# WilliamVenner/squad-mortar-helper

Hardware: AMD Instinct MI355X
Metric: map frames/sec (1920x1080 full CV pipeline), whole job (higher is better)
Workload: dtype u8/f32

## Files before the change

### include/smh_vision_hip_debug.h

```cpp
#ifndef SMH_VISION_HIP_DEBUG_H
#define SMH_VISION_HIP_DEBUG_H

#include "smh_vision_hip.h"

#ifdef __cplusplus
extern "C" {
#endif

SMHV_API int smhv_debug_lsd_classic(int on);
SMHV_API int smhv_debug_lsd_tile_cap(uint32_t cap);
SMHV_API int smhv_debug_lsd_threads(uint32_t threads);
SMHV_API int smhv_debug_pattern_copy(smhv_batch *b, const void *d_frames, uint32_t n, uint32_t rows_in_flight, void *stream);
SMHV_API int smhv_debug_heightmap_color_map_device(smhv_heightmap *hm, void *d_rgba, float *ms);
SMHV_API int smhv_debug_skip_line_search(int on);
SMHV_API int smhv_debug_lsd_spin_limit(uint32_t polls);
SMHV_API int smhv_debug_no_host_atomics(int on);
SMHV_API int smhv_debug_side_kernel(smhv_ctx *ctx, uint32_t workgroups, void *stream);

SMHV_API int smhv_debug_pipeline_stats(smhv_pipeline *p, uint64_t out[32]);
SMHV_API int smhv_debug_pipeline_peek(smhv_pipeline *p, uint64_t out[16]);

SMHV_API int smhv_debug_marker_table(smhv_ctx *ctx, uint32_t *bits);

SMHV_API int smhv_debug_crc32_host_level(const void *data, uint64_t nbytes, int level, uint32_t *crc);
SMHV_API int smhv_debug_band_rows(uint32_t frame_w, uint32_t frame_h, uint32_t n, int fused, uint32_t *rows, uint32_t *bands, int *tiles);
SMHV_API int smhv_debug_map_band_rows(uint32_t rows);
SMHV_API int smhv_debug_render_form(uint32_t form);
SMHV_API int smhv_debug_render_rule(uint32_t map_w, uint32_t map_h, float sw, float sh, uint32_t hm_w, uint32_t hm_h, float *ratio, float *switch_ratio,
                                    uint32_t *lds_texels, uint32_t *form);
SMHV_API int smhv_debug_feed_rows(uint32_t rows);
SMHV_API int smhv_debug_feed_gray_form(uint32_t form);
SMHV_API int smhv_debug_ingest_feed(smhv_ingest *q, uint32_t n, uint32_t *counter);

#ifdef __cplusplus
}
#endif

#endif
```

### squad-mortar-helper_amd/_lib.py

```python
import ctypes as C
import os

_HERE = os.path.dirname(os.path.abspath(__file__))
LIB_PATH = os.environ.get("SMH_VISION_HIP_LIB") or os.path.join(_HERE, "libsmh_vision_hip.so")

MAX_LINES = 32
MAX_SCALES = 3

STAGE_MARKERS, STAGE_UI_MAP, STAGE_OCR, STAGE_SCALES, STAGE_ALL = 0x1, 0x2, 0x4, 0x8, 0xF
STAGE_MINIMAP = 0x10
STAGE_EXACT_STATS = 0x20
STAGE_LSD_HELPERS = 0x40
STAGE_FIRING = 0x80
STAGE_HEIGHTMAP_OVERLAY = 0x100
FIRING_BOUNDS_OFFSET = 1
FIRING_NONE, FIRING_SCALES, FIRING_HEIGHTMAP = 0, 1, 2
VIEW_NONE, VIEW_OCR_INPUT, VIEW_FIND_SCALES_INPUT, VIEW_LSD_PREPROCESS, VIEW_LSD_INPUT, VIEW_CROPPED_BRQ = range(6)
IMAGE_UI_MAP = 100
IMAGE_HEIGHTMAP_OVERLAY = 101
RENDER_HEIGHTMAP, RENDER_MARKERS, RENDER_BOUNDS_OFFSET = 1, 2, 4
RENDER_MAX_LINES = 256
PRIM_LINE, PRIM_RECT, PRIM_FOREGROUND, PRIM_SHIFT1 = 0, 1, 0x100, 0x200
RENDER_MAX_PRIMS = 256
LAYER_MINIMAP_BOUNDS = 1
# ... 106 lines not shown
                ("team_bits", C.c_uint32), ("reserved1", C.c_uint32)]


class DebugOptionsStruct(C.Structure):
    _fields_ = [("size", C.c_uint32), ("flags", C.c_uint32), ("scale", C.c_uint32), ("n_runs", C.c_uint32), ("runs", C.POINTER(TextRun)),
                ("n_probes", C.c_uint32), ("reserved", C.c_uint32), ("probes", C.POINTER(ProbePoint))]


class FeedEntry(C.Structure):
    _fields_ = [("offset", C.c_uint64), ("length", C.c_uint32), ("frame", C.c_uint32), ("kind", C.c_uint32), ("crc", C.c_uint32)]


class FeedHeader(C.Structure):
    _fields_ = [("n_entries", C.c_uint32), ("frames_done", C.c_uint32), ("n_maps", C.c_uint32), ("has_last_crc", C.c_uint32),
                ("last_crc", C.c_uint32), ("reserved", C.c_uint32), ("bytes_used", C.c_uint64)]


LOG_FN = C.CFUNCTYPE(None, C.c_int, C.c_char_p)

SIGNATURES = {
    "smhv_init": (C.c_int, [C.c_int, LOG_FN, C.POINTER(C.c_void_p)]),
    "smhv_shutdown": (None, [C.c_void_p]),
    "smhv_thread_ctx": (C.c_int, [C.c_void_p]),
    "smhv_set_ray_table": (C.c_int, [C.c_void_p, C.POINTER(C.c_float), C.POINTER(C.c_float)]),
    "smhv_last_error": (C.c_char_p, []),
    "smhv_map_bounds": (C.c_int, [C.c_uint32, C.c_uint32, C.POINTER(C.c_uint32)]),
    "smhv_button_bounds": (C.c_int, [C.c_uint32, C.c_uint32, C.POINTER(C.c_uint32)]),
    "smhv_load_frame": (C.c_int, [C.c_void_p, C.c_void_p, C.c_uint32, C.c_uint32]),
    "smhv_load_frame_view": (C.c_int, [C.c_void_p, C.c_void_p] + [C.c_uint32] * 6),
    "smhv_load_frame_device": (C.c_int, [C.c_void_p, C.c_void_p, C.c_uint32, C.c_uint32]),
    "smhv_crop_to_map": (C.c_int, [C.c_void_p, C.c_int, C.POINTER(C.c_int), C.POINTER(C.c_uint32), C.c_void_p]),
    "smhv_red_pixels": (C.c_int, [C.c_void_p, C.POINTER(C.c_uint32)]),
    "smhv_ocr_preprocess": (C.c_int, [C.c_void_p, C.POINTER(C.c_void_p), C.POINTER(C.c_size_t)]),
    "smhv_find_scales_preprocess": (C.c_int, [C.c_void_p, C.c_uint32, C.POINTER(C.c_void_p), C.POINTER(C.c_uint32), C.POINTER(C.c_uint32)]),
    "smhv_isolate_map_markers": (C.c_int, [C.c_void_p]),
    "smhv_mask_marker_lines": (C.c_int, [C.c_void_p]),
    "smhv_get_lsd_image": (C.c_int, [C.c_void_p, C.c_void_p, C.POINTER(C.c_uint32), C.POINTER(C.c_uint32)]),
    "smhv_find_longest_line": (C.c_int, [C.c_void_p, C.c_float, C.c_float, C.c_float, C.POINTER(Line), C.POINTER(C.c_float)]),
    "smhv_find_marker_lines": (C.c_int, [C.c_void_p, C.c_uint32, C.POINTER(Line), C.POINTER(C.c_uint32)]),
    "smhv_lsd_stats": (C.c_int, [C.c_void_p, C.c_uint32, C.c_int, C.POINTER(C.c_uint32), C.POINTER(C.c_uint64)]),
    "smhv_calc_meters_to_px_ratio": (C.c_int, [C.c_void_p, C.POINTER(C.c_uint32), C.c_uint32, C.POINTER(C.c_double), C.POINTER(C.c_int), C.POINTER(C.c_uint32)]),
    "smhv_find_minimap": (C.c_int, [C.c_void_p, C.POINTER(C.c_uint32), C.POINTER(C.c_int)]),
    "smhv_get_debug_view": (C.c_int, [C.c_void_p, C.c_int, C.c_void_p, C.POINTER(C.c_uint32), C.POINTER(C.c_uint32)]),
    "smhv_batch_create": (C.c_int, [C.c_void_p, C.c_uint32, C.c_uint32, C.c_uint32, C.POINTER(C.c_void_p)]),
    "smhv_batch_destroy": (None, [C.c_void_p]),
    "smhv_batch_layout_get": (C.c_int, [C.c_void_p, C.POINTER(BatchLayout)]),
    "smhv_batch_run": (C.c_int, [C.c_void_p, C.c_void_p, C.c_uint32, C.c_uint32, C.c_int, C.c_uint32, C.c_void_p, C.c_void_p]),
    "smhv_batch_device_ptrs": (C.c_int, [C.c_void_p] + [C.POINTER(C.c_void_p)] * 6),
    "smhv_batch_tile_mask": (C.c_int, [C.c_void_p, C.POINTER(C.c_void_p), C.POINTER(C.c_void_p), C.POINTER(C.c_uint32)]),
    "smhv_batch_read_tile_mask": (C.c_int, [C.c_void_p, C.c_uint32, C.c_void_p, C.c_void_p, C.c_void_p, C.POINTER(C.c_int)]),
    "smhv_batch_read_results": (C.c_int, [C.c_void_p, C.c_uint32, C.c_uint32, C.POINTER(FrameResult)]),
    "smhv_batch_read_image": (C.c_int, [C.c_void_p, C.c_int, C.c_uint32, C.c_void_p]),
    "smhv_batch_set_scales_stream": (C.c_int, [C.c_void_p, C.c_void_p]),
    "smhv_batch_wait_map_pass": (C.c_int, [C.c_void_p, C.c_void_p]),
    "smhv_batch_enable_timing": (C.c_int, [C.c_void_p, C.c_int]),
    "smhv_batch_lsd_coop_stats": (C.c_int, [C.c_void_p, C.c_uint32, C.c_uint32, C.POINTER(C.c_uint32)]),
    "smhv_batch_stage_ms": (C.c_int, [C.c_void_p, C.POINTER(C.c_float)]),
    "smhv_pipeline_create": (C.c_int, [C.c_void_p, C.c_uint32, C.c_uint32, C.c_uint32, C.c_uint32, C.POINTER(C.c_void_p)]),
    "smhv_pipeline_create_ex": (C.c_int, [C.c_void_p, C.c_uint32, C.c_uint32, C.c_uint32, C.c_uint32, C.c_void_p, C.POINTER(C.c_void_p)]),
    "smhv_pipeline_hold": (C.c_int, [C.c_void_p, C.c_uint32, C.c_void_p]),
    "smhv_debug_pipeline_stats": (C.c_int, [C.c_void_p, C.POINTER(C.c_uint64)]),
    "smhv_debug_pipeline_peek": (C.c_int, [C.c_void_p, C.POINTER(C.c_uint64)]),
    "smhv_pipeline_destroy": (None, [C.c_void_p]),
    "smhv_pipeline_submit": (C.c_int, [C.c_void_p, C.c_void_p, C.c_uint32, C.c_uint32, C.c_int, C.c_uint32, C.c_void_p, C.c_void_p, C.POINTER(C.c_uint32)]),
    "smhv_pipeline_wait": (C.c_int, [C.c_void_p, C.c_uint32]),
    "smhv_pipeline_wait_all": (C.c_int, [C.c_void_p]),
    "smhv_pipeline_slot": (C.c_int, [C.c_void_p, C.c_uint32, C.POINTER(C.c_void_p), C.POINTER(C.c_void_p)]),
    "smhv_shard_range": (None, [C.c_uint64, C.c_uint32, C.c_uint32, C.POINTER(C.c_uint64), C.POINTER(C.c_uint64)]),
    "smhv_node_create": (C.c_int, [C.POINTER(C.c_int), C.c_uint32, C.c_uint32, C.c_uint32, C.c_uint32, C.c_uint32, LOG_FN, C.POINTER(C.c_void_p)]),
    "smhv_node_destroy": (None, [C.c_void_p]),
    "smhv_node_ctx": (C.c_int, [C.c_void_p, C.c_uint32, C.POINTER(C.c_void_p), C.POINTER(C.c_void_p)]),
    "smhv_node_run": (C.c_int, [C.c_void_p, C.POINTER(C.c_void_p), C.POINTER(C.c_uint32), C.c_uint32, C.c_int, C.c_uint32, C.POINTER(C.c_void_p)]),
    "smhv_node_gather": (C.c_int, [C.c_void_p, C.POINTER(FrameResult), C.POINTER(C.c_uint32)]),
    "smhv_debug_lsd_classic": (C.c_int, [C.c_int]),
    "smhv_debug_lsd_tile_cap": (C.c_int, [C.c_uint32]),
    "smhv_debug_lsd_spin_limit": (C.c_int, [C.c_uint32]),
    "smhv_debug_lsd_threads": (C.c_int, [C.c_uint32]),
    "smhv_debug_skip_line_search": (C.c_int, [C.c_int]),
    "smhv_debug_no_host_atomics": (C.c_int, [C.c_int]),
    "smhv_debug_side_kernel": (C.c_int, [C.c_void_p, C.c_uint32, C.c_void_p]),
    "smhv_trait_times": (C.c_int, [C.c_void_p, C.POINTER(C.c_uint64), C.POINTER(C.c_uint64), C.c_int]),
    "smhv_ui_map": (C.c_int, [C.c_void_p, C.POINTER(C.c_void_p), C.POINTER(C.c_uint32), C.POINTER(C.c_uint32)]),
    "smhv_debug_pattern_copy": (C.c_int, [C.c_void_p, C.c_void_p, C.c_uint32, C.c_uint32, C.c_void_p]),
    "smhv_debug_marker_table": (C.c_int, [C.c_void_p, C.c_void_p]),
    "smhv_ingest_create": (C.c_int, [C.c_void_p, C.c_uint32, C.c_uint32, C.c_uint32, C.c_uint32, C.POINTER(C.c_void_p)]),
    "smhv_ingest_create_ex": (C.c_int, [C.c_void_p, C.c_uint32, C.c_uint32, C.c_uint32, C.c_uint32, C.c_uint32, C.POINTER(C.c_void_p)]),
    "smhv_crc32_host": (C.c_uint32, [C.c_void_p, C.c_uint64]),
    "smhv_debug_map_band_rows": (C.c_int, [C.c_uint32]),
    "smhv_debug_band_rows": (C.c_int, [C.c_uint32, C.c_uint32, C.c_uint32, C.c_int, C.POINTER(C.c_uint32), C.POINTER(C.c_uint32), C.POINTER(C.c_int)]),
    "smhv_debug_ingest_feed": (C.c_int, [C.c_void_p, C.c_uint32, C.POINTER(C.c_uint32)]),
    "smhv_debug_crc32_host_level": (C.c_int, [C.c_void_p, C.c_uint64, C.c_int, C.POINTER(C.c_uint32)]),
    "smhv_ingest_destroy": (None, [C.c_void_p]),
    "smhv_ingest_local_cpus": (C.c_int, [C.c_void_p, C.c_char_p, C.c_size_t]),
    "smhv_ingest_bind_thread": (C.c_int, [C.c_void_p]),
    "smhv_ingest_acquire": (C.c_int, [C.c_void_p, C.POINTER(C.c_void_p)]),
    "smhv_ingest_commit": (C.c_int, [C.c_void_p]),
    "smhv_ingest_push": (C.c_int, [C.c_void_p, C.c_void_p]),
    "smhv_ingest_commit_pixels": (C.c_int, [C.c_void_p, C.c_uint32]),
    "smhv_ingest_push_pixels": (C.c_int, [C.c_void_p, C.c_void_p, C.c_uint32]),
    "smhv_ingest_batch": (C.c_int, [C.c_void_p, C.POINTER(C.c_void_p), C.POINTER(C.c_uint32), C.POINTER(C.c_uint32)]),
    "smhv_ingest_reset": (C.c_int, [C.c_void_p]),
    "smhv_ingest_counts": (C.c_int, [C.c_void_p, C.POINTER(C.c_uint64), C.POINTER(C.c_uint64)]),
    "smhv_crc32_device": (C.c_int, [C.c_void_p, C.c_void_p, C.c_uint64, C.POINTER(C.c_uint32)]),
    "smhv_heightmap_create": (C.c_int, [C.c_void_p, C.c_void_p, C.c_uint32, C.c_uint32, C.POINTER(C.c_int32), C.POINTER(C.c_float), C.POINTER(C.c_void_p)]),
    "smhv_heightmap_destroy": (None, [C.c_void_p]),
    "smhv_heightmap_color_map": (C.c_int, [C.c_void_p, C.c_void_p]),
    "smhv_debug_heightmap_color_map_device": (C.c_int, [C.c_void_p, C.c_void_p, C.POINTER(C.c_float)]),
    "smhv_batch_set_firing": (C.c_int, [C.c_void_p, C.c_void_p, C.POINTER(FiringOptions)]),
    "smhv_pipeline_set_firing": (C.c_int, [C.c_void_p, C.c_void_p, C.POINTER(FiringOptions)]),
    "smhv_batch_read_firing": (C.c_int, [C.c_void_p, C.c_uint32, C.c_uint32, C.POINTER(FiringResult)]),
    "smhv_batch_firing_ptr": (C.c_int, [C.c_void_p, C.POINTER(C.c_void_p)]),
    "smhv_firing_solutions": (C.c_int, [C.c_void_p, C.c_void_p, C.c_uint32, C.POINTER(C.c_double), C.POINTER(C.c_uint32), C.c_void_p,
                                        C.POINTER(FiringOptions), C.POINTER(Firing)]),
    "smhv_batch_overlay_ptr": (C.c_int, [C.c_void_p, C.POINTER(C.c_void_p)]),
    "smhv_heightmap_overlay": (C.c_int, [C.c_void_p, C.c_void_p, C.POINTER(FiringOptions), C.c_void_p]),
    "smhv_map_viewport_calc": (C.c_int, [C.c_float, C.c_float, C.c_float, C.c_float, C.c_uint32, C.POINTER(C.c_float), C.POINTER(C.c_float),
                                         C.POINTER(RenderOptions)]),
    "smhv_batch_render": (C.c_int, [C.c_void_p, C.c_uint32, C.c_uint32, C.c_void_p, C.POINTER(RenderOptions), C.c_void_p]),
    "smhv_batch_render_ptr": (C.c_int, [C.c_void_p, C.POINTER(C.c_void_p), C.POINTER(C.c_uint64)]),
    "smhv_batch_render_size": (C.c_int, [C.c_void_p, C.POINTER(C.c_uint32), C.POINTER(C.c_uint32)]),
    "smhv_batch_read_render": (C.c_int, [C.c_void_p, C.c_uint32, C.c_void_p]),
    "smhv_batch_render_layers": (C.c_int, [C.c_void_p, C.c_uint32, C.c_uint32, C.c_void_p, C.POINTER(RenderOptions), C.POINTER(RenderLayersStruct), C.c_void_p]),
    "smhv_render_map_layers": (C.c_int, [C.c_void_p, C.c_void_p, C.POINTER(RenderOptions), C.POINTER(RenderLayersStruct), C.c_void_p, C.c_uint32, C.c_void_p]),
    "smhv_render_map": (C.c_int, [C.c_void_p, C.c_void_p, C.POINTER(RenderOptions), C.c_void_p, C.c_uint32, C.c_void_p]),
    "smhv_label_font": (C.c_int, [C.c_uint8, C.POINTER(C.c_uint8)]),
    "smhv_batch_render_labels": (C.c_int, [C.c_void_p, C.c_uint32, C.c_uint32, C.c_void_p, C.POINTER(RenderOptions), C.POINTER(LabelOptionsStruct), C.c_void_p]),
    "smhv_batch_read_labels": (C.c_int, [C.c_void_p, C.c_uint32, C.c_uint32, C.POINTER(LabelResult)]),
    "smhv_batch_labels_ptr": (C.c_int, [C.c_void_p, C.POINTER(C.c_void_p)]),
    "smhv_render_map_labeled": (C.c_int, [C.c_void_p, C.c_void_p, C.POINTER(RenderOptions), C.POINTER(RenderLayersStruct), C.c_void_p, C.c_uint32,
                                          C.POINTER(LabelOptionsStruct), C.c_void_p, C.POINTER(LabelResult)]),
    "smhv_text_font": (C.c_int, [C.c_uint8, C.POINTER(C.c_uint8)]),
    "smhv_probe_text": (C.c_int, [C.POINTER(Probe), C.c_char_p, C.c_size_t]),
    "smhv_batch_probe": (C.c_int, [C.c_void_p, C.c_uint32, C.c_uint32, C.POINTER(RenderOptions), C.POINTER(ProbePoint), C.c_uint32, C.c_void_p]),
    "smhv_batch_read_probes": (C.c_int, [C.c_void_p, C.c_uint32, C.c_uint32, C.POINTER(Probe)]),
    "smhv_batch_probes_ptr": (C.c_int, [C.c_void_p, C.POINTER(C.c_void_p)]),
    "smhv_batch_render_debug": (C.c_int, [C.c_void_p, C.c_uint32, C.c_uint32, C.POINTER(RenderOptions), C.POINTER(DebugOptionsStruct), C.c_void_p]),
    "smhv_render_map_debug": (C.c_int, [C.c_void_p, C.c_void_p, C.POINTER(RenderOptions), C.POINTER(RenderLayersStruct), C.c_void_p, C.c_uint32,
                                        C.POINTER(LabelOptionsStruct), C.POINTER(DebugOptionsStruct), C.c_void_p, C.POINTER(LabelResult), C.POINTER(Probe)]),
    "smhv_feed_create": (C.c_int, [C.c_void_p, C.c_uint64, C.c_uint32, C.POINTER(C.c_void_p)]),
    "smhv_feed_destroy": (None, [C.c_void_p]),
    "smhv_feed_reset": (C.c_int, [C.c_void_p]),
    "smhv_batch_feed": (C.c_int, [C.c_void_p, C.c_void_p, C.c_uint32, C.c_uint32, C.c_uint32, C.c_void_p]),
    "smhv_feed_read": (C.c_int, [C.c_void_p, C.POINTER(FeedHeader), C.POINTER(FeedEntry), C.c_uint32, C.c_void_p, C.c_uint64]),
    "smhv_feed_ptrs": (C.c_int, [C.c_void_p, C.POINTER(C.c_void_p), C.POINTER(C.c_void_p), C.POINTER(C.c_void_p)]),
    "smhv_feed_frame": (C.c_int, [C.c_void_p, C.c_void_p, C.c_void_p, C.c_uint32, C.POINTER(C.c_double), C.POINTER(C.c_uint32), C.c_uint32]),
    "smhv_web_event_markers": (C.c_int, [C.c_void_p, C.c_uint32, C.c_int, C.c_void_p, C.c_uint64, C.POINTER(C.c_uint64)]),
    "smhv_web_event_heightmap": (C.c_int, [C.c_void_p, C.c_uint32, C.c_uint32, C.POINTER(C.c_int32), C.POINTER(C.c_float), C.c_void_p, C.c_uint64,
                                           C.POINTER(C.c_uint64)]),
    "smhv_web_event_fit": (C.c_int, [C.c_int, C.c_void_p, C.c_uint64, C.POINTER(C.c_uint64)]),
    "smhv_web_interaction_parse": (C.c_int, [C.c_void_p, C.c_uint64, C.POINTER(C.c_uint32), C.POINTER(C.c_float), C.POINTER(C.c_uint32)]),
    "smhv_debug_feed_rows": (C.c_int, [C.c_uint32]),
    "smhv_debug_feed_gray_form": (C.c_int, [C.c_uint32]),
    "smhv_batch_feed_view": (C.c_int, [C.c_void_p, C.c_void_p, C.c_uint32, C.c_uint32, C.c_uint32, C.c_uint32, C.c_void_p]),
    "smhv_feed_frame_view": (C.c_int, [C.c_void_p, C.c_void_p, C.c_void_p, C.c_uint32, C.POINTER(C.c_double), C.POINTER(C.c_uint32), C.c_uint32, C.c_uint32]),
    "smhv_debug_render_form": (C.c_int, [C.c_uint32]),
    "smhv_debug_render_rule": (C.c_int, [C.c_uint32, C.c_uint32, C.c_float, C.c_float, C.c_uint32, C.c_uint32, C.POINTER(C.c_float), C.POINTER(C.c_float),
                                         C.POINTER(C.c_uint32), C.POINTER(C.c_uint32)]),
}


def firing_options(fit_to_minimap=True, viewport=None):
    o = FiringOptions()
    o.size = C.sizeof(FiringOptions)
    o.flags = 0 if fit_to_minimap else FIRING_BOUNDS_OFFSET
    if viewport is not None:
        sw, sh, tx, ty = viewport
# ... 62 lines not shown
```

### squad-mortar-helper_amd/batch.py

```python
import ctypes as C

import numpy as np

from . import _lib as L

STAGE_NAMES = ("button", "map_pass", "brq_pass", "lsd", "scale_ratio")


def make_anchors(per_frame):
    arr = (L.Anchors * len(per_frame))()
    for i, (start_y, scales) in enumerate(per_frame):
        arr[i].n = min(len(scales), L.MAX_SCALES)
        arr[i].scales_start_y = start_y
        for j, (m, x, y) in enumerate(scales[:L.MAX_SCALES]):
            arr[i].scales[j][0], arr[i].scales[j][1], arr[i].scales[j][2] = m, x, y
    return arr


def results_to_dicts(recs):
    out = []
    for r in recs:
        n = r.n_lines
        out.append(dict(
            map_open=int(r.map_open), n_lines=int(n),
            lines=np.array([[r.lines[i].x0, r.lines[i].y0, r.lines[i].x1, r.lines[i].y1] for i in range(n)], np.float32).reshape(-1, 4),
            mpx=(r.mpx if r.has_mpx else None), n_mask_px=int(r.n_mask_px), red_pixels=int(r.red_pixels),
            rounds=int(r.rounds), ray_steps=int(r.ray_steps),
            length_px=np.array(r.length_px[:n], np.float64), meters=np.array(r.meters[:n], np.float64),
            angle=np.array(r.angle[:n], np.float32),
            minimap=(tuple(r.minimap) if r.has_minimap else None),
            status=int(r.status), error=(None if r.status == L.FRAME_OK else "line search gave the frame up (SMHV_FRAME_LSD_STUCK)" if r.status == L.FRAME_LSD_STUCK
                                         else "status %d" % r.status)))
    return out


class FrameBatch:

    def __init__(self, vision, frame_w, frame_h, max_frames, _handle=None):
        self._lib = L.load()
        self._vision = vision
        self._owned = _handle is None
        if _handle is None:
            b = C.c_void_p()
            L.check(self._lib.smhv_batch_create(vision._ctx, frame_w, frame_h, max_frames, C.byref(b)))
        else:
            b = _handle
        self._b = b
        self.max_frames = max_frames
        self.frame_w, self.frame_h = frame_w, frame_h
        self.layout = L.BatchLayout()
        L.check(self._lib.smhv_batch_layout_get(self._b, C.byref(self.layout)))

    def close(self):
        if self._b:
            if self._owned:
                self._lib.smhv_batch_destroy(self._b)
            self._b = None

    def __del__(self):
        try:
            self.close()
        except Exception:
            pass

    @property
    def roi(self):
        return tuple(self.layout.roi)

    def enable_timing(self, on=True):
        L.check(self._lib.smhv_batch_enable_timing(self._b, int(on)))

    def run(self, frames_ptr, n, stages=L.STAGE_ALL, grayscale=True, max_gap=15, anchors=None, stream=0):
        if anchors is not None and len(anchors) < n:
            raise ValueError("anchors holds %d entries, the run covers %d frames" % (len(anchors), n))
        a = C.cast(anchors, C.c_void_p) if anchors is not None else None
        L.check(self._lib.smhv_batch_run(self._b, C.c_void_p(frames_ptr), n, stages, int(bool(grayscale)), max_gap, a, C.c_void_p(stream)))

    def set_scales_stream(self, stream=0):
        L.check(self._lib.smhv_batch_set_scales_stream(self._b, C.c_void_p(stream)))

    def wait_map_pass(self, stream=0):
        L.check(self._lib.smhv_batch_wait_map_pass(self._b, C.c_void_p(stream)))

    def stage_ms(self):
        ms = (C.c_float * 5)()
        L.check(self._lib.smhv_batch_stage_ms(self._b, ms))
        return dict(zip(STAGE_NAMES, [float(v) for v in ms]))

    def lsd_coop_stats(self, first=0, n=None):
        n = self.max_frames - first if n is None else n
        out = np.zeros((n, 4), np.uint32)
        L.check(self._lib.smhv_batch_lsd_coop_stats(self._b, first, n, out.ctypes.data_as(C.POINTER(C.c_uint32))))
        return out

    def device_ptrs(self):
        p = [C.c_void_p() for _ in range(6)]
        L.check(self._lib.smhv_batch_device_ptrs(self._b, *[C.byref(x) for x in p]))
        return dict(zip(("results", "ui", "mask", "ocr", "scales", "bits"), [x.value for x in p]))

    def tile_mask(self, frame=0):
        geo = (C.c_uint32 * 4)()
        L.check(self._lib.smhv_batch_tile_mask(self._b, None, None, geo))
        trows, wcols, opitch, xoff = [int(v) for v in geo]
        tiled = np.zeros((trows, wcols, 8), np.uint32)
        occ = np.zeros((trows, opitch), np.uint8)
        bits = np.zeros((self.roi[3], wcols), np.uint32)
        written = C.c_int(0)
        L.check(self._lib.smhv_batch_read_tile_mask(self._b, frame, tiled.ctypes.data, occ.ctypes.data, bits.ctypes.data, C.byref(written)))
        return (tiled if written.value else None), (occ if written.value else None), bits, xoff

    def read_results(self, first=0, n=None, check=True):
        n = self.max_frames - first if n is None else n
        recs = (L.FrameResult * n)()
        rc = self._lib.smhv_batch_read_results(self._b, first, n, recs)
        if rc != 0 and not (rc == L.E_STATE and not check):
            try:
                L.check(rc)
            except L.VisionError as e:
                e.records = recs if rc == L.E_STATE else None
                raise
        return recs

    def set_firing(self, heightmap=None, fit_to_minimap=True, viewport=None):
        opt = L.firing_options(fit_to_minimap, viewport)
        L.check(self._lib.smhv_batch_set_firing(self._b, heightmap._hm if heightmap is not None else None, C.byref(opt)))

    def read_firing(self, first=0, n=None):
        n = self.max_frames - first if n is None else n
        out = (L.FiringResult * n)()
        L.check(self._lib.smhv_batch_read_firing(self._b, first, n, out))
        raw = np.frombuffer(out, np.uint8).reshape(n, C.sizeof(L.FiringResult))
        n_lines = raw[:, :4].copy().view(np.uint32).reshape(n)
        lines = raw[:, 8:].copy().view(L.firing_dtype()).reshape(n, L.MAX_LINES)
        return n_lines, lines

    def firing_ptr(self):
        d = C.c_void_p()
        L.check(self._lib.smhv_batch_firing_ptr(self._b, C.byref(d)))
        return d.value or 0

    def read_overlay(self, frame):
        return self.read_image(L.IMAGE_HEIGHTMAP_OVERLAY, frame)

    def overlay_ptr(self):
        d = C.c_void_p()
        L.check(self._lib.smhv_batch_overlay_ptr(self._b, C.byref(d)))
        return d.value or 0

    def render(self, viewport, out_w, out_h, first=0, n=None, heightmap=None, markers=False, fit_to_minimap=True, background=(0, 0, 0, 255),
               stream=None, options=None, layers=None):
        from .render import render_options
        n = self.max_frames - first if n is None else n
        opt = options if options is not None else render_options(viewport, out_w, out_h, heightmap is not None, markers, fit_to_minimap, background)
        if layers is not None:
            ly, keep = layers.struct()
            L.check(self._lib.smhv_batch_render_layers(self._b, first, n, heightmap._hm if heightmap is not None else None, C.byref(opt), C.byref(ly), stream))
            del keep
            return
        L.check(self._lib.smhv_batch_render(self._b, first, n, heightmap._hm if heightmap is not None else None, C.byref(opt), stream))

    def render_size(self):
        w, h = C.c_uint32(), C.c_uint32()
        L.check(self._lib.smhv_batch_render_size(self._b, C.byref(w), C.byref(h)))
        return int(w.value), int(h.value)

    def read_render(self, frame):
        w, h = self.render_size()
        out = np.empty((h, w, 4), np.uint8)
        L.check(self._lib.smhv_batch_read_render(self._b, frame, out.ctypes.data))
        return out

    def render_ptr(self):
        d, st = C.c_void_p(), C.c_uint64()
        L.check(self._lib.smhv_batch_render_ptr(self._b, C.byref(d), C.byref(st)))
        return d.value or 0, int(st.value)

    def render_labels(self, options, labels, first=0, n=None, heightmap=None, stream=None):
        n = self.max_frames - first if n is None else n
        lo, keep = labels.struct()
        L.check(self._lib.smhv_batch_render_labels(self._b, first, n, heightmap._hm if heightmap is not None else None, C.byref(options), C.byref(lo), stream))
        del keep
# ... 149 lines not shown
```

### squad-mortar-helper_amd/csrc/smh_feed.inc

```

struct smhv_feed {
	smhv_ctx *ctx = nullptr;
	uint64_t capacity = 0;
	uint32_t max_frames = 0;
	uint8_t *d_bytes = nullptr;
	smhv_feed_header *d_header = nullptr;
	smhv_feed_entry *d_entries = nullptr;
	uint32_t *d_state = nullptr, *d_raw = nullptr, *d_tab = nullptr;
	FeedMap *d_maps = nullptr;
	uint32_t tab_w = 0, tab_h = 0, tab_xoff = 0, tab_ppg = 0;
	uint8_t *d_view = nullptr;
	size_t view_cap = 0;
	hipEvent_t ev_last = nullptr;
	bool used = false;
	smhv_frame_result *d_rec = nullptr, *h_rec = nullptr;
};

extern "C" SMHV_API void smhv_feed_destroy(smhv_feed *f) {
	if (!f) return;
	if (f->ctx) (void)hipSetDevice(f->ctx->device);
	(void)hipDeviceSynchronize();
	void *ptrs[] = {f->d_bytes, f->d_header, f->d_entries, f->d_state, f->d_raw, f->d_tab, f->d_maps, f->d_rec, f->d_view};
	for (void *p : ptrs)
		if (p) (void)hipFree(p);
// ... 77 lines not shown
	const uint32_t cquads = image ? SMH_FEED_IMAGE_ROW / 4u : v.quads, cxoff = image ? 0u : v.xoff;
	if (f->tab_w != cw || f->tab_h != ch || f->tab_xoff != cxoff || f->tab_ppg != v.ppg) {
		if (v.ppg == 4u) HIPCHK(launch_feed_tables(f->d_tab, cw, ch, cxoff, cquads, s));
		else HIPCHK(launch_feed_view_tables(f->d_tab, cw, ch, cxoff, cquads, v.ppg, s));
		f->tab_w = cw; f->tab_h = ch; f->tab_xoff = cxoff; f->tab_ppg = v.ppg;
	}
	FeedRun r;
	memset(&r, 0, sizeof r);
	r.ui = v.base; r.res = res;
	r.ui_stride = v.stride; r.ui_pitch = v.pitch;
	r.w = v.w; r.h = v.h; r.xoff = v.xoff; r.quads = v.quads;
	r.n = n; r.first = first; r.flags = flags;
	r.len_term = crc32_mul(crc32_xpow(32ull * v.w * v.h), 0xFFFFFFFFu) ^ 0xFFFFFFFFu;
	r.rows_per_wave = feed_rows_per_wave(ch, n);
	r.capacity = f->capacity;
	r.raw = f->d_raw; r.tab = f->d_tab; r.state = f->d_state;
	r.header = f->d_header; r.entries = f->d_entries; r.bytes = f->d_bytes; r.maps = f->d_maps;
	if (v.mode == SMH_RND_SRC_UI) HIPCHK(launch_feed(r, s));
	else if (!image) HIPCHK(launch_feed_view(r, v.mode, s));
	else {
		FeedRun c = r;
		c.ui = v.base - 4ull * v.lead; c.ui_pitch = 4ull * SMH_FEED_IMAGE_ROW; c.ui_stride = 0;
		c.w = cw; c.h = ch; c.xoff = 0u; c.quads = cquads;
		HIPCHK(launch_feed_image(c, r, s));
	}
	HIPCHK(hipEventRecord(f->ev_last, s));
	f->used = true;
	return SMHV_OK;
}

static int feed_batch_source(const smhv_batch *b, uint32_t first, uint32_t map_source, bool resolve, FeedSrc *v) {
	const Geom &g = b->g;
	if (map_source > (uint32_t)SMHV_VIEW_CROPPED_BRQ) return fail(SMHV_E_INVALID, "batch_feed_view: unknown map source %u", map_source);
	if (resolve && !b->ui_written) return fail(SMHV_E_STATE, "batch_feed: no run of this batch has produced a ui_map (SMHV_STAGE_UI_MAP)");
	*v = feed_src_ui(g, b->d_ui + (size_t)first * g.ui_stride);
	switch ((int)map_source) {
	case SMHV_VIEW_NONE: break;
	case SMHV_VIEW_OCR_INPUT:
	case SMHV_VIEW_FIND_SCALES_INPUT: {
		const bool ocr = map_source == (uint32_t)SMHV_VIEW_OCR_INPUT;
		if (resolve && !(ocr ? b->ocr_written : b->scales_written))
			return fail(SMHV_E_STATE, "batch_feed_view: no run of this batch has produced the %s image", ocr ? "OCR input (SMHV_STAGE_OCR)" : "scales input (SMHV_STAGE_SCALES with anchors)");
		v->mode = SMH_RND_SRC_GRAY; v->ppg = 16u;
		v->base = (ocr ? b->d_ocr : b->d_scales) + (size_t)first * g.ocr_stride;
		v->pitch = g.ocr_pitch; v->stride = g.ocr_stride; v->xoff = g.q_xoff; v->w = g.qw; v->h = g.qh;
		v->quads = (v->w + v->xoff + 15u) / 16u;
		break;
	}
	case SMHV_VIEW_LSD_INPUT:
		if (resolve && !b->mask_written) return fail(SMHV_E_STATE, "batch_feed_view: no run of this batch has produced the marker mask (SMHV_STAGE_MARKERS)");
		v->mode = SMH_RND_SRC_GRAY; v->ppg = 16u;
		v->base = b->d_mask + (size_t)first * g.mask_stride;
		v->pitch = g.mask_pitch; v->stride = g.mask_stride;
		v->quads = (v->w + v->xoff + 15u) / 16u;
		break;
	default:
		if (resolve && b->ui_gray) return fail(SMHV_E_STATE, "batch_feed_view: the batch's ui_map is grayscale, map source %u needs the colour one", map_source);
		if (map_source == (uint32_t)SMHV_VIEW_CROPPED_BRQ) {
			const uint32_t x0 = g.m_xoff + g.rw / 2u;
			v->mode = SMH_RND_SRC_CROPPED; v->w = g.rw / 2u; v->h = g.rh / 2u;
			if (resolve && (v->w == 0u || v->h == 0u)) return fail(SMHV_E_STATE, "batch_feed_view: the map has no bottom right quarter");
			v->base += (size_t)(g.rh / 2u) * g.ui_pitch + 16ull * (x0 / 4u);
			v->xoff = x0 & 3u; v->quads = (v->w + v->xoff + 3u) / 4u;
		} else v->mode = SMH_RND_SRC_PREPROCESS;
		break;
	}
	return SMHV_OK;
}

extern "C" SMHV_API int smhv_batch_feed_view(smhv_batch *b, smhv_feed *f, uint32_t first, uint32_t n, uint32_t flags, uint32_t map_source, void *stream) {
	if (!b || !f) return fail(SMHV_E_INVALID, "batch_feed: null argument");
	CTX_OPEN(b->ctx);
	CTX_OPEN(f->ctx);
	if (f->ctx->device != b->ctx->device) return fail(SMHV_E_INVALID, "batch_feed: the feed lives on device %d, the batch on %d", f->ctx->device, b->ctx->device);
	if (n == 0u || (uint64_t)first + n > b->max_frames) return fail(SMHV_E_INVALID, "batch_feed: frames [%u, %u + %u) of a batch of %u", first, first, n, b->max_frames);
	FeedSrc v;
	int rc = feed_batch_source(b, first, map_source, false, &v);
	if (rc) return rc;
	rc = feed_check(f, v.w, v.h, n, flags, "batch_feed");
	if (rc) return rc;
	rc = feed_batch_source(b, first, map_source, true, &v);
	if (rc) return rc;
	HIPCHK(hipSetDevice(b->ctx->device));
	return feed_enqueue(f, v, b->d_results + first, first, n, flags, (hipStream_t)stream);
}

extern "C" SMHV_API int smhv_batch_feed(smhv_batch *b, smhv_feed *f, uint32_t first, uint32_t n, uint32_t flags, void *stream) {
	return smhv_batch_feed_view(b, f, first, n, flags, (uint32_t)SMHV_VIEW_NONE, stream);
}

extern "C" SMHV_API int smhv_feed_read(smhv_feed *f, smhv_feed_header *header, smhv_feed_entry *entries, uint32_t max_entries, uint8_t *bytes, uint64_t cap) {
	if (!f || !header) return fail(SMHV_E_INVALID, "feed_read: null argument");
	CTX_OPEN(f->ctx);
	HIPCHK(hipSetDevice(f->ctx->device));
	if (f->used) HIPCHK(wait_event(f->ev_last));
	HIPCHK(hipMemcpy(header, f->d_header, sizeof *header, hipMemcpyDeviceToHost));
	if (entries && header->n_entries > max_entries) return fail(SMHV_E_INVALID, "feed_read: %u entries, room for %u", header->n_entries, max_entries);
	if (bytes && header->bytes_used > cap) return fail(SMHV_E_INVALID, "feed_read: %llu bytes, room for %llu", (unsigned long long)header->bytes_used, (unsigned long long)cap);
	if (entries && header->n_entries) HIPCHK(hipMemcpy(entries, f->d_entries, sizeof(smhv_feed_entry) * header->n_entries, hipMemcpyDeviceToHost));
	if (bytes && header->bytes_used) HIPCHK(hipMemcpy(bytes, f->d_bytes, (size_t)header->bytes_used, hipMemcpyDeviceToHost));
	return SMHV_OK;
}

extern "C" SMHV_API int smhv_feed_ptrs(smhv_feed *f, void **d_header, void **d_entries, void **d_bytes) {
	if (!f) return fail(SMHV_E_INVALID, "feed_ptrs: null feed");
	if (d_header) *d_header = f->d_header;
	if (d_entries) *d_entries = f->d_entries;
	if (d_bytes) *d_bytes = f->d_bytes;
	return SMHV_OK;
}

extern "C" SMHV_API int smhv_debug_feed_gray_form(uint32_t form) {
	if (form != 0u && form != 4u) return fail(SMHV_E_INVALID, "feed gray form %u (0 = the rule, 4 = four lookups per message dword)", form);
	feed_set_gray_form(form);
	return SMHV_OK;
}

extern "C" SMHV_API int smhv_debug_feed_rows(uint32_t rows) {
	if (rows > 64u) return fail(SMHV_E_INVALID, "feed rows per wave %u (0 = the rule, 1 .. 64)", rows);
	feed_set_rows(rows);
	return SMHV_OK;
}

extern "C" SMHV_API int smhv_feed_frame_view(smhv_ctx *c, smhv_feed *f, const smhv_line *lines, uint32_t n_lines, const double *mpx, const uint32_t minimap[4],
                                             uint32_t flags, uint32_t map_source) {
	int rc = require_open(c, "feed_frame");
	if (rc) return rc;
	CTX_OPEN(c);
	if (!f || (n_lines && !lines)) return fail(SMHV_E_INVALID, "feed_frame: null argument");
	CTX_OPEN(f->ctx);
	if (f->ctx->device != c->device) return fail(SMHV_E_INVALID, "feed_frame: the feed lives on device %d, the context on %d", f->ctx->device, c->device);
	if (n_lines > SMHV_MAX_LINES) return fail(SMHV_E_INVALID, "feed_frame: %u lines (at most %u)", n_lines, (unsigned)SMHV_MAX_LINES);
	if (map_source > (uint32_t)SMHV_VIEW_CROPPED_BRQ) return fail(SMHV_E_INVALID, "feed_frame_view: unknown map source %u", map_source);
	smhv_batch *b = c->fb;
	const Geom &g = b->g;
	FeedSrc v = feed_src_ui(g, b->d_ui);
	if (map_source != (uint32_t)SMHV_VIEW_NONE) {
		const int which = (int)map_source;
		const bool brq = which == SMHV_VIEW_OCR_INPUT || which == SMHV_VIEW_FIND_SCALES_INPUT || which == SMHV_VIEW_CROPPED_BRQ;
		v.mode = SMH_RND_SRC_RGBA; v.w = brq ? g.qw : g.rw; v.h = brq ? g.qh : g.rh;
		v.xoff = 0u; v.quads = 0u; v.pitch = 4ull * v.w; v.stride = 0;
	}
	rc = feed_check(f, v.w, v.h, 1, flags, "feed_frame");
	if (rc) return rc;
	HIPCHK(hipSetDevice(c->device));
	if (f->used) HIPCHK(wait_event(f->ev_last));
	if (v.mode == SMH_RND_SRC_RGBA) {
		const uint64_t dw = (uint64_t)v.w * v.h, rows = (dw + SMH_FEED_IMAGE_ROW - 1u) / SMH_FEED_IMAGE_ROW;
		const size_t need = (size_t)rows * SMH_FEED_IMAGE_ROW * 4u;
		if (rows > SMH_FEED_MAX_ROWS) return fail(SMHV_E_INVALID, "feed_frame_view: a view of %u x %u pixels", v.w, v.h);
		if (f->view_cap < need) {
			if (f->d_view) (void)hipFree(f->d_view);
			f->d_view = nullptr; f->view_cap = 0;
			HIPCHK(hipMalloc((void **)&f->d_view, need));
			f->view_cap = need;
		}
		v.lead = (uint32_t)(rows * SMH_FEED_IMAGE_ROW - dw);
		v.base = f->d_view + 4ull * v.lead;
		if (v.lead) HIPCHK(hipMemsetAsync(f->d_view, 0, 4ull * v.lead, c->s_main));
		Buffers bf = make_buffers(b, c->frame_ptr, 0);
		HIPCHK(launch_debug_view(g, bf, 0, (int)map_source, c->isolated ? 1 : 0, f->d_view + 4ull * v.lead, c->s_main));
	}
	smhv_frame_result *h = f->h_rec;
	memset(h, 0, sizeof *h);
	h->map_open = 1u; h->status = SMHV_FRAME_OK;
	h->n_lines = n_lines;
// ... 83 lines not shown
```

### squad-mortar-helper_amd/csrc/smh_kernels.h

```cpp
#pragma once
#include <hip/hip_runtime.h>
#include <stdint.h>

#include "../../include/smh_vision_hip.h"
#include "../../include/smh_vision_hip_debug.h"

namespace smh {

struct Geom {
	uint32_t W, H;
	uint32_t rx, ry, rw, rh;
	uint32_t bx, by, bw, bh;
	uint32_t qx, qy, qw, qh;
	uint32_t m_ax, m_xoff, m_quads, m_block;
	uint32_t q_ax, q_xoff, q_quads, q_block;
	uint64_t frame_bytes;
	uint64_t ui_pitch, ui_stride;
	uint64_t mask_pitch, mask_stride;
	uint32_t bits_pitch_w; uint64_t bits_stride_w;
	uint64_t ocr_pitch, ocr_stride;
};

struct FrameAux {
	uint32_t open;
// ... 206 lines not shown
#define SMH_CULL_CELLS (SMH_SECTOR_DIM * 4)
#define SMH_CULL_TAB_WORDS (SMH_CULL_CELLS + (SMH_SECTOR_ENTRIES + 3) / 4)

#define SVC_MAX_SLOTS 32u
struct SvcSlot {
	Buffers b;
	uint32_t n;
	uint32_t seq;
	uint32_t done;
	uint32_t pad;
	unsigned long long t_pub;
};
#define SVC_REMOTE_RING 12u
#define SVC_REMOTE_OPEN 0x80000000ull
struct SvcRemoteEntry {
	unsigned long long post;
	unsigned long long claim;
	uint32_t res_a[4];
	uint32_t res_b[4];
	unsigned long long pad[2];
};
struct SvcRemote {
	unsigned long long state;
	unsigned long long info;
	unsigned long long pad[6];
	SvcRemoteEntry ring[SVC_REMOTE_RING];
};
#define SVC_HELP_RING 256u
struct SvcCtl {
	int32_t avail;
	uint32_t closing;
	int32_t help_avail;
	uint32_t help_head, help_reserve;
	uint32_t stat_remote;
	uint32_t head;
	uint32_t reserve;
	uint32_t completed;
	uint32_t busy;
	uint32_t stat_items, stat_waves;
	unsigned long long stat_busy, stat_life;
	unsigned long long stat_phase[4];
	unsigned long long stat_help;
	uint32_t stat_requests, stat_attached;
	unsigned long long stat_t_wait, stat_t_sub, stat_t_last;
	uint32_t stat_h_polls, stat_h_empty, stat_h_lost, stat_h_idle_exit, stat_h_closed_exit, stat_h_pad;
	unsigned long long stat_h_cycles, stat_h_cast_cycles;
	unsigned long long help_ring[SVC_HELP_RING];
};
struct SvcHost {
	unsigned long long state;
	uint32_t launches;
	uint32_t pad0;
	uint32_t done_seq[SVC_MAX_SLOTS];
	uint32_t pad[12];
};
struct SvcParams {
	SvcCtl *ctl;
	unsigned long long *ring;
	SvcSlot *slots;
	SvcHost *host;
	const uint32_t *cull_tab;
	const float *ray_off;
	float max_gap;
	uint32_t tile_cap, list_cap;
	uint32_t part_words;
	uint32_t ring_log2;
	uint32_t epoch;
	uint32_t idle_short, idle_long;
	uint32_t flags;
	SvcRemote *remote;
	uint32_t *remote_store;
	uint32_t remote_store_words;
	uint32_t remote_after;
	uint32_t remote_tickets;
	uint32_t remote_last_div;
	uint32_t compact;
};
uint32_t svc_waves_for(const Geom &g, uint32_t tile_limit, uint32_t *part_words, uint32_t *tile_cap, uint32_t *list_cap, uint32_t *lds_bytes, uint32_t *compact = nullptr);
uint32_t svc_store_words_for(const Geom &g, uint32_t tile_cap, uint32_t compact);
hipError_t svc_probe_host_atomics(SvcHost *h, SvcHost *d_h, bool *ok);
hipError_t launch_svc_publish(SvcCtl *ctl, unsigned long long *ring, SvcSlot *slots, uint32_t slot, const Buffers &b, uint32_t n, uint32_t seq, uint32_t ring_log2, hipStream_t s);
hipError_t launch_lsd_service(const Geom &g, const SvcParams &p, uint32_t workgroups, uint32_t waves, uint32_t lds_bytes, hipStream_t s);

enum : uint32_t { MAP_UI = 1u, MAP_MASK = 2u, MAP_PRIO = 0x100u, MAP_BAND_MAJOR = 0x200u };
enum : uint32_t { BRQ_OCR = 1u, BRQ_SCALES = 2u };

hipError_t launch_button(const Geom &g, const Buffers &b, uint32_t n, int force_open, hipStream_t s);
hipError_t launch_map_pass(const Geom &g, const Buffers &b, uint32_t n, uint32_t flags, int grayscale, hipStream_t s, bool tiles_wanted = false, bool overlapped = false);
struct LaunchTuning {
	uint32_t map_lds_total;
	uint32_t map_grid_cap;
	uint32_t lsd_tile_limit;
	uint32_t map_prio;
	uint32_t map_deep;
	uint32_t map_overlapped;
};
uint32_t map_brq_lds_bytes(const Geom &g);
uint32_t lsd_tile_lds_bytes(const Geom &g, uint32_t tile_limit);
hipError_t launch_map_brq_pass(const Geom &g, const Buffers &b, uint32_t n, uint32_t flags, uint32_t qflags, int grayscale, uint32_t fixed_start_y, int use_anchor_start, hipStream_t s,
                               const LaunchTuning *tune = nullptr);
hipError_t launch_pattern_copy(const Geom &g, const Buffers &b, uint32_t n, uint32_t rows_in_flight, hipStream_t s);
void map_band_rows(uint32_t rh, uint32_t n, int fused, uint32_t *rows, int *tiles);
hipError_t launch_brq_pass(const Geom &g, const Buffers &b, uint32_t n, uint32_t flags, uint32_t fixed_start_y, int use_anchor_start, hipStream_t s);
struct LsdFork { hipStream_t s1, s2; hipEvent_t fork, join1, join2; };
bool lsd_rows_only(const Geom &g);
hipError_t launch_lsd(const Geom &g, const Buffers &b, uint32_t n, float max_gap, int mode, float px, float py, hipStream_t s, const LsdFork *fk, uint32_t tile_bs = 0,
                      bool prefer_classic = false, uint32_t tile_limit = 0, bool *record_fused = nullptr);
size_t lsd_coop_ctl_bytes(uint32_t n);
hipError_t launch_scale_ratio(const Geom &g, const Buffers &b, uint32_t n, uint32_t *d_bars, hipStream_t s);
hipError_t launch_find_minimap(const Geom &g, const Buffers &b, uint32_t n, hipStream_t s);
hipError_t launch_finalize(const Geom &g, const Buffers &b, uint32_t n, uint32_t stages, hipStream_t s);
hipError_t launch_scales_finalize(const Geom &g, const Buffers &b, uint32_t n, uint32_t stages, uint32_t *d_bars, hipStream_t s);
hipError_t launch_firing_lines(const FiringRun &r, const smhv_line *lines, uint32_t n, uint32_t has_mpx, double mpx, uint32_t has_minimap,
                               const uint32_t minimap[4], smhv_firing *out, hipStream_t s);
hipError_t launch_heightmap_color_map(const uint16_t *hm, uint64_t n, uint32_t *mm, uint32_t *rgba, hipStream_t s);
#define SMH_HM_LUT_ENTRIES 65536u
hipError_t launch_heightmap_lut(const uint16_t *hm, uint64_t n, uint32_t *mm, uint32_t *lut, hipStream_t s);
hipError_t launch_hm_overlay(const Geom &g, const OverlayRun &r, uint32_t n, hipStream_t s);
hipError_t launch_render_map(const Geom &g, const RenderRun &r, uint32_t n, hipStream_t s);
hipError_t launch_render_map_layers(const Geom &g, const RenderRun &r, const RenderLayersRun &y, uint32_t n, hipStream_t s);
hipError_t launch_heightmap_lut16(const uint32_t *lut, uint16_t *lut16, uint32_t *vr, hipStream_t s);
#define SMH_HM_LUT_WORDS (SMH_HM_LUT_ENTRIES + 4u + SMH_HM_LUT_ENTRIES / 2u)
hipError_t launch_labels(const LabelRun &r, uint32_t n, hipStream_t s);
hipError_t launch_debug_text(const Geom &g, const DebugRun &r, uint32_t n, hipStream_t s);
void render_set_form(uint32_t form);
uint32_t render_rule(const Geom &g, const RenderRun &r, uint32_t *texels, float *ratio);
float render_switch_ratio();
hipError_t launch_debug_view(const Geom &g, const Buffers &b, uint32_t frame, int which, int isolated, uint8_t *d_rgba, hipStream_t s);
hipError_t launch_marker_table(uint32_t *d_bits, hipStream_t s);
hipError_t launch_pack_rows(const void *d_src, uint32_t src_pitch_bytes, void *d_dst, uint32_t row_bytes, uint32_t rows, hipStream_t s);
hipError_t launch_side_probe(uint32_t *d_out, uint32_t workgroups, uint32_t spin, hipStream_t s);
hipError_t launch_build_sector_table(unsigned long long *d_tab, uint32_t T, hipStream_t s);
hipError_t launch_build_ray_offsets(float *d_off, hipStream_t s);
size_t lsd_lds_bytes();
void lsd_set_classic(bool on);
void lsd_set_tile_cap(uint32_t cap);
void lsd_set_threads(uint32_t threads);
void lsd_set_spin_limit(uint32_t polls);
hipError_t set_ray_table(const float *dx, const float *dy);
#define SMH_CRC_BS 1024
hipError_t launch_to_bgra(const void *d_src, void *d_bgra, uint64_t n_px, uint32_t layout, hipStream_t s);
hipError_t launch_unpack_rows(const void *d_pack, void *d_frame, uint32_t pitch_px, uint32_t roi_x, uint32_t roi_y, uint32_t roi_w, uint32_t roi_h, uint32_t btn_x,
                              uint32_t btn_y, uint32_t btn_w, uint32_t btn_h, hipStream_t s);
hipError_t launch_crc32(const void *d_msg, uint64_t n_dwords, uint32_t wgs, uint32_t rounds, uint32_t x_skip, const uint32_t *d_x_local,
                        const uint32_t *d_x_wg, uint32_t *d_acc, hipStream_t s);
uint32_t crc32_xpow(uint64_t n);
uint32_t crc32_mul(uint32_t a, uint32_t b);

struct FeedMap { uint64_t dst; uint32_t frame, pad; };
struct FeedRun {
	const uint8_t *ui;
	const smhv_frame_result *res;
	uint64_t ui_stride, ui_pitch;
	uint32_t w, h, xoff, quads;
	uint32_t n, first, flags;
	uint32_t len_term;
	uint32_t rows_per_wave;
	uint64_t capacity;
	uint32_t *raw;
	const uint32_t *tab;
	uint32_t *state;
	smhv_feed_header *header;
	smhv_feed_entry *entries;
	uint8_t *bytes;
	FeedMap *maps;
};
#define SMH_FEED_MAX_ROWS 16384u
hipError_t launch_feed_tables(uint32_t *d_tab, uint32_t w, uint32_t h, uint32_t xoff, uint32_t quads, hipStream_t s);
uint32_t feed_rows_per_wave(uint32_t h, uint32_t n);
void feed_set_rows(uint32_t rows);
hipError_t launch_feed(const FeedRun &r, hipStream_t s);
#define SMH_FEED_IMAGE_ROW 1024u
hipError_t launch_feed_view_tables(uint32_t *d_tab, uint32_t w, uint32_t h, uint32_t xoff, uint32_t quads, uint32_t ppg, hipStream_t s);
hipError_t launch_feed_view(const FeedRun &r, uint32_t src_mode, hipStream_t s);
hipError_t launch_feed_image(const FeedRun &crc, const FeedRun &r, hipStream_t s);
void feed_set_gray_form(uint32_t form);

}
```

### squad-mortar-helper_amd/csrc/smh_misc.hip

```cpp
#include "smh_device.h"
#include "smh_record.inc"

namespace smh {

__global__ void __launch_bounds__(64 * SMHV_MAX_SCALES) k_scale_ratio(Geom g, Buffers b, uint32_t *bars) { scale_ratio_body(g, b, blockIdx.x, bars); }

__device__ __forceinline__ bool flat_pixel(const uint8_t *roi0, uint32_t W, uint32_t x, uint32_t y) {
	const uint32_t *p = (const uint32_t *)(roi0 + ((size_t)y * W + x) * 4);
	const int Wi = (int)W;
	const uint32_t c = p[0] & 0x00FFFFFFu;
	uint32_t mx = 0;
#pragma unroll
	for (int dy = -1; dy <= 1; ++dy)
#pragma unroll
		for (int dx = -1; dx <= 1; ++dx)
			if (dx != 0 || dy != 0) mx = max(mx, (uint32_t)__builtin_amdgcn_sad_u8(c, p[dy * Wi + dx] & 0x00FFFFFFu, 0u));
	return (float)mx / 765.0f <= 0.01f;
}

__device__ uint32_t find_edge(const uint8_t *roi0, uint32_t W, uint32_t w, uint32_t h, uint32_t x0, uint32_t y0, int dir) {
	const uint32_t lane = threadIdx.x & 63u;
	const bool vertical = dir < 2;
	uint32_t c_max = vertical ? h : w, oc_max = vertical ? w : h;
	const int cod = (dir == 0 || dir == 2) ? -1 : 1;
// ... 254 lines not shown
__global__ void k_debug_view(Geom g, Buffers b, uint32_t f, int which, int isolated, uint8_t *out) {
	const bool brq = which == SMHV_VIEW_OCR_INPUT || which == SMHV_VIEW_FIND_SCALES_INPUT || which == SMHV_VIEW_CROPPED_BRQ;
	const uint32_t w = brq ? g.qw : g.rw, h = brq ? g.qh : g.rh;
	const uint32_t i = blockIdx.x * blockDim.x + threadIdx.x;
	if (i >= w * h) return;
	const uint32_t y = i / w, x = i - y * w;
	const uint8_t *fp = b.frames + (size_t)f * g.frame_bytes;
	uint32_t o;
	if (which == SMHV_VIEW_OCR_INPUT || which == SMHV_VIEW_FIND_SCALES_INPUT) {
		const uint8_t *img = (which == SMHV_VIEW_OCR_INPUT ? b.ocr : b.scales) + (size_t)f * g.ocr_stride + g.q_xoff;
		o = (uint32_t)img[(size_t)y * g.ocr_pitch + x] * 0x00010101u | 0xFF000000u;
	} else if (which == SMHV_VIEW_LSD_INPUT) {
		o = (uint32_t)b.mask[(size_t)f * g.mask_stride + (size_t)y * g.mask_pitch + g.m_xoff + x] * 0x00010101u | 0xFF000000u;
	} else {
		const uint32_t fx = brq ? g.qx + x : g.rx + x, fy = brq ? g.qy + y : g.ry + y;
		const uint32_t p = *(const uint32_t *)(fp + ((size_t)fy * g.W + fx) * 4);
		uint32_t bb = p & 255u, gg = (p >> 8) & 255u, rr = (p >> 16) & 255u;
		if (which == SMHV_VIEW_LSD_PREPROCESS && isolated && !is_marker(rr, gg, bb)) { rr = 0; gg = 0; bb = 0; }
		o = rr | (gg << 8) | (bb << 16) | 0xFF000000u;
	}
	((uint32_t *)out)[i] = o;
}

__global__ void k_marker_table(uint32_t *bits) {
	const uint32_t w = blockIdx.x * blockDim.x + threadIdx.x;
	if (w >= (1u << 24) / 32u) return;
	uint32_t acc = 0;
	for (uint32_t k = 0; k < 32; ++k) {
		const uint32_t c = w * 32u + k;
		if (is_marker((c >> 16) & 255u, (c >> 8) & 255u, c & 255u)) acc |= 1u << k;
	}
	bits[w] = acc;
}

__global__ void __launch_bounds__(256) k_side_probe(uint32_t *out, uint32_t spin) {
	__shared__ uint32_t lds[21u * 256u];
	asm volatile("; the register footprint of the kernel this one stands in for" ::: "v255", "a23");
	for (uint32_t i = threadIdx.x; i < 21u * 256u; i += blockDim.x) lds[i] = i ^ blockIdx.x;
	__syncthreads();
	uint32_t acc = lds[(threadIdx.x * 37u) % (21u * 256u)];
	for (uint32_t i = 0; i < spin; ++i) acc = acc * 1664525u + 1013904223u;
	if (threadIdx.x == 0) out[blockIdx.x] = acc;
}
hipError_t launch_side_probe(uint32_t *d_out, uint32_t workgroups, uint32_t spin, hipStream_t s) {
	hipLaunchKernelGGL(k_side_probe, dim3(workgroups), dim3(256), 0, s, d_out, spin);
	return hipGetLastError();
}

hipError_t launch_scale_ratio(const Geom &g, const Buffers &b, uint32_t n, uint32_t *d_bars, hipStream_t s) {
	hipLaunchKernelGGL(k_scale_ratio, dim3(n), dim3(64 * SMHV_MAX_SCALES), 0, s, g, b, d_bars);
	return hipGetLastError();
}

hipError_t launch_find_minimap(const Geom &g, const Buffers &b, uint32_t n, hipStream_t s) {
	hipLaunchKernelGGL(k_find_minimap, dim3(n), dim3(256), 0, s, g, b);
	return hipGetLastError();
}

hipError_t launch_finalize(const Geom &g, const Buffers &b, uint32_t n, uint32_t stages, hipStream_t s) {
	if (stages & SMHV_STAGE_FIRING) hipLaunchKernelGGL(k_finalize_firing, dim3(n), dim3(64), 0, s, g, b, stages);
	else hipLaunchKernelGGL(k_finalize, dim3(n), dim3(64), 0, s, g, b, stages);
	return hipGetLastError();
}

hipError_t launch_scales_finalize(const Geom &g, const Buffers &b, uint32_t n, uint32_t stages, uint32_t *d_bars, hipStream_t s) {
	if (stages & SMHV_STAGE_FIRING) hipLaunchKernelGGL(k_scales_finalize_firing, dim3(n), dim3(64 * SMHV_MAX_SCALES), 0, s, g, b, stages, d_bars);
	else hipLaunchKernelGGL(k_scales_finalize, dim3(n), dim3(64 * SMHV_MAX_SCALES), 0, s, g, b, stages, d_bars);
	return hipGetLastError();
}

__global__ void __launch_bounds__(256) k_pack_rows(const uint32_t *__restrict__ src, uint32_t src_pitch_w, uint32_t *__restrict__ dst, uint32_t row_w, uint32_t rows) {
	const uint32_t r = blockIdx.y;
	const uint32_t *s = src + (size_t)r * src_pitch_w;
	uint32_t *d = dst + (size_t)r * row_w;
	for (uint32_t x = blockIdx.x * blockDim.x + threadIdx.x; x < row_w; x += gridDim.x * blockDim.x) d[x] = s[x];
}
hipError_t launch_pack_rows(const void *d_src, uint32_t src_pitch_bytes, void *d_dst, uint32_t row_bytes, uint32_t rows, hipStream_t s) {
	if ((src_pitch_bytes | row_bytes) & 3u) return hipErrorInvalidValue;
	const uint32_t row_w = row_bytes / 4u;
	hipLaunchKernelGGL(k_pack_rows, dim3((row_w + 255u) / 256u, rows), dim3(256), 0, s, (const uint32_t *)d_src, src_pitch_bytes / 4u, (uint32_t *)d_dst, row_w, rows);
	return hipGetLastError();
}

hipError_t launch_debug_view(const Geom &g, const Buffers &b, uint32_t frame, int which, int isolated, uint8_t *d_rgba, hipStream_t s) {
	const bool brq = which == SMHV_VIEW_OCR_INPUT || which == SMHV_VIEW_FIND_SCALES_INPUT || which == SMHV_VIEW_CROPPED_BRQ;
	const uint32_t npx = brq ? g.qw * g.qh : g.rw * g.rh;
	hipLaunchKernelGGL(k_debug_view, dim3((npx + 255) / 256), dim3(256), 0, s, g, b, frame, which, isolated, d_rgba);
	return hipGetLastError();
}

hipError_t launch_marker_table(uint32_t *d_bits, hipStream_t s) {
	hipLaunchKernelGGL(k_marker_table, dim3(((1u << 24) / 32u + 255) / 256), dim3(256), 0, s, d_bits);
	return hipGetLastError();
}

#define CRC_POLY SMH_CRC_POLY
#define CRC_BS 1024

__global__ void __launch_bounds__(CRC_BS) k_crc32(const uint32_t *msg, uint64_t n_dwords, uint32_t rounds, uint32_t x_skip,
                                                 const uint32_t *x_local, const uint32_t *x_wg, uint32_t *acc) {
	__shared__ uint32_t tab[4][256];
	__shared__ uint32_t wsum[CRC_BS / 64];
	const uint32_t tid = threadIdx.x;
	if (tid < 256u) {
		uint32_t c = tid;
		for (int k = 0; k < 8; ++k) c = (c >> 1) ^ ((c & 1u) ? CRC_POLY : 0u);
		tab[0][tid] = c;
	}
	__syncthreads();
	if (tid < 256u) {
		uint32_t c = tab[0][tid];
		for (int k = 1; k < 4; ++k) { c = (c >> 8) ^ tab[0][c & 255u]; tab[k][tid] = c; }
	}
	__syncthreads();
	const uint64_t G = (uint64_t)gridDim.x * CRC_BS, T = (uint64_t)blockIdx.x * CRC_BS + tid;
	const uint64_t pad = (uint64_t)rounds * G * 4u - n_dwords;
	uint32_t v = 0;
	for (uint32_t r = 0; r < rounds; ++r) {
		const uint64_t vi = ((uint64_t)r * G + T) * 4u;
		uint32_t d[4] = {0u, 0u, 0u, 0u};
		if (vi >= pad && ((vi - pad) & 3u) == 0u && (((uintptr_t)msg) & 15u) == 0u) {
			const uint4 q = *(const uint4 *)(msg + (vi - pad));
			d[0] = q.x; d[1] = q.y; d[2] = q.z; d[3] = q.w;
		} else {
#pragma unroll
			for (int j = 0; j < 4; ++j) if (vi + j >= pad) d[j] = msg[vi + j - pad];
		}
		if (r) v = gf2_mulmod(v, x_skip);
#pragma unroll
		for (int j = 0; j < 4; ++j) {
			const uint32_t c = v ^ d[j];
			v = tab[3][c & 255u] ^ tab[2][(c >> 8) & 255u] ^ tab[1][(c >> 16) & 255u] ^ tab[0][c >> 24];
		}
	}
	v = gf2_mulmod(v, x_local[tid]);
	v = wave_xor32_dpp(v);
	if ((tid & 63u) == 0u) wsum[tid >> 6] = v;
	__syncthreads();
	if (tid == 0) {
		uint32_t w = 0;
		for (int k = 0; k < CRC_BS / 64; ++k) w ^= wsum[k];
		atomicXor(acc, gf2_mulmod(w, x_wg[blockIdx.x]));
	}
}

uint32_t crc32_xpow(uint64_t n) {
	uint32_t r = 0x80000000u, b = 0x40000000u;
	for (; n; n >>= 1) { if (n & 1u) r = gf2_mulmod(r, b); b = gf2_mulmod(b, b); }
	return r;
}
uint32_t crc32_mul(uint32_t a, uint32_t b) { return gf2_mulmod(a, b); }

hipError_t launch_crc32(const void *d_msg, uint64_t n_dwords, uint32_t wgs, uint32_t rounds, uint32_t x_skip, const uint32_t *d_x_local,
                        const uint32_t *d_x_wg, uint32_t *d_acc, hipStream_t s) {
	hipLaunchKernelGGL(k_crc32, dim3(wgs), dim3(CRC_BS), 0, s, (const uint32_t *)d_msg, n_dwords, rounds, x_skip, d_x_local, d_x_wg, d_acc);
	return hipGetLastError();
}

template <int BPP>
__global__ void __launch_bounds__(256) k_to_bgra(const uint32_t *__restrict__ src, uint4 *__restrict__ dst, uint64_t n_groups, uint64_t n_px) {
	for (uint64_t gidx = (uint64_t)blockIdx.x * 256u + threadIdx.x; gidx < n_groups; gidx += (uint64_t)gridDim.x * 256u) {
		uint32_t w[4] = {0u, 0u, 0u, 0u}, px[4];
		const uint64_t n_src_dwords = (n_px * BPP + 3u) / 4u;
#pragma unroll
		for (int k = 0; k < BPP; ++k) { const uint64_t i = gidx * BPP + k; if (i < n_src_dwords) w[k] = src[i]; }
		if (BPP == 4) {
// ... 60 lines not shown
```

### squad-mortar-helper_amd/csrc/smh_runtime.cpp

```cpp
#include <hip/hip_runtime.h>

#include <atomic>
#include <condition_variable>
#include <deque>
#include <thread>
#include <cmath>
#include <cstdarg>
#include <cstdio>
#include <cstdlib>
#include <cstring>
#include <ctime>
#include <sched.h>
#include <pthread.h>
#include <cctype>
#include <mutex>
#include <vector>
#include <new>
#include <string>

#include "smh_consts.h"
#include "smh_kernels.h"

using namespace smh;

// ... 90 lines not shown
	if ((uint64_t)xr + w > W || (uint64_t)yb + h > H || w == 0 || h == 0)
		return fail(SMHV_E_GEOMETRY, "frame %ux%u: button bounds underflow", W, H);
	out[0] = W - xr - w; out[1] = H - yb - h; out[2] = w; out[3] = h;
	return SMHV_OK;
}

static int compute_geom(uint32_t W, uint32_t H, Geom *g) {
	uint32_t m[4], bt[4];
	int rc = smhv_map_bounds(W, H, m);
	if (rc) return rc;
	rc = smhv_button_bounds(W, H, bt);
	if (rc) return rc;
	memset(g, 0, sizeof *g);
	g->W = W; g->H = H;
	g->rx = m[0]; g->ry = m[1]; g->rw = m[2]; g->rh = m[3];
	g->bx = bt[0]; g->by = bt[1]; g->bw = bt[2]; g->bh = bt[3];
	g->qw = g->rw / 2; g->qh = g->rh / 2;
	g->qx = g->rx + g->qw; g->qy = g->ry + g->qh;
	if (g->qw < SMH_OCR_DILATE_RADIUS || g->qh < SMH_OCR_DILATE_RADIUS) return fail(SMHV_E_GEOMETRY, "frame %ux%u too small", W, H);
	g->m_ax = g->rx & ~3u; g->m_xoff = g->rx - g->m_ax;
	g->m_quads = (g->rw + g->m_xoff + 3u) / 4u;
	g->m_block = (g->m_quads + 63u) & ~63u;
	g->q_ax = g->qx & ~3u; g->q_xoff = g->qx - g->q_ax;
	g->q_quads = (g->qw + g->q_xoff + 3u) / 4u;
	g->q_block = (g->q_quads + 63u) & ~63u;
	if (g->m_block > 1024u) return fail(SMHV_E_GEOMETRY, "frame %ux%u: map ROI wider than 4096 px is not supported", W, H);
	const uint32_t mq = (g->m_quads + 15u) & ~15u, qq = (g->q_quads + 15u) & ~15u;
	g->frame_bytes = (uint64_t)W * H * 4;
	g->ui_pitch = (uint64_t)mq * 16; g->ui_stride = g->ui_pitch * g->rh;
	g->mask_pitch = (uint64_t)mq * 4; g->mask_stride = g->mask_pitch * g->rh;
	g->bits_pitch_w = mq / 8; g->bits_stride_w = (uint64_t)g->bits_pitch_w * g->rh;
	g->ocr_pitch = (uint64_t)qq * 4; g->ocr_stride = g->ocr_pitch * g->qh;
	return SMHV_OK;
}

struct smhv_batch {
	smhv_ctx *ctx = nullptr;
	Geom g{};
	uint32_t max_frames = 0;
	uint8_t *d_ui = nullptr, *d_mask = nullptr, *d_ocr = nullptr, *d_scales = nullptr;
	uint32_t *d_bits = nullptr, *d_bars = nullptr, *d_tiled = nullptr;
	uint8_t *d_occ = nullptr;
	FrameAux *d_aux = nullptr;
	smhv_frame_result *d_results = nullptr;
	smhv_anchors *d_anchors = nullptr;
	BatchError *h_err = nullptr, *d_err = nullptr;
	FarmFrame *d_farm = nullptr;
	uint8_t *d_lsd_ctl = nullptr;
	uint32_t *d_lsd_req = nullptr;
	LsdCacheEntry *d_lsd_cache = nullptr;
	uint32_t lsd_epoch = 0;
	struct AnchorStage { smhv_anchors *h = nullptr; hipEvent_t done = nullptr; };
	std::vector<AnchorStage> anchor_stage;
	static constexpr int TIMING_RING = 64;
	static constexpr int TIMING_EVENTS = 10;
	bool timing = false;
	hipEvent_t (*ev)[TIMING_EVENTS] = nullptr;
	uint64_t timed_runs = 0;
	hipStream_t s_scales = nullptr;
	hipStream_t s_scales_ext = nullptr;
	hipEvent_t ev_map_done = nullptr;
	hipEvent_t ev_fork = nullptr, ev_join = nullptr;
	LsdFork lsd_fork{};
	uint32_t lsd_late_kc = 0;
	uint32_t lsd_bs = 1024;
	bool lsd_prefer_classic = false;
	LaunchTuning tune{0u, 0u, 0u, 0u};
	hipEvent_t ev_probe[3] = {nullptr, nullptr, nullptr};
	bool probe = false, probe_valid = false;
	smhv_heightmap *fire_hm = nullptr;
	smhv_firing_options fire_opt{};
	smhv_firing_result *d_firing = nullptr;
	FiringRun *d_fire_run = nullptr;
	struct FireStage { FiringRun *h = nullptr; hipEvent_t done = nullptr; };
	std::vector<FireStage> fire_stage;
	uint8_t *d_overlay = nullptr;
	uint8_t *d_render = nullptr;
	size_t render_cap = 0;
	uint32_t render_w = 0, render_h = 0;
	smhv_heightmap *render_hm = nullptr;
	hipEvent_t ev_render = nullptr;
	bool ui_written = false;
	bool ui_gray = false, mask_written = false, ocr_written = false, scales_written = false;
	smhv_render_prim *h_prims = nullptr, *d_prims = nullptr;
	hipEvent_t ev_prims = nullptr;
	smhv_label_result *d_labels = nullptr;
	LabelCull *d_label_cull = nullptr;
	smhv_label_line *h_label_extra = nullptr, *d_label_extra = nullptr;
	hipEvent_t ev_label_extra = nullptr;
	smhv_heightmap *label_hm = nullptr;
	smhv_probe *d_probes = nullptr;
	DebugItem *d_dbg_items = nullptr;
	uint8_t *d_dbg_pool = nullptr, *h_dbg_stage = nullptr, *d_dbg_stage = nullptr;
	hipEvent_t ev_dbg_stage = nullptr, ev_dbg = nullptr;
	bool probed = false;
};

struct smhv_heightmap {
	smhv_ctx *ctx = nullptr;
	uint16_t *d = nullptr;
	uint32_t w = 0, h = 0;
	int32_t bounds[4] = {0, 0, 0, 0};
	float scale[3] = {0.0f, 0.0f, 0.0f};
	std::atomic<int> refs{1};
	mutable std::mutex lut_mu;
	mutable std::atomic<uint32_t *> d_lut{nullptr};
};
static void hm_retain(smhv_heightmap *hm) { if (hm) hm->refs.fetch_add(1, std::memory_order_relaxed); }
static void hm_release(smhv_heightmap *hm);

struct smhv_ctx {
	int device = 0;
	smhv_log_fn log = nullptr;
	hipStream_t s_main = nullptr, s_markers = nullptr, s_scales = nullptr;
	hipStream_t s_ui = nullptr;
	hipEvent_t ev_map = nullptr, ev_ui[2] = {nullptr, nullptr};
	hipEvent_t ev_ui_part[3] = {nullptr, nullptr, nullptr};
	uint8_t *h_ui[2] = {nullptr, nullptr};
	size_t h_ui_cap[2] = {0, 0};
	uint8_t *d_ui_tight = nullptr;
	size_t d_ui_tight_cap = 0;
	uint8_t *d_fire = nullptr, *h_fire = nullptr;
	size_t fire_cap = 0;
	std::mutex fire_mu;
	uint32_t ui_turn = 0;
	bool ui_pending = false, minimap_cached = false;
	uint32_t W = 0, H = 0;
	bool have_frame = false;
	uint8_t *d_frame = nullptr;
	size_t d_frame_cap = 0;
	const uint8_t *frame_ptr = nullptr;
	smhv_batch *fb = nullptr;
	uint8_t *h_ocr = nullptr, *h_scales = nullptr;
	uint8_t *h_stage[3] = {nullptr, nullptr, nullptr};
	size_t h_stage_cap[3] = {0, 0, 0};
	smhv_frame_result *h_res = nullptr;
	FrameAux *h_aux = nullptr;
	uint32_t *h_bars = nullptr;
	bool cropped = false, map_open = false, isolated = false, mask_valid = false, scales_valid = false;
	static constexpr int SECTOR_CACHE = 8;
	uint32_t sector_T[SECTOR_CACHE] = {};
	uint32_t *sector_tab[SECTOR_CACHE] = {};
	int sector_n = 0;
	float *d_ray_off = nullptr;
	uint32_t *d_side = nullptr;
	std::atomic<uint64_t> tt_ns[SMHV_TRAIT_CALLS] = {}, tt_calls[SMHV_TRAIT_CALLS] = {};
	std::mutex mu;
	std::atomic<int> refs{1};
	std::atomic<bool> closed{false};
};

static std::mutex g_ctx_mu;
static std::vector<smhv_ctx *> g_ctx_open;

static void ctx_release(smhv_ctx *c) {
	if (c && c->refs.fetch_sub(1, std::memory_order_acq_rel) == 1) delete c;
}
#define CTX_OPEN(c)                                                                                          \
	do {                                                                                                     \
		if (!(c) || (c)->closed.load(std::memory_order_acquire)) return fail(SMHV_E_INVALID, "the context was shut down"); \
	} while (0)

static void logf(smhv_ctx *c, int lvl, const char *fmt, ...) {
	if (!c || !c->log) return;
	char buf[512];
	va_list ap;
// ... 181 lines not shown
	g_no_host_atomics.store(on != 0, std::memory_order_relaxed);
	return SMHV_OK;
}
extern "C" SMHV_API int smhv_debug_side_kernel(smhv_ctx *c, uint32_t workgroups, void *stream) {
	if (!c || workgroups == 0 || workgroups > 1024u) return fail(SMHV_E_INVALID, "side_kernel: 1..1024 workgroups");
	CTX_OPEN(c);
	HIPCHK(hipSetDevice(c->device));
	if (!c->d_side) HIPCHK(hipMalloc((void **)&c->d_side, 1024u * sizeof(uint32_t)));
	HIPCHK(launch_side_probe(c->d_side, workgroups, 64u, (hipStream_t)stream));
	return SMHV_OK;
}
extern "C" SMHV_API int smhv_debug_lsd_threads(uint32_t threads) {
	if (threads != 0 && (threads < 128 || threads > 1024 || threads % 64)) return fail(SMHV_E_INVALID, "lsd_threads: 0 or a multiple of 64 from 128 to 1024");
	lsd_set_threads(threads);
	return SMHV_OK;
}

extern "C" SMHV_API int smhv_debug_lsd_spin_limit(uint32_t polls) {
	lsd_set_spin_limit(polls);
	return SMHV_OK;
}

extern "C" SMHV_API int smhv_set_ray_table(smhv_ctx *c, const float *dx, const float *dy) {
	if (!c || !dx || !dy) return fail(SMHV_E_INVALID, "bad arguments");
	CTX_OPEN(c);
	for (int i = 0; i < SMH_LSD_RAYS; ++i) {
		const double a = (double)i / 10.0 * 3.14159265358979323846 / 180.0;
		if (!(std::fabs((double)dx[i] - std::cos(a)) < 1e-5 && std::fabs((double)dy[i] - std::sin(a)) < 1e-5))
			return fail(SMHV_E_INVALID, "ray table entry %d is not (cos, sin) of %.1f degrees", i, i / 10.0);
	}
	std::lock_guard<std::mutex> lk(g_ctx_mu);
	HIPCHK(hipSetDevice(c->device));
	HIPCHK(hipDeviceSynchronize());
	HIPCHK(set_ray_table(dx, dy));
	for (smhv_ctx *o : g_ctx_open)
		if (o->device == c->device && o->d_ray_off) HIPCHK(launch_build_ray_offsets(o->d_ray_off, c->s_main));
	HIPCHK(hipStreamSynchronize(c->s_main));
	return SMHV_OK;
}

static hipError_t create_stream(hipStream_t *st, const uint32_t *cu_mask) {
	return cu_mask ? hipExtStreamCreateWithCUMask(st, 8, cu_mask) : hipStreamCreateWithFlags(st, hipStreamNonBlocking);
}

extern "C" SMHV_API int smhv_batch_create(smhv_ctx *c, uint32_t W, uint32_t H, uint32_t max_frames, smhv_batch **out) {
	if (!c || !out || max_frames == 0) return fail(SMHV_E_INVALID, "bad arguments");
	*out = nullptr;
	CTX_OPEN(c);
	Geom g;
	int rc = compute_geom(W, H, &g);
	if (rc) return rc;
	HIPCHK(hipSetDevice(c->device));
	smhv_batch *b = new (std::nothrow) smhv_batch();
	if (!b) return fail(SMHV_E_INVALID, "out of host memory");
	c->refs.fetch_add(1, std::memory_order_relaxed);
	b->ctx = c; b->g = g; b->max_frames = max_frames;
	const size_t n = max_frames;
#define ALLOC0(ptr, bytes)                                          \
	do {                                                            \
		hipError_t _e = hipMalloc((void **)&(ptr), (bytes));        \
		if (_e == hipSuccess) _e = hipMemset((ptr), 0, (bytes));    \
		if (_e != hipSuccess) { smhv_batch_destroy(b); return fail(SMHV_E_HIP, "allocating %zu bytes: %s", (size_t)(bytes), hipGetErrorString(_e)); } \
	} while (0)
	ALLOC0(b->d_ui, g.ui_stride * n);
	ALLOC0(b->d_mask, g.mask_stride * n);
	ALLOC0(b->d_bits, g.bits_stride_w * 4 * n);
	ALLOC0(b->d_tiled, tiled_stride_w(g) * 4 * n);
	ALLOC0(b->d_occ, occ_stride(g) * n);
	ALLOC0(b->d_ocr, g.ocr_stride * n);
	ALLOC0(b->d_scales, g.ocr_stride * n);
	ALLOC0(b->d_aux, sizeof(FrameAux) * n);
	ALLOC0(b->d_results, sizeof(smhv_frame_result) * (n + 3));
	ALLOC0(b->d_anchors, sizeof(smhv_anchors) * n);
	ALLOC0(b->d_bars, sizeof(uint32_t) * SMHV_MAX_SCALES * 4 * n);
	ALLOC0(b->d_lsd_ctl, lsd_coop_ctl_bytes(max_frames));
	ALLOC0(b->d_lsd_req, sizeof(uint32_t) * SMH_LSD_REQ_CAP * n);
	ALLOC0(b->d_farm, sizeof(FarmFrame) * n);
	ALLOC0(b->d_lsd_cache, sizeof(LsdCacheEntry) * SMH_LSD_CACHE_SLOTS * n);
#undef ALLOC0
	{
		hipError_t e = hipHostMalloc((void **)&b->h_err, sizeof(BatchError), hipHostMallocMapped | hipHostMallocCoherent);
		if (e == hipSuccess) { memset(b->h_err, 0, sizeof(BatchError)); e = hipHostGetDevicePointer((void **)&b->d_err, b->h_err, 0); }
		if (e == hipSuccess) e = hipEventCreateWithFlags(&b->ev_map_done, hipEventDisableTiming);
		if (max_frames > 1 && !lsd_rows_only(b->g)) {
			if (e == hipSuccess) e = create_stream(&b->lsd_fork.s1, nullptr);
			if (e == hipSuccess) e = create_stream(&b->lsd_fork.s2, nullptr);
			if (e == hipSuccess) e = hipEventCreateWithFlags(&b->lsd_fork.fork, hipEventDisableTiming);
			if (e == hipSuccess) e = hipEventCreateWithFlags(&b->lsd_fork.join1, hipEventDisableTiming);
			if (e == hipSuccess) e = hipEventCreateWithFlags(&b->lsd_fork.join2, hipEventDisableTiming);
		}
		if (e != hipSuccess) { smhv_batch_destroy(b); return fail(SMHV_E_HIP, "branch streams: %s", hipGetErrorString(e)); }
	}
	*out = b;
	return SMHV_OK;
}

extern "C" SMHV_API void smhv_batch_destroy(smhv_batch *b) {
	if (!b) return;
	if (b->ctx) (void)hipSetDevice(b->ctx->device);
	(void)hipDeviceSynchronize();
	void *ptrs[] = {b->d_ui, b->d_mask, b->d_bits, b->d_tiled, b->d_occ, b->d_ocr, b->d_scales, b->d_aux, b->d_results, b->d_anchors, b->d_bars, b->d_farm,
	                b->d_lsd_ctl, b->d_lsd_req, b->d_lsd_cache, b->d_firing, b->d_fire_run, b->d_overlay, b->d_render, b->d_prims, b->d_labels,
	                b->d_label_cull, b->d_label_extra, b->d_probes, b->d_dbg_items, b->d_dbg_pool, b->d_dbg_stage};
	for (void *p : ptrs)
		if (p) (void)hipFree(p);
	if (b->h_prims) (void)hipHostFree(b->h_prims);
	if (b->ev_prims) (void)hipEventDestroy(b->ev_prims);
	if (b->h_label_extra) (void)hipHostFree(b->h_label_extra);
	if (b->ev_label_extra) (void)hipEventDestroy(b->ev_label_extra);
	if (b->h_dbg_stage) (void)hipHostFree(b->h_dbg_stage);
	if (b->ev_dbg_stage) (void)hipEventDestroy(b->ev_dbg_stage);
	if (b->ev_dbg) (void)hipEventDestroy(b->ev_dbg);
	if (b->h_err) (void)hipHostFree(b->h_err);
	for (auto &a : b->anchor_stage) {
		if (a.h) (void)hipHostFree(a.h);
		if (a.done) (void)hipEventDestroy(a.done);
	}
	for (auto &a : b->fire_stage) {
		if (a.h) (void)hipHostFree(a.h);
		if (a.done) (void)hipEventDestroy(a.done);
	}
	hm_release(b->fire_hm);
	hm_release(b->render_hm);
	hm_release(b->label_hm);
	if (b->ev_render) (void)hipEventDestroy(b->ev_render);
	if (b->ev) {
		for (int r = 0; r < smhv_batch::TIMING_RING; ++r)
			for (int i = 0; i < smhv_batch::TIMING_EVENTS; ++i) if (b->ev[r][i]) (void)hipEventDestroy(b->ev[r][i]);
		delete[] b->ev;
	}
	if (b->s_scales) (void)hipStreamDestroy(b->s_scales);
	if (b->ev_fork) (void)hipEventDestroy(b->ev_fork);
	if (b->ev_join) (void)hipEventDestroy(b->ev_join);
	if (b->ev_map_done) (void)hipEventDestroy(b->ev_map_done);
	for (auto e : b->ev_probe) if (e) (void)hipEventDestroy(e);
	if (b->lsd_fork.s1) (void)hipStreamDestroy(b->lsd_fork.s1);
	if (b->lsd_fork.s2) (void)hipStreamDestroy(b->lsd_fork.s2);
	if (b->lsd_fork.fork) (void)hipEventDestroy(b->lsd_fork.fork);
	if (b->lsd_fork.join1) (void)hipEventDestroy(b->lsd_fork.join1);
	if (b->lsd_fork.join2) (void)hipEventDestroy(b->lsd_fork.join2);
	ctx_release(b->ctx);
	delete b;
}

static int batch_check_errors(smhv_batch *b, const char *what) {
	BatchError *e = b->h_err;
	if (!e) return SMHV_OK;
	const uint32_t count = __atomic_load_n(&e->count, __ATOMIC_ACQUIRE);
	if (count == 0) return SMHV_OK;
	const BatchError snap = *e;
	memset(e, 0, sizeof *e);
	logf(b->ctx, 1, "%s: %u frame(s) failed, first: frame %u status %u", what, count, snap.frame, snap.status);
	if (snap.status == SMHV_FRAME_LSD_STUCK)
		return fail(SMHV_E_STATE, "%s: %u frame(s) without marker lines (status != 0 in their records); first: frame %u, line search gave up "
		            "(SMHV_FRAME_LSD_STUCK: head %u tail %u list %u/%u lines %u rounds %u spec %u head-state %u)", what, count, snap.frame,
		            snap.info[0], snap.info[1], snap.info[2], snap.info[3], snap.info[4], snap.info[5], snap.info[6], snap.info[7]);
	return fail(SMHV_E_STATE, "%s: %u frame(s) failed; first: frame %u, status %u", what, count, snap.frame, snap.status);
}
extern "C" int smhv_internal_batch_check(smhv_batch *b, const char *what) { return b ? batch_check_errors(b, what) : SMHV_OK; }

extern "C" SMHV_API int smhv_batch_layout_get(smhv_batch *b, smhv_batch_layout *o) {
	if (!b || !o) return fail(SMHV_E_INVALID, "bad arguments");
	const Geom &g = b->g;
	memset(o, 0, sizeof *o);
	o->frame_w = g.W; o->frame_h = g.H;
	o->roi[0] = g.rx; o->roi[1] = g.ry; o->roi[2] = g.rw; o->roi[3] = g.rh;
	o->button[0] = g.bx; o->button[1] = g.by; o->button[2] = g.bw; o->button[3] = g.bh;
	o->brq_w = g.qw; o->brq_h = g.qh;
	o->ui_pitch = g.ui_pitch; o->ui_stride = g.ui_stride; o->ui_offset = (uint64_t)g.m_xoff * 4;
	o->mask_pitch = g.mask_pitch; o->mask_stride = g.mask_stride; o->mask_offset = g.m_xoff;
	o->ocr_pitch = g.ocr_pitch; o->ocr_stride = g.ocr_stride; o->ocr_offset = g.q_xoff;
	o->scales_pitch = g.ocr_pitch; o->scales_stride = g.ocr_stride; o->scales_offset = g.q_xoff;
	o->bits_pitch_words = g.bits_pitch_w; o->bits_stride = g.bits_stride_w * 4; o->bits_xoff = g.m_xoff;
	return SMHV_OK;
}

extern "C" SMHV_API int smhv_batch_enable_timing(smhv_batch *b, int enable) {
	if (!b) return fail(SMHV_E_INVALID, "null batch");
	if (enable && !b->ev) {
		HIPCHK(hipSetDevice(b->ctx->device));
		b->ev = new hipEvent_t[smhv_batch::TIMING_RING][smhv_batch::TIMING_EVENTS]();
		for (int r = 0; r < smhv_batch::TIMING_RING; ++r)
			for (int i = 0; i < smhv_batch::TIMING_EVENTS; ++i) HIPCHK(hipEventCreate(&b->ev[r][i]));
	}
	b->timing = enable != 0;
	b->timed_runs = 0;
	return SMHV_OK;
}

static void hm_release(smhv_heightmap *hm) {
	if (!hm || hm->refs.fetch_sub(1, std::memory_order_acq_rel) != 1) return;
	(void)hipSetDevice(hm->ctx->device);
	(void)hipDeviceSynchronize();
	if (hm->d) (void)hipFree(hm->d);
	if (uint32_t *l = hm->d_lut.load(std::memory_order_acquire)) (void)hipFree(l);
	ctx_release(hm->ctx);
	delete hm;
}

static smhv_firing_options firing_opts(const smhv_firing_options *opt) {
	smhv_firing_options o{};
	o.size = sizeof o;
	if (opt) { o.flags = opt->flags; o.viewport_scale[0] = opt->viewport_scale[0]; o.viewport_scale[1] = opt->viewport_scale[1];
	           o.viewport_top_left[0] = opt->viewport_top_left[0]; o.viewport_top_left[1] = opt->viewport_top_left[1]; }
	if (o.viewport_scale[0] == 0.0f) o.viewport_scale[0] = 1.0f;
	if (o.viewport_scale[1] == 0.0f) o.viewport_scale[1] = 1.0f;
	return o;
}

static void firing_run_params(const smhv_heightmap *hm, const smhv_firing_options *o, FiringRun *r) {
	memset(r, 0, sizeof *r);
	if (hm) {
		r->hm = hm->d; r->hm_w = hm->w; r->hm_h = hm->h;
		r->b0x = (float)hm->bounds[0]; r->b0y = (float)hm->bounds[1];
		r->zscale = (double)hm->scale[2] / 0.1953125;
	}
	r->flags = o->flags;
// ... 22 lines not shown
		hipError_t e = hipMalloc((void **)&b->d_firing, sizeof(smhv_firing_result) * (size_t)b->max_frames);
		if (e == hipSuccess) e = hipMalloc((void **)&b->d_fire_run, sizeof(FiringRun));
		if (e == hipSuccess) e = hipMemset(b->d_firing, 0, sizeof(smhv_firing_result) * (size_t)b->max_frames);
		if (e != hipSuccess) {
			if (b->d_firing) (void)hipFree(b->d_firing);
			if (b->d_fire_run) (void)hipFree(b->d_fire_run);
			b->d_firing = nullptr; b->d_fire_run = nullptr;
			return fail(SMHV_E_HIP, "firing slab: %s", hipGetErrorString(e));
		}
	}
	smhv_batch::FireStage *st = nullptr;
	for (auto &a : b->fire_stage)
		if (hipEventQuery(a.done) == hipSuccess) { st = &a; break; }
	if (!st) {
		smhv_batch::FireStage a;
		hipError_t e = hipHostMalloc((void **)&a.h, sizeof(FiringRun));
		if (e == hipSuccess) e = hipEventCreateWithFlags(&a.done, hipEventDisableTiming);
		if (e != hipSuccess) { if (a.h) (void)hipHostFree(a.h); return fail(SMHV_E_HIP, "firing staging: %s", hipGetErrorString(e)); }
		b->fire_stage.push_back(a);
		st = &b->fire_stage.back();
	}
	firing_run_params(b->fire_hm, &b->fire_opt, st->h);
	st->h->out = b->d_firing;
	HIPCHK(hipMemcpyAsync(b->d_fire_run, st->h, sizeof(FiringRun), hipMemcpyHostToDevice, sb));
	HIPCHK(hipEventRecord(st->done, sb));
	return SMHV_OK;
}

static int hm_lut(const smhv_heightmap *hm, const uint32_t **lut) {
	uint32_t *l = hm->d_lut.load(std::memory_order_acquire);
	if (!l) {
		std::lock_guard<std::mutex> lk(hm->lut_mu);
		l = hm->d_lut.load(std::memory_order_relaxed);
		if (!l) {
			HIPCHK(hipSetDevice(hm->ctx->device));
			hipStream_t s = nullptr;
			hipError_t e = hipMalloc((void **)&l, sizeof(uint32_t) * SMH_HM_LUT_WORDS);
			if (e == hipSuccess) e = hipStreamCreateWithFlags(&s, hipStreamNonBlocking);
			if (e == hipSuccess) e = launch_heightmap_lut(hm->d, (uint64_t)hm->w * hm->h, l + SMH_HM_LUT_ENTRIES, l, s);
			if (e == hipSuccess) e = launch_heightmap_lut16(l, (uint16_t *)(l + SMH_HM_LUT_ENTRIES + 4u), l + SMH_HM_LUT_ENTRIES + 2u, s);
			if (e == hipSuccess) e = hipStreamSynchronize(s);
			if (s) (void)hipStreamDestroy(s);
			if (e != hipSuccess) {
				if (l) (void)hipFree(l);
				return fail(SMHV_E_HIP, "heightmap overlay colour table: %s", hipGetErrorString(e));
			}
			hm->d_lut.store(l, std::memory_order_release);
		}
	}
	*lut = l;
	return SMHV_OK;
}

static int overlay_prepare(smhv_batch *b, const smhv_heightmap *hm, uint32_t flags, const smhv_frame_result *res, hipStream_t s, OverlayRun *r) {
	const uint32_t *lut = nullptr;
	int rc = hm_lut(hm, &lut);
	if (rc) return rc;
	if (!b->d_overlay) {
		const size_t bytes = b->g.ui_stride * (size_t)b->max_frames;
		hipError_t e = hipMalloc((void **)&b->d_overlay, bytes);
		if (e == hipSuccess) e = hipMemsetAsync(b->d_overlay, 0, bytes, s);
		if (e != hipSuccess) {
			if (b->d_overlay) (void)hipFree(b->d_overlay);
			b->d_overlay = nullptr;
			return fail(SMHV_E_HIP, "overlay slab: %s", hipGetErrorString(e));
		}
	}
	memset(r, 0, sizeof *r);
	r->ui = b->d_ui; r->out = b->d_overlay; r->aux = b->d_aux; r->res = res;
	r->hm = hm->d; r->lut = lut; r->hm_w = hm->w; r->hm_h = hm->h;
	r->b0x = (float)hm->bounds[0]; r->b0y = (float)hm->bounds[1];
	r->flags = flags;
	return SMHV_OK;
}

static int check_overlay_stages(uint32_t stages, const smhv_heightmap *hm) {
	if (!(stages & SMHV_STAGE_HEIGHTMAP_OVERLAY)) return SMHV_OK;
	if ((stages & (SMHV_STAGE_UI_MAP | SMHV_STAGE_MINIMAP)) != (SMHV_STAGE_UI_MAP | SMHV_STAGE_MINIMAP))
		return fail(SMHV_E_INVALID, "SMHV_STAGE_HEIGHTMAP_OVERLAY needs SMHV_STAGE_UI_MAP and SMHV_STAGE_MINIMAP");
	if (!hm) return fail(SMHV_E_INVALID, "SMHV_STAGE_HEIGHTMAP_OVERLAY needs a heightmap (smhv_batch_set_firing / smhv_pipeline_set_firing)");
	return SMHV_OK;
}

struct SvcPublish { SvcCtl *ctl; unsigned long long *ring; SvcSlot *slots; uint32_t slot, seq, ring_log2; const uint32_t *cull_tab; bool have_cull; hipStream_t s_pro; hipEvent_t ev_pro;
                    bool *published; };
static int batch_run_impl(smhv_batch *b, const void *d_frames, uint32_t n, uint32_t stages, int grayscale, uint32_t max_gap,
                          const smhv_anchors *anchors, hipStream_t s, hipStream_t sl, const SvcPublish *svc = nullptr) {
	if (!b || !d_frames || n == 0 || n > b->max_frames) return fail(SMHV_E_INVALID, "bad arguments (n=%u, capacity %u)", n, b ? b->max_frames : 0);
	if ((uintptr_t)d_frames & 3u) return fail(SMHV_E_INVALID, "d_frames is not aligned to a pixel (4 bytes)");
	CTX_OPEN(b->ctx);
	if ((stages & (SMHV_STAGE_ALL | SMHV_STAGE_MINIMAP)) == 0) return fail(SMHV_E_INVALID, "no stage selected");
	if ((stages & SMHV_STAGE_FIRING) && !(stages & SMHV_STAGE_MARKERS)) return fail(SMHV_E_INVALID, "SMHV_STAGE_FIRING needs SMHV_STAGE_MARKERS");
	{ int rc = check_overlay_stages(stages, b->fire_hm); if (rc) return rc; }
	stages &= SMHV_STAGE_ALL | SMHV_STAGE_MINIMAP | SMHV_STAGE_EXACT_STATS | SMHV_STAGE_LSD_HELPERS | SMHV_STAGE_FIRING | SMHV_STAGE_HEIGHTMAP_OVERLAY;
	HIPCHK(hipSetDevice(b->ctx->device));
	const Geom &g = b->g;
	Buffers bf = make_buffers(b, (const uint8_t *)d_frames, 0);
	OverlayRun orun{};
	if (stages & SMHV_STAGE_HEIGHTMAP_OVERLAY) {
		int rc = overlay_prepare(b, b->fire_hm, b->fire_opt.flags, bf.results, s, &orun);
		if (rc) return rc;
	}
	if ((bf.co.epoch & 0xFFFFu) == 0u && b->d_farm) HIPCHK(hipMemsetAsync(b->d_farm, 0, sizeof(FarmFrame) * (size_t)b->max_frames, s));
	if (stages & SMHV_STAGE_LSD_HELPERS) bf.co.ctl = (LsdCtl *)b->d_lsd_ctl;
	if (svc && svc->have_cull) bf.cull_tab = svc->cull_tab;
	else if ((stages & SMHV_STAGE_MARKERS) && !(stages & SMHV_STAGE_EXACT_STATS)) {
		int rc = sector_table_for(b->ctx, max_gap, s, &bf);
		if (rc) return rc;
	}
	const bool scales = (stages & SMHV_STAGE_SCALES) && anchors;
	const hipStream_t sb = (svc && svc->s_pro) ? svc->s_pro : s;
	if (scales) {
		smhv_batch::AnchorStage *st = nullptr;
		for (auto &a : b->anchor_stage)
			if (hipEventQuery(a.done) == hipSuccess) { st = &a; break; }
		if (!st) {
			smhv_batch::AnchorStage a;
			hipError_t e = hipHostMalloc((void **)&a.h, sizeof(smhv_anchors) * b->max_frames);
			if (e == hipSuccess) e = hipEventCreateWithFlags(&a.done, hipEventDisableTiming);
			if (e != hipSuccess) { if (a.h) (void)hipHostFree(a.h); return fail(SMHV_E_HIP, "anchor staging: %s", hipGetErrorString(e)); }
			b->anchor_stage.push_back(a);
			st = &b->anchor_stage.back();
		}
		memcpy(st->h, anchors, sizeof(smhv_anchors) * n);
		HIPCHK(hipMemcpyAsync(b->d_anchors, st->h, sizeof(smhv_anchors) * n, hipMemcpyHostToDevice, sb));
		HIPCHK(hipEventRecord(st->done, sb));
	}
	if (stages & SMHV_STAGE_FIRING) {
		int rc = firing_upload(b, sb);
		if (rc) return rc;
		bf.firing = b->d_fire_run;
	}
	const bool t = b->timing;
	hipEvent_t *ev = t ? b->ev[b->timed_runs % smhv_batch::TIMING_RING] : nullptr;
#define STAGE_BEGIN(i, st) do { if (t) HIPCHK(hipEventRecord(ev[2 * (i)], (st))); } while (0)
#define STAGE_END(i, st) do { if (t) HIPCHK(hipEventRecord(ev[2 * (i) + 1], (st))); } while (0)
	STAGE_BEGIN(0, sb);
	HIPCHK(launch_button(g, bf, n, 0, sb));
	STAGE_END(0, sb);
	if (sb != s) {
		HIPCHK(hipEventRecord(svc->ev_pro, sb));
		HIPCHK(hipStreamWaitEvent(s, svc->ev_pro, 0));
	}
	uint32_t mflags = 0, qflags = 0;
	if (stages & SMHV_STAGE_MARKERS) mflags |= MAP_MASK;
	if (stages & SMHV_STAGE_UI_MAP) mflags |= MAP_UI;
	if (stages & SMHV_STAGE_OCR) qflags |= BRQ_OCR;
	if (scales) qflags |= BRQ_SCALES;
	if (b->probe) HIPCHK(hipEventRecord(b->ev_probe[0], s));
	STAGE_BEGIN(1, s);
	if (mflags && qflags) HIPCHK(launch_map_brq_pass(g, bf, n, mflags, qflags, grayscale, 0, 1, s, &b->tune));
	else if (mflags) HIPCHK(launch_map_pass(g, bf, n, mflags, grayscale, s, true, b->tune.map_overlapped != 0u));
	STAGE_END(1, s);
	if (mflags & MAP_UI) { b->ui_written = true; b->ui_gray = grayscale != 0; }
	if (mflags & MAP_MASK) b->mask_written = true;
	if (qflags & BRQ_OCR) b->ocr_written = true;
	if (qflags & BRQ_SCALES) b->scales_written = true;
	STAGE_BEGIN(2, s);
	if (qflags && !mflags) HIPCHK(launch_brq_pass(g, bf, n, qflags, 0, 1, s));
	STAGE_END(2, s);
	if (!svc) HIPCHK(hipEventRecord(b->ev_map_done, s));
	if (b->probe) HIPCHK(hipEventRecord(b->ev_probe[1], s));
	if (sl != s) HIPCHK(hipStreamWaitEvent(sl, b->ev_map_done, 0));
	const bool skip_lsd = g_skip_lsd.load(std::memory_order_relaxed);
	if (svc) {
		if (stages & SMHV_STAGE_MINIMAP) HIPCHK(launch_find_minimap(g, bf, n, s));
		if (stages & SMHV_STAGE_HEIGHTMAP_OVERLAY) HIPCHK(launch_hm_overlay(g, orun, n, s));
		bf.rec_stages = SMH_REC_ON | (scales ? stages : (stages & ~SMHV_STAGE_SCALES));
		bf.rec_bars = b->d_bars;
		STAGE_BEGIN(3, s);
		HIPCHK(launch_svc_publish(svc->ctl, svc->ring, svc->slots, svc->slot, bf, n, svc->seq, svc->ring_log2, s));
		if (svc->published) *svc->published = true;
		STAGE_END(3, s);
		STAGE_BEGIN(4, s);
		STAGE_END(4, s);
		if (t) b->timed_runs++;
		return SMHV_OK;
	}
	STAGE_BEGIN(3, sl);
	const uint32_t late_kc = b->lsd_late_kc;
	if (late_kc > 0u) { bf.lsd_flags |= SMH_LSD_LATE_HELP; bf.lsd_late_kc = late_kc; }
	bool record_fused = false;
	if (!(stages & SMHV_STAGE_MINIMAP)) {
		bf.rec_stages = SMH_REC_ON | (scales ? stages : (stages & ~SMHV_STAGE_SCALES));
		bf.rec_bars = b->d_bars;
	}
	if ((stages & SMHV_STAGE_MARKERS) && !skip_lsd) HIPCHK(launch_lsd(g, bf, n, (float)max_gap, 0, 0.0f, 0.0f, sl, b->lsd_fork.s1 ? &b->lsd_fork : nullptr, b->lsd_bs, b->lsd_prefer_classic,
	                                                      (mflags && qflags) ? b->tune.lsd_tile_limit : 0u,
	                                                      &record_fused));
	STAGE_END(3, sl);
	if (b->probe) { HIPCHK(hipEventRecord(b->ev_probe[2], sl)); b->probe_valid = (stages & SMHV_STAGE_MARKERS) && mflags; }
	if (stages & SMHV_STAGE_MINIMAP) HIPCHK(launch_find_minimap(g, bf, n, sl));
	if (stages & SMHV_STAGE_HEIGHTMAP_OVERLAY) HIPCHK(launch_hm_overlay(g, orun, n, sl));
	STAGE_BEGIN(4, sl);
	if (record_fused) {  }
	else if (scales) HIPCHK(launch_scales_finalize(g, bf, n, stages, b->d_bars, sl));
	else HIPCHK(launch_finalize(g, bf, n, stages & ~SMHV_STAGE_SCALES, sl));
	STAGE_END(4, sl);
#undef STAGE_BEGIN
#undef STAGE_END
	if (t) b->timed_runs++;
	return SMHV_OK;
}

extern "C" SMHV_API int smhv_batch_run(smhv_batch *b, const void *d_frames, uint32_t n, uint32_t stages, int grayscale, uint32_t max_gap,
                                       const smhv_anchors *anchors, void *stream) {
	return batch_run_impl(b, d_frames, n, stages, grayscale, max_gap, anchors, (hipStream_t)stream, (hipStream_t)stream);
}

extern "C" SMHV_API int smhv_debug_pattern_copy(smhv_batch *b, const void *d_frames, uint32_t n, uint32_t rows_in_flight, void *stream) {
	if (!b || !d_frames || n == 0 || n > b->max_frames || (rows_in_flight != 0u && rows_in_flight != 4u && rows_in_flight != 8u && rows_in_flight != 12u))
		return fail(SMHV_E_INVALID, "bad arguments (rows in flight: 0 = 4, 4, 8, 12)");
	CTX_OPEN(b->ctx);
	HIPCHK(hipSetDevice(b->ctx->device));
	const Buffers bf = make_buffers(b, (const uint8_t *)d_frames, 0);
	HIPCHK(launch_pattern_copy(b->g, bf, n, rows_in_flight, (hipStream_t)stream));
	return SMHV_OK;
}

extern "C" SMHV_API int smhv_batch_wait_map_pass(smhv_batch *b, void *stream) {
	if (!b) return fail(SMHV_E_INVALID, "null batch");
	HIPCHK(hipSetDevice(b->ctx->device));
	HIPCHK(hipStreamWaitEvent((hipStream_t)stream, b->ev_map_done, 0));
	return SMHV_OK;
}

extern "C" SMHV_API int smhv_batch_set_scales_stream(smhv_batch *b, void *stream) {
	if (!b) return fail(SMHV_E_INVALID, "null batch");
	(void)stream;
	return SMHV_OK;
}

extern "C" SMHV_API int smhv_batch_stage_ms(smhv_batch *b, float ms[5]) {
	if (!b || !ms) return fail(SMHV_E_INVALID, "bad arguments");
	if (!b->ev || b->timed_runs == 0) return fail(SMHV_E_STATE, "no timed smhv_batch_run since timing was enabled");
	const uint64_t runs = b->timed_runs < (uint64_t)smhv_batch::TIMING_RING ? b->timed_runs : (uint64_t)smhv_batch::TIMING_RING;
	double acc[5] = {0, 0, 0, 0, 0};
	for (uint64_t r = 0; r < runs; ++r) {
		hipEvent_t *ev = b->ev[(b->timed_runs - 1 - r) % smhv_batch::TIMING_RING];
		for (int i = 0; i < 5; ++i) {
			float m = 0;
			HIPCHK(hipEventSynchronize(ev[2 * i + 1]));
			HIPCHK(hipEventElapsedTime(&m, ev[2 * i], ev[2 * i + 1]));
			acc[i] += m;
		}
	}
	for (int i = 0; i < 5; ++i) ms[i] = (float)(acc[i] / (double)runs);
	b->timed_runs = 0;
	return SMHV_OK;
}

extern "C" SMHV_API int smhv_batch_lsd_coop_stats(smhv_batch *b, uint32_t first, uint32_t n, uint32_t *out) {
	if (!b || !out || (uint64_t)first + n > b->max_frames) return fail(SMHV_E_INVALID, "bad arguments");
	HIPCHK(hipSetDevice(b->ctx->device));
	HIPCHK(hipDeviceSynchronize());
	std::vector<LsdCoop> h(n);
	HIPCHK(hipMemcpy(h.data(), b->d_lsd_ctl + sizeof(LsdCtl) + sizeof(LsdCoop) * (size_t)first, sizeof(LsdCoop) * n, hipMemcpyDeviceToHost));
	for (uint32_t i = 0; i < n; ++i) { out[4 * i] = h[i].stat_groups; out[4 * i + 1] = h[i].stat_hits; out[4 * i + 2] = h[i].stat_casts; out[4 * i + 3] = h[i].req_tail; }
	return SMHV_OK;
}

extern "C" SMHV_API int smhv_batch_device_ptrs(smhv_batch *b, void **r, void **ui, void **mask, void **ocr, void **scales, void **bits) {
	if (!b) return fail(SMHV_E_INVALID, "null batch");
	if (r) *r = b->d_results;
	if (ui) *ui = b->d_ui;
	if (mask) *mask = b->d_mask;
	if (ocr) *ocr = b->d_ocr;
	if (scales) *scales = b->d_scales;
	if (bits) *bits = b->d_bits;
	return SMHV_OK;
}

extern "C" SMHV_API int smhv_batch_tile_mask(smhv_batch *b, void **d_tiled, void **d_occ, uint32_t geometry[4]) {
	if (!b) return fail(SMHV_E_INVALID, "null batch");
	if (d_tiled) *d_tiled = b->d_tiled;
	if (d_occ) *d_occ = b->d_occ;
	if (geometry) { geometry[0] = tiled_rows(b->g); geometry[1] = b->g.bits_pitch_w; geometry[2] = occ_pitch(b->g); geometry[3] = b->g.m_xoff; }
	return SMHV_OK;
}

extern "C" SMHV_API int smhv_batch_read_tile_mask(smhv_batch *b, uint32_t frame, uint32_t *tiled, uint8_t *occ, uint32_t *bits, int *written) {
	if (!b || frame >= b->max_frames) return fail(SMHV_E_INVALID, "bad arguments");
	HIPCHK(hipSetDevice(b->ctx->device));
	HIPCHK(hipDeviceSynchronize());
	const Geom &g = b->g;
	if (tiled) HIPCHK(hipMemcpy(tiled, b->d_tiled + (size_t)frame * tiled_stride_w(g), tiled_stride_w(g) * 4, hipMemcpyDeviceToHost));
	if (occ) HIPCHK(hipMemcpy(occ, b->d_occ + (size_t)frame * occ_stride(g), occ_stride(g), hipMemcpyDeviceToHost));
	if (bits) HIPCHK(hipMemcpy(bits, b->d_bits + (size_t)frame * g.bits_stride_w, g.bits_stride_w * 4, hipMemcpyDeviceToHost));
	if (written) {
		FrameAux a;
		HIPCHK(hipMemcpy(&a, b->d_aux + frame, sizeof a, hipMemcpyDeviceToHost));
		*written = a.tiles ? 1 : 0;
	}
	return SMHV_OK;
}

extern "C" SMHV_API int smhv_batch_read_results(smhv_batch *b, uint32_t first, uint32_t n, smhv_frame_result *out) {
	if (!b || !out || (uint64_t)first + n > b->max_frames) return fail(SMHV_E_INVALID, "bad arguments");
	HIPCHK(hipSetDevice(b->ctx->device));
	HIPCHK(hipDeviceSynchronize());
	HIPCHK(hipMemcpy(out, b->d_results + first, sizeof(smhv_frame_result) * n, hipMemcpyDeviceToHost));
	return batch_check_errors(b, "batch_read_results");
}

static int copy_image_d2h(smhv_ctx *c, int slot, uint8_t *dst, const uint8_t *d_rows, size_t pitch, size_t xoff, size_t width, size_t rows, hipStream_t s) {
	const size_t bytes = pitch * rows;
	if (c->h_stage_cap[slot] < bytes) {
		if (c->h_stage[slot]) { (void)hipHostFree(c->h_stage[slot]); c->h_stage[slot] = nullptr; c->h_stage_cap[slot] = 0; }
		HIPCHK(hipHostMalloc((void **)&c->h_stage[slot], bytes, hipHostMallocDefault));
		c->h_stage_cap[slot] = bytes;
	}
	HIPCHK(hipMemcpyAsync(c->h_stage[slot], d_rows, bytes, hipMemcpyDeviceToHost, s));
	HIPCHK(wait_stream(s));
	for (size_t r = 0; r < rows; ++r) memcpy(dst + r * width, c->h_stage[slot] + r * pitch + xoff, width);
	return SMHV_OK;
}

extern "C" SMHV_API int smhv_batch_read_image(smhv_batch *b, int which, uint32_t frame, uint8_t *out) {
	if (!b || !out || frame >= b->max_frames) return fail(SMHV_E_INVALID, "bad arguments");
	CTX_OPEN(b->ctx);
	const Geom &g = b->g;
	HIPCHK(hipSetDevice(b->ctx->device));
	HIPCHK(hipDeviceSynchronize());
	if (which == SMHV_IMAGE_HEIGHTMAP_OVERLAY && !b->d_overlay) return fail(SMHV_E_STATE, "batch_read_image: no run of this batch had SMHV_STAGE_HEIGHTMAP_OVERLAY");
	switch (which) {
	case 100:
	case SMHV_IMAGE_HEIGHTMAP_OVERLAY:
		HIPCHK(hipMemcpy2D(out, (size_t)g.rw * 4, (which == 100 ? b->d_ui : b->d_overlay) + frame * g.ui_stride + (size_t)g.m_xoff * 4, g.ui_pitch, (size_t)g.rw * 4,
		                   g.rh, hipMemcpyDeviceToHost));
		break;
	case SMHV_VIEW_LSD_INPUT: {
		std::lock_guard<std::mutex> lk(b->ctx->mu);
		return copy_image_d2h(b->ctx, 2, out, b->d_mask + frame * g.mask_stride, g.mask_pitch, g.m_xoff, g.rw, g.rh, b->ctx->s_main);
	}
	case SMHV_VIEW_OCR_INPUT: {
		std::lock_guard<std::mutex> lk(b->ctx->mu);
		return copy_image_d2h(b->ctx, 2, out, b->d_ocr + frame * g.ocr_stride, g.ocr_pitch, g.q_xoff, g.qw, g.qh, b->ctx->s_main);
	}
	case SMHV_VIEW_FIND_SCALES_INPUT: {
		std::lock_guard<std::mutex> lk(b->ctx->mu);
		return copy_image_d2h(b->ctx, 2, out, b->d_scales + frame * g.ocr_stride, g.ocr_pitch, g.q_xoff, g.qw, g.qh, b->ctx->s_main);
	}
	default:
		return fail(SMHV_E_INVALID, "unsupported image id %d", which);
	}
	return SMHV_OK;
}

static std::atomic<int> g_own_queues[64];
struct smhv_pipeline {
	smhv_ctx *ctx = nullptr;
	uint32_t depth = 0;
	smhv_pipeline_options opt{};
	std::vector<smhv_batch *> batch;
	std::vector<hipStream_t> stream;
	std::vector<hipEvent_t> done;
	std::vector<hipEvent_t> hold;
	std::vector<char> held;
	std::vector<hipStream_t> last_sl;
	hipEvent_t ev_after = nullptr;
	LaunchTuning tuning{0u, 0u, 0u, 0u};
	bool adapt = false, tune_on = true;
	float ratio_ema = 0.0f;
	uint64_t submitted = 0;
	uint64_t round_start = 0;
	bool svc = false;
	uint32_t svc_compact = 0;
	uint32_t svc_streams = 0, svc_waves = 0, svc_part_words = 0, svc_tile_cap = 0, svc_list_cap = 0, svc_lds = 0, svc_wgs = 0, svc_ring_log2 = 0;
	SvcCtl *d_svc_ctl = nullptr;
	unsigned long long *d_svc_ring = nullptr;
	SvcSlot *d_svc_slots = nullptr;
	SvcHost *h_svc = nullptr, *d_svc_host = nullptr;
	SvcRemote *d_svc_remote = nullptr;
	uint32_t *d_svc_store = nullptr;
	uint32_t svc_store_words = 0;
	hipStream_t s_search = nullptr, s_pro = nullptr;
	std::mutex peek_mu;
	hipStream_t s_peek = nullptr;
	SvcCtl *h_peek = nullptr;
	smhv_heightmap *fire_hm = nullptr;
	smhv_firing_options fire_opt{};
	std::vector<hipEvent_t> ev_pub;
	std::vector<hipEvent_t> ev_pro;
	std::vector<uint32_t> seq;
	std::vector<hipStream_t> slot_st;
	uint32_t seq_counter = 0, svc_epoch = 0;
	bool svc_key_valid = false;
	const uint32_t *svc_cull = nullptr;
	uint32_t svc_max_gap = 0;
	std::vector<hipStream_t> svc_stream;
	std::vector<uint8_t> slot_frame;
	bool adaptive = false, mode_frame = false;
	uint32_t own_queues = 0;
	struct ModeCtl {
		uint32_t phase = 0, count = 0, settle = 0, key_n = 0, key_stages = 0, key_gap = 0, decisions = 0;
		uint32_t cand_n = 0, cand_stages = 0, cand_gap = 0, cand_count = 0;
		uint32_t remeasured = 0;
		bool window_mixed = false;
		uint64_t frames = 0;
		struct timespec t0{};
		double rate[2] = {0.0, 0.0};
	} mc;
};
static int svc_wait_slot(smhv_pipeline *p, uint32_t slot);
static int slot_wait(smhv_pipeline *p, uint32_t slot) {
	if (p->svc && p->slot_frame[slot]) return svc_wait_slot(p, slot);
	HIPCHK(wait_event(p->done[slot]));
	return SMHV_OK;
}
static int svc_launch(smhv_pipeline *p, uint32_t slot);
static int svc_submit(smhv_pipeline *p, uint32_t slot, const void *d_frames, uint32_t n, uint32_t stages, int grayscale, uint32_t max_gap,
                      const smhv_anchors *anchors, void *after_stream, uint32_t *slot_out);

extern "C" SMHV_API void smhv_pipeline_destroy(smhv_pipeline *p) {
	if (!p) return;
// ... 575 lines not shown

static void reset_frame_state(smhv_ctx *c) {
	c->have_frame = true; c->cropped = false; c->map_open = false; c->isolated = false; c->mask_valid = false; c->minimap_cached = false;
}

extern "C" SMHV_API int smhv_load_frame(smhv_ctx *c, const uint8_t *bgra, uint32_t w, uint32_t h) {
	TraitTimer tt_(c, SMHV_T_LOAD_FRAME);
	if (!c || !bgra || w == 0 || h == 0) return fail(SMHV_E_INVALID, "bad arguments");
	CTX_OPEN(c);
	HIPCHK(hipSetDevice(c->device));
	int rc = ensure_frame_buffers(c, w, h);
	if (rc) return rc;
	const size_t bytes = (size_t)w * h * 4;
	if (c->d_frame_cap < bytes) {
		HIPCHK(hipDeviceSynchronize());
		if (c->d_frame) (void)hipFree(c->d_frame);
		c->d_frame = nullptr; c->d_frame_cap = 0;
		HIPCHK(hipMalloc((void **)&c->d_frame, bytes));
		c->d_frame_cap = bytes;
	}
	const Geom &g = c->fb->g;
	const uint32_t y0 = g.ry < g.by ? g.ry : g.by;
	const uint32_t y1 = (g.ry + g.rh > g.by + g.bh) ? g.ry + g.rh : g.by + g.bh;
	const size_t off = (size_t)y0 * w * 4, len = (size_t)(y1 - y0) * w * 4;
	HIPCHK(hipMemcpyAsync(c->d_frame + off, bgra + off, len, hipMemcpyHostToDevice, c->s_main));
	HIPCHK(wait_stream(c->s_main));
	c->frame_ptr = c->d_frame;
	reset_frame_state(c);
	return SMHV_OK;
}

extern "C" SMHV_API int smhv_load_frame_view(smhv_ctx *c, const uint8_t *parent_bgra, uint32_t parent_w, uint32_t parent_h,
                                              uint32_t x, uint32_t y, uint32_t w, uint32_t h) {
	if (!c || !parent_bgra || w == 0 || h == 0) return fail(SMHV_E_INVALID, "bad arguments");
	if ((uint64_t)x + w > parent_w || (uint64_t)y + h > parent_h)
		return fail(SMHV_E_INVALID, "load_frame_view: the view %ux%u+%u+%u does not lie inside its %ux%u parent", w, h, x, y, parent_w, parent_h);
	if (x == 0 && w == parent_w) return smhv_load_frame(c, parent_bgra + (size_t)y * parent_w * 4, w, h);
	CTX_OPEN(c);
	HIPCHK(hipSetDevice(c->device));
	int rc = ensure_frame_buffers(c, w, h);
	if (rc) return rc;
	const size_t bytes = (size_t)w * h * 4;
	if (c->d_frame_cap < bytes) {
		HIPCHK(hipDeviceSynchronize());
		if (c->d_frame) (void)hipFree(c->d_frame);
		c->d_frame = nullptr; c->d_frame_cap = 0;
		HIPCHK(hipMalloc((void **)&c->d_frame, bytes));
		c->d_frame_cap = bytes;
	}
	const Geom &g = c->fb->g;
	const uint32_t y0 = g.ry < g.by ? g.ry : g.by;
	const uint32_t y1 = (g.ry + g.rh > g.by + g.bh) ? g.ry + g.rh : g.by + g.bh;
	const uint8_t *src = parent_bgra + ((size_t)(y + y0) * parent_w + x) * 4;
	HIPCHK(hipMemcpy2DAsync(c->d_frame + (size_t)y0 * w * 4, (size_t)w * 4, src, (size_t)parent_w * 4, (size_t)w * 4, y1 - y0, hipMemcpyHostToDevice, c->s_main));
	HIPCHK(wait_stream(c->s_main));
	c->frame_ptr = c->d_frame;
	reset_frame_state(c);
	return SMHV_OK;
}

extern "C" SMHV_API int smhv_load_frame_device(smhv_ctx *c, const void *d_bgra, uint32_t w, uint32_t h) {
	TraitTimer tt_(c, SMHV_T_LOAD_FRAME);
	if (!c || !d_bgra || w == 0 || h == 0) return fail(SMHV_E_INVALID, "bad arguments");
	CTX_OPEN(c);
	HIPCHK(hipSetDevice(c->device));
	int rc = ensure_frame_buffers(c, w, h);
	if (rc) return rc;
	c->frame_ptr = (const uint8_t *)d_bgra;
	reset_frame_state(c);
	return SMHV_OK;
}

static int require_open(smhv_ctx *c, const char *what);
extern "C" SMHV_API int smhv_crop_to_map(smhv_ctx *c, int grayscale, int *map_open, uint32_t roi[4], uint8_t *ui_rgba) {
	TraitTimer tt_(c, SMHV_T_CROP_TO_MAP);
	if (!c || !map_open) return fail(SMHV_E_INVALID, "bad arguments");
	if (!c->have_frame) return fail(SMHV_E_INVALID, "crop_to_map called before load_frame");
	HIPCHK(hipSetDevice(c->device));
	smhv_batch *b = c->fb;
	const Geom &g = b->g;
	Buffers bf = make_buffers(b, c->frame_ptr, 0);
	hipStream_t s = c->s_main;
	HIPCHK(launch_button(g, bf, 1, 0, s));
	HIPCHK(launch_map_pass(g, bf, 1, MAP_UI | MAP_MASK, grayscale, s));
	b->ui_written = true; b->ui_gray = grayscale != 0;
	HIPCHK(hipEventRecord(c->ev_map, s));
	Buffers bm = make_buffers(b, c->frame_ptr, 3);
	HIPCHK(launch_find_minimap(g, bm, 1, s));
	HIPCHK(hipMemcpyAsync(c->h_aux, b->d_aux, sizeof(FrameAux), hipMemcpyDeviceToHost, s));
	HIPCHK(hipMemcpyAsync(&c->h_res[3], b->d_results + 3, sizeof(smhv_frame_result), hipMemcpyDeviceToHost, s));
	HIPCHK(wait_stream(s));
	c->cropped = true; c->isolated = false; c->mask_valid = false; c->ui_pending = false;
	c->map_open = c->h_aux->open != 0;
	*map_open = c->map_open ? 1 : 0;
	if (!c->map_open) return SMHV_OK;
	c->minimap_cached = true;
	if (roi) { roi[0] = g.rx; roi[1] = g.ry; roi[2] = g.rw; roi[3] = g.rh; }
	c->mask_valid = true;
	const uint32_t t = (c->ui_turn++) & 1u;
	const size_t ui_bytes = (size_t)g.rw * g.rh * 4;
	if (c->h_ui_cap[t] < ui_bytes) {
		if (c->h_ui[t]) { HIPCHK(hipEventSynchronize(c->ev_ui[t])); (void)hipHostFree(c->h_ui[t]); c->h_ui[t] = nullptr; c->h_ui_cap[t] = 0; }
		HIPCHK(hipHostMalloc((void **)&c->h_ui[t], ui_bytes, hipHostMallocDefault));
		c->h_ui_cap[t] = ui_bytes;
	}
	if (c->d_ui_tight_cap < ui_bytes) {
		HIPCHK(wait_stream(c->s_ui));
		if (c->d_ui_tight) (void)hipFree(c->d_ui_tight);
		c->d_ui_tight = nullptr; c->d_ui_tight_cap = 0;
		HIPCHK(hipMalloc((void **)&c->d_ui_tight, ui_bytes));
		c->d_ui_tight_cap = ui_bytes;
	}
	HIPCHK(hipStreamWaitEvent(c->s_ui, c->ev_map, 0));
	const size_t row_bytes = (size_t)g.rw * 4;
	HIPCHK(launch_pack_rows(b->d_ui + (size_t)g.m_xoff * 4, g.ui_pitch, c->d_ui_tight, (uint32_t)row_bytes, g.rh, c->s_ui));
	if (!ui_rgba) {
		HIPCHK(hipMemcpyAsync(c->h_ui[t], c->d_ui_tight, ui_bytes, hipMemcpyDeviceToHost, c->s_ui));
		HIPCHK(hipEventRecord(c->ev_ui[t], c->s_ui));
		c->ui_pending = true;
		return SMHV_OK;
	}
	const uint32_t parts = 4, rows_per = (g.rh + parts - 1) / parts;
	for (uint32_t k = 0; k < parts; ++k) {
		const uint32_t r0 = k * rows_per, r1 = std::min(g.rh, r0 + rows_per);
		if (r1 > r0) HIPCHK(hipMemcpyAsync(c->h_ui[t] + (size_t)r0 * row_bytes, c->d_ui_tight + (size_t)r0 * row_bytes, (size_t)(r1 - r0) * row_bytes, hipMemcpyDeviceToHost, c->s_ui));
		HIPCHK(hipEventRecord(k + 1 < parts ? c->ev_ui_part[k] : c->ev_ui[t], c->s_ui));
	}
	c->ui_pending = true;
	for (uint32_t k = 0; k < parts; ++k) {
		const uint32_t r0 = k * rows_per, r1 = std::min(g.rh, r0 + rows_per);
		HIPCHK(wait_event(k + 1 < parts ? c->ev_ui_part[k] : c->ev_ui[t]));
		if (r1 > r0) memcpy(ui_rgba + (size_t)r0 * row_bytes, c->h_ui[t] + (size_t)r0 * row_bytes, (size_t)(r1 - r0) * row_bytes);
	}
	return SMHV_OK;
}

extern "C" SMHV_API int smhv_ui_map(smhv_ctx *c, const uint8_t **rgba, uint32_t *w, uint32_t *h) {
	TraitTimer tt_(c, SMHV_T_UI_MAP);
	int rc = require_open(c, "ui_map");
	if (rc) return rc;
	if (!rgba) return fail(SMHV_E_INVALID, "null output");
	if (!c->ui_pending) return fail(SMHV_E_STATE, "ui_map: crop_to_map has not produced a map for this frame");
	HIPCHK(hipSetDevice(c->device));
	const uint32_t t = (c->ui_turn - 1u) & 1u;
	HIPCHK(wait_event(c->ev_ui[t]));
	*rgba = c->h_ui[t];
	if (w) *w = c->fb->g.rw;
	if (h) *h = c->fb->g.rh;
	return SMHV_OK;
}

extern "C" SMHV_API int smhv_red_pixels(smhv_ctx *c, uint32_t *count) {
	if (!c || !count) return fail(SMHV_E_INVALID, "bad arguments");
	if (!c->cropped) return fail(SMHV_E_STATE, "crop_to_map has not run for this frame");
	*count = c->h_aux->red;
	return SMHV_OK;
}

static int require_open(smhv_ctx *c, const char *what) {
	if (!c) return fail(SMHV_E_INVALID, "null context");
	if (!c->have_frame || !c->cropped) return fail(SMHV_E_INVALID, "%s called before load_frame/crop_to_map", what);
	if (!c->map_open) return fail(SMHV_E_STATE, "%s: the map is closed for this frame (crop_to_map returned None)", what);
	return SMHV_OK;
}

extern "C" SMHV_API int smhv_ocr_preprocess(smhv_ctx *c, const uint8_t **out, size_t *len) {
	TraitTimer tt_(c, SMHV_T_OCR_PREPROCESS);
	int rc = require_open(c, "ocr_preprocess");
	if (rc) return rc;
	if (!out || !len) return fail(SMHV_E_INVALID, "null output");
	HIPCHK(hipSetDevice(c->device));
	smhv_batch *b = c->fb;
	const Geom &g = b->g;
	Buffers bf = make_buffers(b, c->frame_ptr, 1);
	hipStream_t s = c->s_scales;
	HIPCHK(launch_brq_pass(g, bf, 1, BRQ_OCR, 0, 0, s));
	rc = copy_image_d2h(c, 1, c->h_ocr, b->d_ocr, g.ocr_pitch, g.q_xoff, g.qw, g.qh, s);
	if (rc) return rc;
	*out = c->h_ocr; *len = (size_t)g.qw * g.qh;
	return SMHV_OK;
}

extern "C" SMHV_API int smhv_find_scales_preprocess(smhv_ctx *c, uint32_t scales_start_y, const uint8_t **out, uint32_t *w, uint32_t *h) {
	TraitTimer tt_(c, SMHV_T_FIND_SCALES_PREPROCESS);
	int rc = require_open(c, "find_scales_preprocess");
	if (rc) return rc;
	HIPCHK(hipSetDevice(c->device));
	smhv_batch *b = c->fb;
	const Geom &g = b->g;
	if (scales_start_y > g.qh) return fail(SMHV_E_INVALID, "scales_start_y %u is below the %u-row quadrant", scales_start_y, g.qh);
	Buffers bf = make_buffers(b, c->frame_ptr, 1);
	hipStream_t s = c->s_scales;
	HIPCHK(launch_brq_pass(g, bf, 1, BRQ_SCALES, scales_start_y, 0, s));
	rc = copy_image_d2h(c, 1, c->h_scales, b->d_scales, g.ocr_pitch, g.q_xoff, g.qw, g.qh, s);
	if (rc) return rc;
	c->scales_valid = true;
	if (out) *out = c->h_scales;
	if (w) *w = g.qw;
	if (h) *h = g.qh;
	return SMHV_OK;
}

extern "C" SMHV_API int smhv_isolate_map_markers(smhv_ctx *c) {
	TraitTimer tt_(c, SMHV_T_ISOLATE_MAP_MARKERS);
	int rc = require_open(c, "isolate_map_markers");
	if (rc) return rc;
	c->isolated = true;
	return SMHV_OK;
}

extern "C" SMHV_API int smhv_mask_marker_lines(smhv_ctx *c) {
	TraitTimer tt_(c, SMHV_T_MASK_MARKER_LINES);
	int rc = require_open(c, "mask_marker_lines");
	if (rc) return rc;
	if (c->mask_valid) return SMHV_OK;
	HIPCHK(hipSetDevice(c->device));
	smhv_batch *b = c->fb;
	Buffers bf = make_buffers(b, c->frame_ptr, 0);
	HIPCHK(launch_map_pass(b->g, bf, 1, MAP_MASK, 1, c->s_markers));
	HIPCHK(wait_stream(c->s_markers));
	c->mask_valid = true;
	return SMHV_OK;
}

static int require_mask(smhv_ctx *c, const char *what) {
	int rc = require_open(c, what);
	if (rc) return rc;
	if (!c->mask_valid) return fail(SMHV_E_INVALID, "%s called before mask_marker_lines", what);
	return SMHV_OK;
}

extern "C" SMHV_API int smhv_get_lsd_image(smhv_ctx *c, uint8_t *out, uint32_t *w, uint32_t *h) {
	int rc = require_mask(c, "get_lsd_image");
	if (rc) return rc;
	HIPCHK(hipSetDevice(c->device));
	const Geom &g = c->fb->g;
	if (w) *w = g.rw;
	if (h) *h = g.rh;
	if (out) {
		rc = copy_image_d2h(c, 0, out, c->fb->d_mask, g.mask_pitch, g.m_xoff, g.rw, g.rh, c->s_markers);
		if (rc) return rc;
	}
	return SMHV_OK;
}

extern "C" SMHV_API int smhv_find_longest_line(smhv_ctx *c, float px, float py, float max_gap, smhv_line *line, float *len_sq) {
	TraitTimer tt_(c, SMHV_T_FIND_LONGEST_LINE);
	int rc = require_mask(c, "find_longest_line");
	if (rc) return rc;
	if (!line || !len_sq) return fail(SMHV_E_INVALID, "null output");
	HIPCHK(hipSetDevice(c->device));
	smhv_batch *b = c->fb;
	Buffers bf = make_buffers(b, c->frame_ptr, 2);
	hipStream_t s = c->s_markers;
	HIPCHK(launch_lsd(b->g, bf, 1, max_gap, 1, px, py, s, nullptr));
	HIPCHK(hipMemcpyAsync(&c->h_res[2], b->d_results + 2, sizeof(smhv_frame_result), hipMemcpyDeviceToHost, s));
	HIPCHK(wait_stream(s));
	*line = c->h_res[2].lines[0];
	*len_sq = (float)c->h_res[2].length_px[0];
	return SMHV_OK;
}

extern "C" SMHV_API int smhv_find_marker_lines(smhv_ctx *c, uint32_t max_gap, smhv_line out[SMHV_MAX_LINES], uint32_t *n) {
	TraitTimer tt_(c, SMHV_T_FIND_MARKER_LINES);
	int rc = require_mask(c, "find_marker_lines");
	if (rc) return rc;
	if (!out || !n) return fail(SMHV_E_INVALID, "null output");
	HIPCHK(hipSetDevice(c->device));
	smhv_batch *b = c->fb;
	Buffers bf = make_buffers(b, c->frame_ptr, 0);
	hipStream_t s = c->s_markers;
	rc = sector_table_for(c, max_gap, s, &bf);
	if (rc) return rc;
	HIPCHK(launch_lsd(b->g, bf, 1, (float)max_gap, 0, 0.0f, 0.0f, s, nullptr, 1024u, true));
	HIPCHK(launch_finalize(b->g, bf, 1, SMHV_STAGE_MARKERS, s));
	HIPCHK(hipMemcpyAsync(&c->h_res[0], b->d_results, sizeof(smhv_frame_result), hipMemcpyDeviceToHost, s));
	HIPCHK(wait_stream(s));
	*n = c->h_res[0].n_lines;
	memcpy(out, c->h_res[0].lines, sizeof(smhv_line) * SMHV_MAX_LINES);
	return SMHV_OK;
}

extern "C" SMHV_API int smhv_lsd_stats(smhv_ctx *c, uint32_t max_gap, int exact, uint32_t *rounds, uint64_t *ray_steps) {
	int rc = require_mask(c, "lsd_stats");
	if (rc) return rc;
	if (!rounds || !ray_steps) return fail(SMHV_E_INVALID, "null output");
	HIPCHK(hipSetDevice(c->device));
	smhv_batch *b = c->fb;
	Buffers bf = make_buffers(b, c->frame_ptr, 2);
	hipStream_t s = c->s_markers;
	if (!exact) {
		rc = sector_table_for(c, max_gap, s, &bf);
		if (rc) return rc;
	}
	HIPCHK(launch_lsd(b->g, bf, 1, (float)max_gap, 0, 0.0f, 0.0f, s, nullptr, 1024u, true));
	HIPCHK(hipMemcpyAsync(&c->h_res[2], b->d_results + 2, sizeof(smhv_frame_result), hipMemcpyDeviceToHost, s));
	HIPCHK(wait_stream(s));
	*rounds = c->h_res[2].rounds;
	*ray_steps = c->h_res[2].ray_steps;
	return SMHV_OK;
}

// ... 423 lines not shown
	if (q->roi) HIPCHK(wait_event(q->done[slot]));
	*host_bgra = q->h_stage[slot];
	q->acquired = true;
	return SMHV_OK;
}

static uint32_t pixel_layout_bytes(uint32_t layout) {
	switch (layout) {
	case SMHV_PIXELS_BGRA8: case SMHV_PIXELS_RGBA8: return 4u;
	case SMHV_PIXELS_RGB8: return 3u;
	case SMHV_PIXELS_LUMA_A8: return 2u;
	case SMHV_PIXELS_LUMA8: return 1u;
	default: return 0u;
	}
}

extern "C" SMHV_API int smhv_ingest_commit_pixels(smhv_ingest *q, uint32_t layout) {
	if (!q || !q->acquired) return fail(SMHV_E_INVALID, "ingest_commit: nothing acquired");
	const uint32_t bpp = pixel_layout_bytes(layout);
	if (!bpp) return fail(SMHV_E_INVALID, "ingest_commit_pixels: unknown pixel layout %u", layout);
	HIPCHK(hipSetDevice(q->ctx->device));
	const uint32_t slot = (uint32_t)(q->head % q->slots);
	if (q->roi) {
		if (layout != SMHV_PIXELS_BGRA8) return fail(SMHV_E_INVALID, "ingest_commit_pixels: a queue created with SMHV_INGEST_ROI_UPLOAD takes BGRA8 frames only");
		{
			std::lock_guard<std::mutex> lk(q->mu);
			q->crc_state[slot] = 1;
			q->jobs.push_back(slot);
		}
		q->cv_job.notify_one();
		q->head++;
		q->acquired = false;
		return SMHV_OK;
	}
	if (layout == SMHV_PIXELS_BGRA8) {
		HIPCHK(hipMemcpyAsync(q->d_stage[slot], q->h_stage[slot], q->frame_bytes, hipMemcpyHostToDevice, q->s));
	} else {
		if (!q->d_raw[slot]) HIPCHK(hipMalloc((void **)&q->d_raw[slot], q->frame_bytes));
		HIPCHK(hipMemcpyAsync(q->d_raw[slot], q->h_stage[slot], q->frame_bytes / 4 * bpp, hipMemcpyHostToDevice, q->s));
		HIPCHK(launch_to_bgra(q->d_raw[slot], q->d_stage[slot], (uint64_t)q->W * q->H, layout, q->s));
	}
	HIPCHK(hipMemsetAsync(q->d_acc + slot, 0, sizeof(uint32_t), q->s));
	HIPCHK(launch_crc32(q->d_stage[slot], q->frame_bytes / 4, q->wgs, q->rounds, q->x_skip, q->d_x_local, q->d_x_wg, q->d_acc + slot, q->s));
	HIPCHK(hipMemcpyAsync(q->h_acc + slot, q->d_acc + slot, sizeof(uint32_t), hipMemcpyDeviceToHost, q->s));
	HIPCHK(hipEventRecord(q->done[slot], q->s));
	q->head++;
	q->acquired = false;
	return SMHV_OK;
}

extern "C" SMHV_API int smhv_ingest_commit(smhv_ingest *q) { return smhv_ingest_commit_pixels(q, SMHV_PIXELS_BGRA8); }

extern "C" SMHV_API int smhv_ingest_push_pixels(smhv_ingest *q, const uint8_t *pixels, uint32_t layout) {
	if (!q || !pixels) return fail(SMHV_E_INVALID, "ingest_push: null argument");
	const uint32_t bpp = pixel_layout_bytes(layout);
	if (!bpp) return fail(SMHV_E_INVALID, "ingest_push_pixels: unknown pixel layout %u", layout);
	uint8_t *dst = nullptr;
	int rc = smhv_ingest_acquire(q, &dst);
	if (rc) return rc;
	memcpy(dst, pixels, q->frame_bytes / 4 * bpp);
	return smhv_ingest_commit_pixels(q, layout);
}

namespace smh { extern std::atomic<uint32_t> g_map_band_rows, g_map_band_major; }
extern "C" SMHV_API int smhv_debug_map_band_rows(uint32_t rows) {
	g_map_band_major.store((rows >> 31) ? 1u : ((rows >> 30) & 1u) ? 2u : 0u, std::memory_order_relaxed);
	rows &= 0x3FFFFFFFu;
	if (rows & 7u) return fail(SMHV_E_INVALID, "debug_map_band_rows: a multiple of 8 (0: the library's rule)");
	g_map_band_rows.store(rows, std::memory_order_relaxed);
	return SMHV_OK;
}

extern "C" SMHV_API int smhv_debug_band_rows(uint32_t frame_w, uint32_t frame_h, uint32_t n, int fused, uint32_t *rows, uint32_t *bands, int *tiles) {
	Geom g;
	int rc = compute_geom(frame_w, frame_h, &g);
	if (rc) return rc;
	uint32_t rb = 0;
	map_band_rows(g.rh, n ? n : 1u, fused, &rb, tiles);
	if (rows) *rows = rb;
	if (bands) *bands = (g.rh + rb - 1) / rb;
	return SMHV_OK;
}

extern "C" SMHV_API int smhv_debug_ingest_feed(smhv_ingest *q, uint32_t n, uint32_t *counter) {
	if (!q || !counter) return fail(SMHV_E_INVALID, "ingest_feed: null argument");
	for (uint32_t i = 0; i < n; ++i) {
		uint8_t *buf = nullptr;
		int rc = smhv_ingest_acquire(q, &buf);
		if (rc) return rc;
		const uint32_t c = (*counter)++;
		buf[0] = (uint8_t)c; buf[1] = (uint8_t)(c >> 8); buf[2] = (uint8_t)(c >> 16); buf[3] = 255;
		rc = smhv_ingest_commit(q);
		if (rc) return rc;
	}
	return SMHV_OK;
}

extern "C" SMHV_API int smhv_ingest_push(smhv_ingest *q, const uint8_t *bgra) { return smhv_ingest_push_pixels(q, bgra, SMHV_PIXELS_BGRA8); }

extern "C" SMHV_API int smhv_ingest_batch(smhv_ingest *q, const void **d_frames, uint32_t *n, uint32_t *last_crc) {
	if (!q || !d_frames || !n) return fail(SMHV_E_INVALID, "ingest_batch: null argument");
	if (q->acquired) return fail(SMHV_E_INVALID, "ingest_batch: a staging buffer is acquired but not committed");
	HIPCHK(hipSetDevice(q->ctx->device));
	while (q->tail < q->head) {
		int rc = ingest_resolve_one(q);
		if (rc == INGEST_FULL) break;
		if (rc) return rc;
	}
	HIPCHK(wait_stream(q->s));
	if (q->roi) HIPCHK(wait_stream(q->s_alt));
	*d_frames = q->d_slab; *n = q->count;
	if (last_crc) *last_crc = q->last_crc;
	return SMHV_OK;
}

extern "C" SMHV_API int smhv_ingest_reset(smhv_ingest *q) {
	if (!q) return fail(SMHV_E_INVALID, "ingest_reset: null argument");
	if (q->acquired) return fail(SMHV_E_INVALID, "ingest_reset: a staging buffer is acquired but not committed");
	q->count = 0;
	return SMHV_OK;
}

extern "C" SMHV_API int smhv_ingest_counts(smhv_ingest *q, uint64_t *n_new, uint64_t *n_dup) {
	if (!q) return fail(SMHV_E_INVALID, "ingest_counts: null argument");
	if (n_new) *n_new = q->n_new;
	if (n_dup) *n_dup = q->n_dup;
	return SMHV_OK;
}

extern "C" SMHV_API int smhv_heightmap_create(smhv_ctx *c, const uint16_t *data, uint32_t w, uint32_t h, const int32_t bounds[4], const float scale[3],
                                              smhv_heightmap **out) {
	if (!c || !data || !bounds || !scale || !out) return fail(SMHV_E_INVALID, "heightmap_create: null argument");
	*out = nullptr;
	CTX_OPEN(c);
	if (w == 0 || h == 0 || (uint64_t)w * h > (1ull << 28)) return fail(SMHV_E_INVALID, "heightmap_create: %u x %u texels (1 .. 2^28)", w, h);
	HIPCHK(hipSetDevice(c->device));
	smhv_heightmap *hm = new (std::nothrow) smhv_heightmap();
	if (!hm) return fail(SMHV_E_INVALID, "out of host memory");
	hm->w = w; hm->h = h;
	memcpy(hm->bounds, bounds, sizeof hm->bounds);
	memcpy(hm->scale, scale, sizeof hm->scale);
	const size_t bytes = (size_t)w * h * sizeof(uint16_t);
	hipError_t e = hipMalloc((void **)&hm->d, bytes);
	if (e == hipSuccess) e = hipMemcpy(hm->d, data, bytes, hipMemcpyHostToDevice);
	if (e != hipSuccess) {
		if (hm->d) (void)hipFree(hm->d);
		delete hm;
		return fail(SMHV_E_HIP, "heightmap_create: %s", hipGetErrorString(e));
	}
	c->refs.fetch_add(1, std::memory_order_relaxed);
	hm->ctx = c;
	*out = hm;
	return SMHV_OK;
}

extern "C" SMHV_API void smhv_heightmap_destroy(smhv_heightmap *hm) { hm_release(hm); }

extern "C" SMHV_API int smhv_heightmap_color_map(smhv_heightmap *hm, uint8_t *rgba) {
	if (!hm || !rgba) return fail(SMHV_E_INVALID, "heightmap_color_map: null argument");
	smhv_ctx *c = hm->ctx;
	CTX_OPEN(c);
	HIPCHK(hipSetDevice(c->device));
	const uint64_t n = (uint64_t)hm->w * hm->h;
	uint32_t *d = nullptr;
	HIPCHK(hipMalloc((void **)&d, 16 + n * 4));
	hipError_t e = launch_heightmap_color_map(hm->d, n, d, d + 4, c->s_main);
// ... 317 lines not shown
	return copy_image_d2h(c, 2, rgba, b->d_render, (size_t)r.out_stride / opt->out_h, 0, (size_t)opt->out_w * 4, opt->out_h, c->s_main);
}

static int check_render_layers(const smhv_render_layers *ly, const char *what) {
	if (!ly) return fail(SMHV_E_INVALID, "%s: null layers", what);
	if (ly->size != sizeof(smhv_render_layers)) return fail(SMHV_E_INVALID, "%s: smhv_render_layers.size %u != %zu", what, ly->size, sizeof(smhv_render_layers));
	if (ly->flags & ~SMHV_LAYER_MINIMAP_BOUNDS) return fail(SMHV_E_INVALID, "%s: unknown layer flags 0x%x", what, ly->flags);
	if (ly->map_source > (uint32_t)SMHV_VIEW_CROPPED_BRQ) return fail(SMHV_E_INVALID, "%s: unknown map source %u", what, ly->map_source);
	if (ly->n_prims > SMHV_RENDER_MAX_PRIMS) return fail(SMHV_E_INVALID, "%s: %u prims (at most %u)", what, ly->n_prims, SMHV_RENDER_MAX_PRIMS);
	if (ly->n_prims && !ly->prims) return fail(SMHV_E_INVALID, "%s: %u prims and a null pointer", what, ly->n_prims);
	for (uint32_t i = 0; i < ly->n_prims; ++i) {
		const smhv_render_prim &p = ly->prims[i];
		if ((p.kind & ~(0xFFu | SMHV_PRIM_FOREGROUND | SMHV_PRIM_SHIFT1)) || (p.kind & 0xFFu) > SMHV_PRIM_RECT)
			return fail(SMHV_E_INVALID, "%s: prim %u has the unknown kind 0x%x", what, i, p.kind);
		if (p.rgba[3] != 255u) return fail(SMHV_E_INVALID, "%s: prim %u has alpha %u (255 only)", what, i, p.rgba[3]);
	}
	return SMHV_OK;
}

static int render_upload_prims(smhv_batch *b, const smhv_render_layers *ly, RenderLayersRun *y, hipStream_t s) {
	if (ly->n_prims == 0u) return SMHV_OK;
	const size_t cap = sizeof(smhv_render_prim) * (size_t)SMHV_RENDER_MAX_PRIMS;
	if (!b->h_prims) HIPCHK(hipHostMalloc((void **)&b->h_prims, cap));
	if (!b->d_prims) HIPCHK(hipMalloc((void **)&b->d_prims, cap));
	if (!b->ev_prims) HIPCHK(hipEventCreateWithFlags(&b->ev_prims, hipEventDisableTiming));
	else HIPCHK(wait_event(b->ev_prims));
	uint32_t k = 0;
	for (uint32_t pass = 0; pass < 2u; ++pass) {
		for (uint32_t i = 0; i < ly->n_prims; ++i)
			if (((ly->prims[i].kind & SMHV_PRIM_FOREGROUND) != 0u) == (pass == 1u)) b->h_prims[k++] = ly->prims[i];
		if (pass == 0u) y->n_below = k;
	}
	y->n_fg = k - y->n_below;
	y->prims = b->d_prims;
	HIPCHK(hipMemcpyAsync(b->d_prims, b->h_prims, sizeof(smhv_render_prim) * (size_t)k, hipMemcpyHostToDevice, s));
	HIPCHK(hipEventRecord(b->ev_prims, s));
	return SMHV_OK;
}

extern "C" SMHV_API int smhv_batch_render_layers(smhv_batch *b, uint32_t first, uint32_t n, const smhv_heightmap *hm, const smhv_render_options *opt,
                                                 const smhv_render_layers *layers, void *stream) {
	if (!b) return fail(SMHV_E_INVALID, "batch_render_layers: null batch");
	CTX_OPEN(b->ctx);
	int rc = check_render_options(opt, hm, "batch_render_layers");
	if (rc) return rc;
	rc = check_render_layers(layers, "batch_render_layers");
	if (rc) return rc;
	if (n == 0u || (uint64_t)first + n > b->max_frames) return fail(SMHV_E_INVALID, "batch_render_layers: frames [%u, %u + %u) of a batch of %u", first, first, n, b->max_frames);
	if (!b->ui_written) return fail(SMHV_E_STATE, "batch_render_layers: no run of this batch has produced a ui_map (SMHV_STAGE_UI_MAP)");
	const Geom &g = b->g;
	RenderLayersRun y{};
	y.flags = layers->flags;
	y.src_mode = SMH_RND_SRC_UI; y.src_w = g.rw; y.src_h = g.rh;
	switch ((int)layers->map_source) {
	case SMHV_VIEW_NONE: break;
	case SMHV_VIEW_OCR_INPUT:
	case SMHV_VIEW_FIND_SCALES_INPUT: {
		const bool ocr = layers->map_source == (uint32_t)SMHV_VIEW_OCR_INPUT;
		if (!(ocr ? b->ocr_written : b->scales_written))
			return fail(SMHV_E_STATE, "batch_render_layers: no run of this batch has produced the %s image", ocr ? "OCR input (SMHV_STAGE_OCR)" : "scales input (SMHV_STAGE_SCALES with anchors)");
		y.src_mode = SMH_RND_SRC_GRAY; y.src = (ocr ? b->d_ocr : b->d_scales) + (size_t)first * g.ocr_stride;
		y.src_pitch = g.ocr_pitch; y.src_stride = g.ocr_stride; y.src_xoff = g.q_xoff; y.src_w = g.qw; y.src_h = g.qh;
		break;
	}
	case SMHV_VIEW_LSD_INPUT:
		if (!b->mask_written) return fail(SMHV_E_STATE, "batch_render_layers: no run of this batch has produced the marker mask (SMHV_STAGE_MARKERS)");
		y.src_mode = SMH_RND_SRC_GRAY; y.src = b->d_mask + (size_t)first * g.mask_stride;
		y.src_pitch = g.mask_pitch; y.src_stride = g.mask_stride; y.src_xoff = g.m_xoff;
		break;
	default:
		if (b->ui_gray) return fail(SMHV_E_STATE, "batch_render_layers: the batch's ui_map is grayscale, map source %u needs the colour one", layers->map_source);
		if (layers->map_source == (uint32_t)SMHV_VIEW_CROPPED_BRQ) {
			y.src_mode = SMH_RND_SRC_CROPPED; y.src_w = g.rw / 2u; y.src_h = g.rh / 2u;
			if (y.src_w == 0u || y.src_h == 0u) return fail(SMHV_E_STATE, "batch_render_layers: the map has no bottom right quarter");
		} else y.src_mode = SMH_RND_SRC_PREPROCESS;
		break;
	}
	HIPCHK(hipSetDevice(b->ctx->device));
	const bool use_hm = (opt->flags & SMHV_RENDER_HEIGHTMAP) != 0u;
	RenderRun r;
	rc = render_prepare(b, first, n, b->d_results + first, use_hm ? hm : nullptr, opt, &r);
	if (rc) return rc;
	hipStream_t s = (hipStream_t)stream;
	rc = render_upload_prims(b, layers, &y, s);
	if (rc) return rc;
	render_bind(b, use_hm ? hm : nullptr);
	for (uint32_t done = 0; done < n;) {
		const uint32_t k = std::min(n - done, 65535u);
		RenderRun part = r;
		part.ui += (size_t)done * g.ui_stride; part.out += (size_t)done * r.out_stride; part.aux += done; part.res += done;
		RenderLayersRun yp = y;
		if (yp.src) yp.src += (size_t)done * y.src_stride;
		HIPCHK(launch_render_map_layers(g, part, yp, k, s));
		done += k;
	}
	HIPCHK(hipEventRecord(b->ev_render, s));
	return SMHV_OK;
}

extern "C" SMHV_API int smhv_render_map_layers(smhv_ctx *c, const smhv_heightmap *hm, const smhv_render_options *opt, const smhv_render_layers *layers,
                                               const smhv_line *lines, uint32_t n_lines, uint8_t *rgba) {
	int rc = require_open(c, "render_map_layers");
	if (rc) return rc;
	CTX_OPEN(c);
	if (!rgba || (n_lines && !lines)) return fail(SMHV_E_INVALID, "render_map_layers: null argument");
	if (n_lines > SMHV_RENDER_MAX_LINES) return fail(SMHV_E_INVALID, "render_map_layers: %u lines (at most %u)", n_lines, SMHV_RENDER_MAX_LINES);
	rc = check_render_options(opt, hm, "render_map_layers");
	if (rc) return rc;
	rc = check_render_layers(layers, "render_map_layers");
	if (rc) return rc;
	HIPCHK(hipSetDevice(c->device));
	smhv_batch *b = c->fb;
	const Geom &g = b->g;
	const bool use_hm = (opt->flags & SMHV_RENDER_HEIGHTMAP) != 0u;
	std::lock_guard<std::mutex> lk(c->fire_mu);
	RenderRun r;
	rc = render_prepare(b, 0, 1, b->d_results + 3, use_hm ? hm : nullptr, opt, &r);
	if (rc) return rc;
	RenderLayersRun y{};
	y.flags = layers->flags;
	y.src_mode = SMH_RND_SRC_UI; y.src_w = g.rw; y.src_h = g.rh;
	uint8_t *d_view = nullptr;
	if (layers->map_source != (uint32_t)SMHV_VIEW_NONE) {
		const int which = (int)layers->map_source;
		const bool brq = which == SMHV_VIEW_OCR_INPUT || which == SMHV_VIEW_FIND_SCALES_INPUT || which == SMHV_VIEW_CROPPED_BRQ;
		y.src_w = brq ? g.qw : g.rw; y.src_h = brq ? g.qh : g.rh;
		HIPCHK(hipMalloc((void **)&d_view, (size_t)y.src_w * y.src_h * 4u));
		Buffers bf = make_buffers(b, c->frame_ptr, 0);
		hipError_t e = launch_debug_view(g, bf, 0, which, c->isolated ? 1 : 0, d_view, c->s_main);
		if (e != hipSuccess) { (void)hipFree(d_view); return fail(SMHV_E_HIP, "render_map_layers: debug view: %s", hipGetErrorString(e)); }
		y.src_mode = SMH_RND_SRC_RGBA; y.src = d_view; y.src_pitch = (uint64_t)y.src_w * 4u;
	}
	const auto run = [&]() -> int {
		const size_t line_bytes = sizeof(smhv_line) * (size_t)SMHV_RENDER_MAX_LINES;
		if (c->fire_cap < line_bytes) {
			if (c->d_fire) (void)hipFree(c->d_fire);
			if (c->h_fire) (void)hipHostFree(c->h_fire);
			c->d_fire = c->h_fire = nullptr; c->fire_cap = 0;
			HIPCHK(hipMalloc((void **)&c->d_fire, line_bytes));
			HIPCHK(hipHostMalloc((void **)&c->h_fire, line_bytes));
			c->fire_cap = line_bytes;
		}
		if (n_lines && (opt->flags & SMHV_RENDER_MARKERS)) {
			memcpy(c->h_fire, lines, sizeof(smhv_line) * (size_t)n_lines);
			HIPCHK(hipMemcpyAsync(c->d_fire, c->h_fire, sizeof(smhv_line) * (size_t)n_lines, hipMemcpyHostToDevice, c->s_main));
			r.lines = (const smhv_line *)c->d_fire; r.n_lines = n_lines;
		} else
			r.flags &= ~SMHV_RENDER_MARKERS;
		int rc2 = render_upload_prims(b, layers, &y, c->s_main);
		if (rc2) return rc2;
		HIPCHK(launch_render_map_layers(g, r, y, 1, c->s_main));
		HIPCHK(hipEventRecord(b->ev_render, c->s_main));
		std::lock_guard<std::mutex> lk2(c->mu);
		return copy_image_d2h(c, 2, rgba, b->d_render, (size_t)r.out_stride / opt->out_h, 0, (size_t)opt->out_w * 4, opt->out_h, c->s_main);
	};
	rc = run();
	if (d_view) {
		if (rc) (void)hipStreamSynchronize(c->s_main);
		(void)hipFree(d_view);
	}
	return rc;
}

extern "C" SMHV_API int smhv_debug_render_form(uint32_t form) {
	if (form > 3u) return fail(SMHV_E_INVALID, "render form %u (0 = the rule, 1 = gathers, 2 = LDS staging, 3 = the colour table in LDS)", form);
	render_set_form(form);
// ... 24 lines not shown
```

### squad-mortar-helper_amd/csrc/smh_stream.hip

```cpp
#include <algorithm>
#include <atomic>
#include <cstdlib>

#include "smh_device.h"

namespace smh {

__device__ __forceinline__ uint32_t tile_occupancy(uint64_t rows_any, uint32_t lane, uint32_t ntr, uint8_t *occp, uint32_t pitch) {
	uint32_t alo = (uint32_t)rows_any, ahi = (uint32_t)(rows_any >> 32);
	alo |= SMH_DPP(alo, 0x101); ahi |= SMH_DPP(ahi, 0x101);
	alo |= SMH_DPP(alo, 0x102); ahi |= SMH_DPP(ahi, 0x102);
	alo |= SMH_DPP(alo, 0x104); ahi |= SMH_DPP(ahi, 0x104);
	uint32_t occ = 0;
#pragma unroll
	for (int t = 0; t < 4; ++t) occ |= (((alo >> (8 * t)) & 255u) ? 1u : 0u) << t;
#pragma unroll
	for (int t = 0; t < 3; ++t) occ |= (((ahi >> (8 * t)) & 255u) ? 1u : 0u) << (4 + t);
	if (lane & 7u) occ = 0u;
	uint32_t mine = 0;
#pragma unroll
	for (int t = 0; t < 7; ++t) {
		const uint64_t bal = __ballot((occ >> t) & 1u) & 0x0101010101010101ull;
		const uint32_t byte = (uint32_t)((bal * 0x0102040810204080ull) >> 56);
		if (lane == (uint32_t)t) mine = byte;
// ... 89 lines not shown
				uint32_t ov[4];
#pragma unroll
				for (int c = 0; c < 4; ++c) {
					const uint32_t p = pv[c], bb = p & 255u, gg = (p >> 8) & 255u, rr8 = (p >> 16) & 255u;
					if (GRAY) ov[c] = luma8(rr8, gg, bb) * 0x00010101u | 0xFF000000u;
					else ov[c] = rr8 | (gg << 8) | (bb << 16) | 0xFF000000u;
				}
				o.x = ov[0]; o.y = ov[1]; o.z = ov[2]; o.w = ov[3];
				*(uint4 *)(uip + (size_t)row * g.ui_pitch) = o;
			}
			if (do_mask) {
				uint32_t pre = 0;
#pragma unroll
				for (int c = 0; c < 4; ++c) pre |= marker_prefilter(pv[c]) ? (1u << c) : 0u;
				prehits |= (pre & vmask) << (4 * k);
			}
		}
		if (do_mask && __any(prehits != 0u)) {
			uint32_t *hpx = s_hits + wave * 160u;
			uint32_t *hres = hpx + 64;
			unsigned short *hid = (unsigned short *)(hres + 64);
			const uint32_t cnt = (uint32_t)__popc(prehits);
			uint32_t incl = cnt;
			for (int o = 1; o < 64; o <<= 1) { const uint32_t t = __shfl_up(incl, o); if (lane >= (uint32_t)o) incl += t; }
			const uint32_t total = __shfl(incl, 63);
			const uint32_t off = incl - cnt;
			hres[lane] = 0u;
			for (uint32_t base = 0; base < total; base += 64u) {
				uint32_t o = off - base;
#pragma unroll
				for (int k = 0; k < 4; ++k) {
					const uint32_t pk[4] = {px[k].x, px[k].y, px[k].z, px[k].w};
#pragma unroll
					for (int c = 0; c < 4; ++c)
						if ((prehits >> (4 * k + c)) & 1u) {
							if (o < 64u) { hpx[o] = pk[c]; hid[o] = (unsigned short)((lane << 4) | (uint32_t)(4 * k + c)); }
							++o;
						}
				}
				__builtin_amdgcn_wave_barrier();
				const uint32_t e = base + lane;
				if (e < total) {
					const uint32_t p = hpx[lane];
					if (marker_exact((p >> 16) & 255u, (p >> 8) & 255u, p & 255u)) {
						const uint32_t id = hid[lane];
						atomicOr(&hres[id >> 4], 1u << (id & 15u));
					}
				}
				__builtin_amdgcn_wave_barrier();
			}
			const uint32_t res = hres[lane];
			if (res) {
				const int sh = r - (r0 - 1);
#pragma unroll
				for (int c = 0; c < 4; ++c) {
					uint32_t y = (res >> c) & 0x1111u;
					y = (y | (y >> 3) | (y >> 6) | (y >> 9)) & 0xFu;
					P[c] |= (uint64_t)y << sh;
				}
			}
		}
	}
	if (!do_mask) return;

	__shared__ uint64_t s_edge_first[16], s_edge_last[16];
	if (lane == 0) s_edge_first[wave] = P[0];
	if (lane == 63) s_edge_last[wave] = P[3];
	__syncthreads();
	uint64_t left = __shfl_up(P[3], 1), right = __shfl_down(P[0], 1);
	if (lane == 0) left = wave > 0 ? s_edge_last[wave - 1] : 0ull;
	if (lane == 63) right = wave + 1 < nwave ? s_edge_first[wave + 1] : 0ull;
	const int nrows = r1 - r0;
	const uint64_t rowmask = ((nrows >= 63 ? ~0ull : ((1ull << nrows) - 1ull)) << 1);
	uint64_t D[4];
#define SMH_VERT(p) ((p) | ((p) << 1) | ((p) >> 1))
	D[0] = SMH_VERT(P[0]) | left | P[1];
	D[1] = SMH_VERT(P[1]) | P[0] | P[2];
	D[2] = SMH_VERT(P[2]) | P[1] | P[3];
	D[3] = SMH_VERT(P[3]) | P[2] | right;
#undef SMH_VERT
#pragma unroll
	for (int c = 0; c < 4; ++c) D[c] = ((vmask >> c) & 1u) ? (D[c] & rowmask) : 0ull;

	const uint32_t quads_padded = (g.m_quads + 15u) & ~15u;
	const uint64_t any = D[0] | D[1] | D[2] | D[3];
	const uint64_t lanes_set = __ballot(any != 0ull);
	uint32_t occ7 = 0;
	if constexpr (TILES) {
		const uint32_t ntr = ((uint32_t)nrows + 7u) >> 3, op = occ_pitch(g);
		uint8_t *occp = b.occ + (size_t)f * occ_stride(g) + (size_t)((uint32_t)r0 >> 3) * op + wave;
		if (lanes_set) occ7 = tile_occupancy(any >> 1, lane, ntr, occp, op);
		else if (lane < ntr) occp[(size_t)lane * op] = 0;
		if (blockIdx.x == 0 && q == 0) b.aux[f].tiles = 1u;
	}
	if (q < quads_padded) {
		uint8_t *mp = b.mask + (size_t)f * g.mask_stride + (size_t)q * 4;
		uint32_t *bp = b.bits + (size_t)f * g.bits_stride_w + (q >> 3);
		uint32_t *tp = nullptr;
		if constexpr (TILES) tp = b.tiled + (size_t)f * tiled_stride_w(g) + ((size_t)((uint32_t)r0 >> 3) * g.bits_pitch_w + (q >> 3)) * 8u;
		for (int row = r0; row < r1; ++row) {
			const int bit = row - r0 + 1;
			const uint32_t nib = (uint32_t)((D[0] >> bit) & 1ull) | ((uint32_t)((D[1] >> bit) & 1ull) << 1) |
			                     ((uint32_t)((D[2] >> bit) & 1ull) << 2) | ((uint32_t)((D[3] >> bit) & 1ull) << 3);
			*(uint32_t *)(mp + (size_t)row * g.mask_pitch) = ((nib * 0x00204081u) & 0x01010101u) * 0xFFu;
			uint32_t v = nib;
			v |= __shfl_down(v, 1) << 4;
			v |= __shfl_down(v, 2) << 8;
			v |= __shfl_down(v, 4) << 16;
			if ((lane & 7u) == 0) bp[(size_t)row * g.bits_pitch_w] = v;
			if constexpr (TILES) {
				const uint32_t i = (uint32_t)(row - r0);
				if ((occ7 >> (i >> 3)) & 1u) tp[(size_t)(i >> 3) * g.bits_pitch_w * 8u + (i & 7u)] = v;
			}
		}
	}
	if (lanes_set) {
		const uint64_t rows_set = wave_or64(any);
		const uint32_t cnt = wave_sum32(__popcll(D[0]) + __popcll(D[1]) + __popcll(D[2]) + __popcll(D[3]));
		if (lane == 0) {
			FrameAux *a = &b.aux[f];
			atomicMin(&a->y_min, (uint32_t)(r0 - 1 + __builtin_ctzll(rows_set)));
			atomicMax(&a->y_max, (uint32_t)(r0 - 1 + 63 - __builtin_clzll(rows_set)));
			atomicMin(&a->w_min, (wave * 64u + (uint32_t)__builtin_ctzll(lanes_set)) >> 3);
			atomicMax(&a->w_max, (wave * 64u + 63u - (uint32_t)__builtin_clzll(lanes_set)) >> 3);
			atomicAdd(&a->n_mask_px, cnt);
		}
	}
}

#define BRQ_RB 58

__global__ void __launch_bounds__(1024) k_brq_pass(Geom g, Buffers b, uint32_t flags, uint32_t fixed_start_y, int use_anchor_start) {
	const uint32_t f = blockIdx.y;
	if (!b.aux[f].open) return;
	uint32_t start_y = fixed_start_y;
	bool do_scales = (flags & BRQ_SCALES) != 0;
	if (use_anchor_start) {
		const smhv_anchors an = b.anchors[f];
		start_y = an.scales_start_y;
		if (an.n == 0 || start_y > g.qh) do_scales = false;
	}
	const bool do_ocr = (flags & BRQ_OCR) != 0;
	const uint32_t q = threadIdx.x, lane = q & 63u, wave = q >> 6, nwave = blockDim.x >> 6;
	const int r0 = (int)(blockIdx.x * BRQ_RB);
	const int r1 = min(r0 + BRQ_RB, (int)g.qh);
	const bool qact = q < g.q_quads;
	uint32_t vmask = 0, wmask = 0;
#pragma unroll
	for (int c = 0; c < 4; ++c) {
		const uint32_t x = 4 * q + c - g.q_xoff;
		if (x < g.qw) vmask |= 1u << c;
		if (x + SMH_OCR_DILATE_RADIUS <= g.qw) wmask |= 1u << c;
	}
	if (!qact) { vmask = 0; wmask = 0; }
	wmask &= vmask;

	const uint8_t *fp = b.frames + (size_t)f * g.frame_bytes + ((size_t)g.qy * g.W + g.q_ax + 4 * q) * 4;
	const size_t row_bytes = (size_t)g.W * 4;
	uint8_t *op = b.ocr + (size_t)f * g.ocr_stride + (size_t)q * 4;
	uint8_t *sp = b.scales + (size_t)f * g.ocr_stride + (size_t)q * 4;

	uint64_t Wb[4] = {0, 0, 0, 0}, Eb[4] = {0, 0, 0, 0};
	const int rs = max(r0 - 3, 0), re = min(r1 + 2, (int)g.qh - 1);
	const uint8_t *lp = qact ? fp : fp - (size_t)q * 16;
	uint4 nx[4];
#pragma unroll
	for (int k = 0; k < 4; ++k) nx[k] = *(const uint4 *)(lp + (size_t)min(rs + k, re) * row_bytes);
	for (int r = rs; r <= re; r += 4) {
		uint4 px[4];
#pragma unroll
		for (int k = 0; k < 4; ++k) px[k] = nx[k];
		if (r + 4 <= re) {
#pragma unroll
			for (int k = 0; k < 4; ++k) nx[k] = *(const uint4 *)(lp + (size_t)min(r + 4 + k, re) * row_bytes);
		}
#pragma unroll
		for (int k = 0; k < 4; ++k) {
			const int row = r + k;
			if (row > re) break;
			const int bit = row - (r0 - 3);
			const uint32_t pv[4] = {px[k].x, px[k].y, px[k].z, px[k].w};
			const bool out_row = row >= r0 && row < r1;
			const bool nb_row = (uint32_t)row + SMH_OCR_DILATE_RADIUS <= g.qh;
			uint32_t ocr_w = 0, sc_w = 0;
#pragma unroll
			for (int c = 0; c < 4; ++c) {
				const uint32_t p = pv[c], bb = p & 255u, gg = (p >> 8) & 255u, rr8 = (p >> 16) & 255u;
// ... 313 lines not shown
				const uint8_t *rowp = inside ? fbase + (size_t)(r + k) * row_bytes : dummy;
				SMH_LD128(dst[k], inside ? loff : 0u, rowp);
			}
		};
		if constexpr (SETS == 2) {
			u32x4 S0[GR], S1[GR];
			load4(S0, rs);
			for (int r = rs; ; r += 8) {
				load4(S1, r + 4);
				SMH_WAIT_SET(4, S0);
				group(S0, r);
				if (r + 4 > re) break;
				load4(S0, r + 8);
				SMH_WAIT_SET(4, S1);
				group(S1, r + 4);
				if (r + 8 > re) break;
			}
			asm volatile("s_waitcnt vmcnt(0) ; smh-drain" : "+v"(S0[0]), "+v"(S0[1]), "+v"(S0[2]), "+v"(S0[3]), "+v"(S1[0]), "+v"(S1[1]), "+v"(S1[2]), "+v"(S1[3]) : : "memory");
		} else {
			u32x4 S0[GR], S1[GR], S2[GR];
			load4(S0, rs);
			load4(S1, rs + 4);
			for (int r = rs; ; r += 12) {
				load4(S2, r + 8);
				SMH_WAIT_SET(8, S0);
				group(S0, r);
				if (r + 4 > re) break;
				load4(S0, r + 12);
				SMH_WAIT_SET(8, S1);
				group(S1, r + 4);
				if (r + 8 > re) break;
				load4(S1, r + 16);
				SMH_WAIT_SET(8, S2);
				group(S2, r + 8);
				if (r + 12 > re) break;
			}
			asm volatile("s_waitcnt vmcnt(0) ; smh-drain" : "+v"(S0[0]), "+v"(S0[1]), "+v"(S0[2]), "+v"(S0[3]), "+v"(S1[0]), "+v"(S1[1]), "+v"(S1[2]), "+v"(S1[3]),
			             "+v"(S2[0]), "+v"(S2[1]), "+v"(S2[2]), "+v"(S2[3]) : : "memory");
		}
	}

	uint64_t V[4];
#pragma unroll
	for (int c = 0; c < 4; ++c) {
		const uint64_t w = get_w(c);
		V[c] = w | (w << 1) | (w << 2) | (w << 3) | (w >> 1) | (w >> 2) | (w >> 3);
	}
	__shared__ uint64_t s_edge_first[16], s_edge_last[16], s_first[16][4], s_last[16][4];
	if (lane == 0) { s_edge_first[gwave] = P[0]; s_first[gwave][0] = V[0]; s_first[gwave][1] = V[1]; s_first[gwave][2] = V[2]; s_first[gwave][3] = V[3]; }
	if (lane == 63) { s_edge_last[gwave] = P[3]; s_last[gwave][0] = V[0]; s_last[gwave][1] = V[1]; s_last[gwave][2] = V[2]; s_last[gwave][3] = V[3]; }
	__syncthreads();
	if (do_mask) {
		uint64_t left = __shfl_up(P[3], 1), right = __shfl_down(P[0], 1);
		if (lane == 0) left = wave > 0 ? s_edge_last[gwave - 1] : 0ull;
		if (lane == 63) right = wave + 1 < nwave ? s_edge_first[gwave + 1] : 0ull;
		const int nrows = r1 - r0;
		const uint64_t rowmask = ((nrows >= 61 ? ~0ull : ((1ull << nrows) - 1ull)) << 3);
		uint64_t D[4];
#define SMH_VERT(p) ((p) | ((p) << 1) | ((p) >> 1))
		D[0] = SMH_VERT(P[0]) | left | P[1];
		D[1] = SMH_VERT(P[1]) | P[0] | P[2];
		D[2] = SMH_VERT(P[2]) | P[1] | P[3];
		D[3] = SMH_VERT(P[3]) | P[2] | right;
#undef SMH_VERT
#pragma unroll
		for (int c = 0; c < 4; ++c) D[c] = ((vmask >> c) & 1u) ? (D[c] & rowmask) : 0ull;
		const uint32_t quads_padded = (g.m_quads + 15u) & ~15u;
		const uint64_t any = D[0] | D[1] | D[2] | D[3];
		const uint64_t lanes_set = __ballot(any != 0ull);
		uint32_t occ7 = 0;
		uint32_t *tiled_out = nullptr;
		if constexpr (TILES) {
			MapKernelArgsPtr kb = ka;
			asm volatile("" : "+s"(kb));
			tiled_out = kb->b.tiled;
			uint8_t *const occ_out = kb->b.occ;
			const uint32_t ntr = ((uint32_t)nrows + 7u) >> 3, opitch = occ_pitch(g);
			uint8_t *occp = occ_out + (size_t)f * occ_stride(g) + (size_t)((uint32_t)r0 >> 3) * opitch + wave;
			if (lanes_set) occ7 = tile_occupancy(any >> 3, lane, ntr, occp, opitch);
			else if (lane < ntr) occp[(size_t)lane * opitch] = 0;
			if (band == 0u && q == 0u) b.aux[f].tiles = 1u;
		}
		if (q < quads_padded && !lanes_set) {
			uint8_t *mbase = b.mask + (size_t)f * g.mask_stride;
			uint32_t *bbase = b.bits + (size_t)f * g.bits_stride_w;
			const uint32_t moff = q * 4u, boff = (q >> 3) * 4u;
			const bool bit_lane = (lane & 7u) == 0;
			for (int row = r0; row < r1; ++row) {
				*(uint32_t *)(mbase + (size_t)row * g.mask_pitch + moff) = 0u;
				if (bit_lane) *(uint32_t *)((uint8_t *)bbase + (size_t)row * g.bits_pitch_w * 4u + boff) = 0u;
			}
		} else if (q < quads_padded) {
			uint8_t *mbase = b.mask + (size_t)f * g.mask_stride;
			uint32_t *bbase = b.bits + (size_t)f * g.bits_stride_w;
			const uint32_t moff = q * 4u, boff = (q >> 3) * 4u;
			const bool bit_lane = (lane & 7u) == 0;
			uint32_t *tp = nullptr;
			uint32_t tpitch = 0;
			if constexpr (TILES) { tp = tiled_out + (size_t)f * tiled_stride_w(g) + ((size_t)((uint32_t)r0 >> 3) * g.bits_pitch_w + (q >> 3)) * 8u; tpitch = g.bits_pitch_w * 8u; }
#pragma unroll
			for (int half = 0; half < 2; ++half) {
				const uint32_t d0 = (uint32_t)(D[0] >> (32 * half)), d1 = (uint32_t)(D[1] >> (32 * half)), d2 = (uint32_t)(D[2] >> (32 * half)), d3 = (uint32_t)(D[3] >> (32 * half));
				const int row_lo = max(r0, base + 32 * half), row_hi = min(r1, base + 32 * half + 32);
				for (int row = row_lo; row < row_hi; ++row) {
					const uint32_t bit = (uint32_t)(row - base) & 31u;
					const uint32_t nib = ((d0 >> bit) & 1u) | (((d1 >> bit) & 1u) << 1) | (((d2 >> bit) & 1u) << 2) | (((d3 >> bit) & 1u) << 3);
					*(uint32_t *)(mbase + (size_t)row * g.mask_pitch + moff) = nib_to_bytes(nib);
					uint32_t v = nib;
					v |= SMH_DPP(v, 0x101) << 4;
					v |= SMH_DPP(v, 0x102) << 8;
					v |= SMH_DPP(v, 0x104) << 16;
					if (bit_lane) *(uint32_t *)((uint8_t *)bbase + (size_t)row * g.bits_pitch_w * 4u + boff) = v;
					if constexpr (TILES) {
						const uint32_t i = (uint32_t)(row - r0);
						if ((occ7 >> (i >> 3)) & 1u) tp[(size_t)(i >> 3) * tpitch + (i & 7u)] = v;
					}
				}
			}
		}
		if (lanes_set) {
			const uint64_t rows_set = wave_or64(any);
			const uint32_t cnt = wave_sum32(__popcll(D[0]) + __popcll(D[1]) + __popcll(D[2]) + __popcll(D[3]));
			if (lane == 0) {
				FrameAux *a = &b.aux[f];
				atomicMin(&a->y_min, (uint32_t)(base + __builtin_ctzll(rows_set)));
				atomicMax(&a->y_max, (uint32_t)(base + 63 - __builtin_clzll(rows_set)));
				atomicMin(&a->w_min, (wave * 64u + (uint32_t)__builtin_ctzll(lanes_set)) >> 3);
				atomicMax(&a->w_max, (wave * 64u + 63u - (uint32_t)__builtin_clzll(lanes_set)) >> 3);
				atomicAdd(&a->n_mask_px, cnt);
			}
		}
	}
	if (!(wave_q && do_ocr)) return;
	uint64_t X[12];
#pragma unroll
	for (int c = 0; c < 4; ++c) {
		uint64_t l = __shfl_up(V[c], 1), r = __shfl_down(V[c], 1);
		if (lane == 0) l = wave > 0 ? s_last[gwave - 1][c] : 0ull;
		if (lane == 63) r = wave + 1 < nwave ? s_first[gwave + 1][c] : 0ull;
		X[c] = l; X[4 + c] = V[c]; X[8 + c] = r;
	}
#pragma unroll
	for (int c = 0; c < 4; ++c) {
		uint64_t d = 0;
#pragma unroll
		for (int k = -3; k <= 3; ++k) d |= X[4 + c + k];
		uint64_t kk = get_e(c) & d;
		while (kk) {
			const int bit = __builtin_ctzll(kk);
			kk &= kk - 1;
			const int row = base + bit;
			const uint32_t p = *(const uint32_t *)(fp + (size_t)row * row_bytes + 4 * c);
			const uint32_t l = luma_bgra(p);
			op[(size_t)(row - qy0) * g.ocr_pitch + qoff + c] = (uint8_t)(255u - l);
		}
	}
}

template <bool GRAY, bool LOOP, int SETS, bool TILES>
__global__ void __launch_bounds__(1024) k_map_brq_pass(Geom g, Buffers b, uint32_t flags, uint32_t qflags, uint32_t RB, uint32_t fixed_start_y, int use_anchor_start,
                                                       uint32_t nbands, uint32_t items) {
#ifdef SMH_MAP_FAT
	asm volatile("; register footprint experiment" ::: SMH_MAP_FAT);
#endif
	static_assert(sizeof(MapKernelArgs) == sizeof(Geom) + sizeof(Buffers) + 7 * 4 + 4 || sizeof(MapKernelArgs) == sizeof(Geom) + sizeof(Buffers) + 7 * 4, "the kernel's parameter list");
	MapKernelArgsPtr ka = (MapKernelArgsPtr)__builtin_amdgcn_kernarg_segment_ptr();
	if (flags & MAP_PRIO) __builtin_amdgcn_s_setprio(3);
	if (LOOP) {
		for (uint32_t item = blockIdx.x; item < items; item += gridDim.x) {
			const uint32_t f = item / nbands, band = item - f * nbands;
			map_brq_item<GRAY, SETS, TILES>(ka, f, band);
			__syncthreads();
		}
	} else {
		uint32_t f = blockIdx.y, band = blockIdx.x;
		if (flags & MAP_BAND_MAJOR) {
			const uint32_t id = blockIdx.y * gridDim.x + blockIdx.x;
			band = id / gridDim.y; f = id - band * gridDim.y;
		}
		map_brq_item<GRAY, SETS, TILES>(ka, f, band);
	}
}

hipError_t launch_button(const Geom &g, const Buffers &b, uint32_t n, int force_open, hipStream_t s) {
	hipLaunchKernelGGL(k_button, dim3(n), dim3(256), 0, s, g, b, force_open);
	return hipGetLastError();
}

static uint32_t work_item_order(bool overlapped) {
	const uint32_t forced = g_map_band_major.load(std::memory_order_relaxed);
	return (forced == 1u || (forced == 0u && !overlapped)) ? (uint32_t)MAP_BAND_MAJOR : 0u;
}

hipError_t launch_map_pass(const Geom &g, const Buffers &b, uint32_t n, uint32_t flags, int grayscale, hipStream_t s, bool tiles_wanted, bool overlapped) {
	const uint32_t RB = band_rows_for(g.rh, n, MAP_RB_MAX, tiles_wanted && b.tiled != nullptr, overlapped);
	const dim3 grid((g.rh + RB - 1) / RB, n);
	const unsigned lds = (g.m_block / 64u) * 640u;
	const bool tiles = tiles_wanted && b.tiled != nullptr && (RB & 7u) == 0u;
	if (tiles) {
		if (grayscale) hipLaunchKernelGGL((k_map_pass<true, true>), grid, dim3(g.m_block), lds, s, g, b, flags, RB);
		else hipLaunchKernelGGL((k_map_pass<false, true>), grid, dim3(g.m_block), lds, s, g, b, flags, RB);
	} else {
		if (grayscale) hipLaunchKernelGGL((k_map_pass<true, false>), grid, dim3(g.m_block), lds, s, g, b, flags, RB);
		else hipLaunchKernelGGL((k_map_pass<false, false>), grid, dim3(g.m_block), lds, s, g, b, flags, RB);
	}
	return hipGetLastError();
}

static uint32_t map_brq_static_lds() {
	static const uint32_t v = [] { hipFuncAttributes a; return hipFuncGetAttributes(&a, (const void *)k_map_brq_pass<true, true, 2, false>) == hipSuccess ? (uint32_t)a.sharedSizeBytes : 2048u; }();
	return v;
}
uint32_t map_brq_lds_bytes(const Geom &g) { return map_brq_static_lds() + (g.m_block / 64u) * 640u; }

hipError_t launch_map_brq_pass(const Geom &g, const Buffers &b, uint32_t n, uint32_t flags, uint32_t qflags, int grayscale, uint32_t fixed_start_y, int use_anchor_start, hipStream_t s,
                               const LaunchTuning *tune) {
	const uint32_t cap0 = tune ? tune->map_grid_cap : 0u;
	const uint32_t RB0 = band_rows_for(g.rh, n, MAPQ_RB_MAX, false);
	const bool no_tiles = b.tiled == nullptr || (tune && tune->map_deep) || (cap0 && cap0 < ((g.rh + RB0 - 1) / RB0) * n);
	const uint32_t RB = no_tiles ? RB0 : band_rows_for(g.rh, n, MAPQ_RB_MAX, true, tune && tune->map_overlapped);
	const uint32_t nbands = (g.rh + RB - 1) / RB, items = nbands * n;
	unsigned lds = (g.m_block / 64u) * 640u;
	if (tune && tune->map_lds_total > map_brq_lds_bytes(g)) lds = tune->map_lds_total - map_brq_static_lds();
	if (lds > 65536u) {
		static std::atomic<uint64_t> attr_devices{0};
		int dev = 0;
		hipError_t e = hipGetDevice(&dev);
		if (e != hipSuccess) return e;
		if (dev >= 64 || !((attr_devices.load(std::memory_order_acquire) >> dev) & 1ull)) {
			const void *fns[] = {(const void *)k_map_brq_pass<true, true, 2, false>, (const void *)k_map_brq_pass<false, true, 2, false>, (const void *)k_map_brq_pass<true, false, 2, false>,
			                     (const void *)k_map_brq_pass<false, false, 2, false>, (const void *)k_map_brq_pass<true, false, 2, true>, (const void *)k_map_brq_pass<false, false, 2, true>,
			                     (const void *)k_map_brq_pass<true, false, 3, false>, (const void *)k_map_brq_pass<false, false, 3, false>};
			for (const void *fn : fns) if (e == hipSuccess) e = hipFuncSetAttribute(fn, hipFuncAttributeMaxDynamicSharedMemorySize, 160 * 1024 - 2048);
			if (e != hipSuccess) return e;
			if (dev < 64) attr_devices.fetch_or(1ull << dev, std::memory_order_release);
		}
	}
	if (tune && tune->map_prio) flags |= MAP_PRIO;
	flags |= work_item_order(tune && tune->map_overlapped);
	const uint32_t cap = tune ? tune->map_grid_cap : 0u;
	const bool deep = tune && tune->map_deep && !(cap && cap < items);
	const bool tiles = !no_tiles && (RB & 7u) == 0u && !(cap && cap < items) && !deep;
#define SMH_LAUNCH_MAPQ(GRAYV, LOOPV, SETSV, TILESV, GRID) \
	hipLaunchKernelGGL((k_map_brq_pass<GRAYV, LOOPV, SETSV, TILESV>), GRID, dim3(g.m_block), lds, s, g, b, flags, qflags, RB, fixed_start_y, use_anchor_start, nbands, items)
	if (cap && cap < items) {
		if (grayscale) SMH_LAUNCH_MAPQ(true, true, 2, false, dim3(cap)); else SMH_LAUNCH_MAPQ(false, true, 2, false, dim3(cap));
	} else if (deep) {
		if (grayscale) SMH_LAUNCH_MAPQ(true, false, 3, false, dim3(nbands, n)); else SMH_LAUNCH_MAPQ(false, false, 3, false, dim3(nbands, n));
	} else if (tiles) {
		if (grayscale) SMH_LAUNCH_MAPQ(true, false, 2, true, dim3(nbands, n)); else SMH_LAUNCH_MAPQ(false, false, 2, true, dim3(nbands, n));
	} else {
		if (grayscale) SMH_LAUNCH_MAPQ(true, false, 2, false, dim3(nbands, n)); else SMH_LAUNCH_MAPQ(false, false, 2, false, dim3(nbands, n));
	}
#undef SMH_LAUNCH_MAPQ
	return hipGetLastError();
}

template <int NR>
__global__ void __launch_bounds__(1024) k_pattern_copy(Geom g, Buffers b, uint32_t RB, uint32_t band_major) {
	uint32_t f = blockIdx.y, band = blockIdx.x;
	if (band_major) {
		const uint32_t id = blockIdx.y * gridDim.x + blockIdx.x;
		band = id / gridDim.y; f = id - band * gridDim.y;
	}
	const uint32_t q = threadIdx.x;
	const int r0 = (int)(band * RB), r1 = min(r0 + (int)RB, (int)g.rh);
	if (q >= g.m_quads) return;
	const uint8_t *fp = b.frames + (size_t)f * g.frame_bytes + ((size_t)g.ry * g.W + g.m_ax) * 4 + (size_t)q * 16;
	uint8_t *up = b.ui + (size_t)f * g.ui_stride + (size_t)q * 16;
	uint8_t *mp = b.mask + (size_t)f * g.mask_stride + (size_t)q * 4;
	const int qy0 = (int)(g.qy - g.ry);
	const int qq = (int)q - (int)((g.q_ax - g.m_ax) >> 2);
	const bool in_q = qq >= 0 && (uint32_t)qq < g.q_quads;
	uint8_t *op = b.ocr + (size_t)f * g.ocr_stride + (size_t)(in_q ? qq : 0) * 4;
	uint8_t *sp = b.scales + (size_t)f * g.ocr_stride + (size_t)(in_q ? qq : 0) * 4;
	const size_t row_bytes = (size_t)g.W * 4;
	for (int r = r0; r < r1; r += NR) {
		uint4 v[NR];
#pragma unroll
		for (int k = 0; k < NR; ++k) v[k] = *(const uint4 *)(fp + (size_t)min(r + k, r1 - 1) * row_bytes);
#pragma unroll
		for (int k = 0; k < NR; ++k) {
			const int row = r + k;
			if (row >= r1) break;
			*(uint4 *)(up + (size_t)row * g.ui_pitch) = v[k];
			const uint32_t m = v[k].x ^ v[k].y ^ v[k].z ^ v[k].w;
			*(uint32_t *)(mp + (size_t)row * g.mask_pitch) = m;
			const int qrow = row - qy0;
			if (in_q && qrow >= 0 && qrow < (int)g.qh) {
				*(uint32_t *)(op + (size_t)qrow * g.ocr_pitch) = ~m;
				*(uint32_t *)(sp + (size_t)qrow * g.ocr_pitch) = m + 1u;
			}
		}
	}
}

hipError_t launch_pattern_copy(const Geom &g, const Buffers &b, uint32_t n, uint32_t rows_in_flight, hipStream_t s) {
	const uint32_t RB = band_rows_for(g.rh, n, MAPQ_RB_MAX);
	const dim3 grid((g.rh + RB - 1) / RB, n), block(g.m_block);
	const uint32_t bm = g_map_band_major.load(std::memory_order_relaxed) == 2u ? 0u : 1u;
	switch (rows_in_flight) {
	case 0: case 4: hipLaunchKernelGGL(k_pattern_copy<4>, grid, block, 0, s, g, b, RB, bm); break;
	case 8: hipLaunchKernelGGL(k_pattern_copy<8>, grid, block, 0, s, g, b, RB, bm); break;
	case 12: hipLaunchKernelGGL(k_pattern_copy<12>, grid, block, 0, s, g, b, RB, bm); break;
	default: return hipErrorInvalidValue;
	}
	return hipGetLastError();
}

void map_band_rows(uint32_t rh, uint32_t n, int fused, uint32_t *rows, int *tiles) {
	const uint32_t RB = band_rows_for(rh, n, fused ? MAPQ_RB_MAX : MAP_RB_MAX, true, fused == 2);
	if (rows) *rows = RB;
	if (tiles) *tiles = (RB & 7u) == 0u ? 1 : 0;
}

hipError_t launch_brq_pass(const Geom &g, const Buffers &b, uint32_t n, uint32_t flags, uint32_t fixed_start_y, int use_anchor_start, hipStream_t s) {
	const dim3 grid((g.qh + BRQ_RB - 1) / BRQ_RB, n);
	hipLaunchKernelGGL(k_brq_pass, grid, dim3(g.q_block), 0, s, g, b, flags, fixed_start_y, use_anchor_start);
	return hipGetLastError();
}

}
```

Before: 556,500.

## Defer byte-mask writes; expand mask lazily from bit mask on demand

The map pass no longer writes the per-pixel byte mask in the batched path and keeps only the packed bit mask. A new expand kernel rebuilds the byte mask from the bits when a consumer asks for it (device_ptrs, LSD-input views, feed or render). Staleness is tracked under a mutex, and an eager mode turns on once the pointer has been handed out. This removes a large byte-per-pixel store stream from the hot pipeline, at the cost of extra sync and bookkeeping and correctness risk if some consumer reads the mask without materializing it. A small tile-cap fallback fix is also included.

```diff
diff --git a/include/smh_vision_hip_debug.h b/include/smh_vision_hip_debug.h
--- a/include/smh_vision_hip_debug.h
+++ b/include/smh_vision_hip_debug.h
@@ -30,6 +30,8 @@
                                     uint32_t *lds_texels, uint32_t *form);
 SMHV_API int smhv_debug_feed_rows(uint32_t rows);
 SMHV_API int smhv_debug_feed_gray_form(uint32_t form);
+SMHV_API int smhv_debug_batch_mask_state(smhv_batch *b, uint32_t *stale_frames, int *eager);
+SMHV_API int smhv_debug_mask_expand(smhv_batch *b, uint32_t n, void *stream);
 SMHV_API int smhv_debug_ingest_feed(smhv_ingest *q, uint32_t n, uint32_t *counter);
 
 #ifdef __cplusplus
diff --git a/squad-mortar-helper_amd/_lib.py b/squad-mortar-helper_amd/_lib.py
--- a/squad-mortar-helper_amd/_lib.py
+++ b/squad-mortar-helper_amd/_lib.py
@@ -212,6 +212,8 @@
     "smhv_trait_times": (C.c_int, [C.c_void_p, C.POINTER(C.c_uint64), C.POINTER(C.c_uint64), C.c_int]),
     "smhv_ui_map": (C.c_int, [C.c_void_p, C.POINTER(C.c_void_p), C.POINTER(C.c_uint32), C.POINTER(C.c_uint32)]),
     "smhv_debug_pattern_copy": (C.c_int, [C.c_void_p, C.c_void_p, C.c_uint32, C.c_uint32, C.c_void_p]),
+    "smhv_debug_batch_mask_state": (C.c_int, [C.c_void_p, C.POINTER(C.c_uint32), C.POINTER(C.c_int)]),
+    "smhv_debug_mask_expand": (C.c_int, [C.c_void_p, C.c_uint32, C.c_void_p]),
     "smhv_debug_marker_table": (C.c_int, [C.c_void_p, C.c_void_p]),
     "smhv_ingest_create": (C.c_int, [C.c_void_p, C.c_uint32, C.c_uint32, C.c_uint32, C.c_uint32, C.POINTER(C.c_void_p)]),
     "smhv_ingest_create_ex": (C.c_int, [C.c_void_p, C.c_uint32, C.c_uint32, C.c_uint32, C.c_uint32, C.c_uint32, C.POINTER(C.c_void_p)]),
diff --git a/squad-mortar-helper_amd/batch.py b/squad-mortar-helper_amd/batch.py
--- a/squad-mortar-helper_amd/batch.py
+++ b/squad-mortar-helper_amd/batch.py
@@ -1,4 +1,5 @@
 import ctypes as C
+from collections.abc import Mapping
 
 import numpy as np
 
@@ -34,6 +35,26 @@
     return out
 
 
+_PTR_KEYS = ("results", "ui", "mask", "ocr", "scales", "bits")
+
+
+class _DevicePtrs(Mapping):
+
+    def __init__(self, batch, ptrs):
+        self._batch, self._ptrs = batch, ptrs
+
+    def __getitem__(self, key):
+        if key == "mask" and self._ptrs["mask"] is None:
+            self._ptrs["mask"] = self._batch._mask_ptr()
+        return self._ptrs[key]
+
+    def __iter__(self):
+        return iter(_PTR_KEYS)
+
+    def __len__(self):
+        return len(_PTR_KEYS)
+
+
 class FrameBatch:
 
     def __init__(self, vision, frame_w, frame_h, max_frames, _handle=None):
@@ -95,8 +116,20 @@
 
     def device_ptrs(self):
         p = [C.c_void_p() for _ in range(6)]
-        L.check(self._lib.smhv_batch_device_ptrs(self._b, *[C.byref(x) for x in p]))
-        return dict(zip(("results", "ui", "mask", "ocr", "scales", "bits"), [x.value for x in p]))
+        args = [C.byref(x) for x in p]
+        args[2] = None
+        L.check(self._lib.smhv_batch_device_ptrs(self._b, *args))
+        return _DevicePtrs(self, dict(zip(_PTR_KEYS, [x.value for x in p])))
+
+    def _mask_ptr(self):
+        m = C.c_void_p()
+        L.check(self._lib.smhv_batch_device_ptrs(self._b, None, None, C.byref(m), None, None, None))
+        return m.value
+
+    def mask_state(self):
+        stale, eager = C.c_uint32(0), C.c_int(0)
+        L.check(self._lib.smhv_debug_batch_mask_state(self._b, C.byref(stale), C.byref(eager)))
+        return int(stale.value), bool(eager.value)
 
     def tile_mask(self, frame=0):
         geo = (C.c_uint32 * 4)()
diff --git a/squad-mortar-helper_amd/csrc/smh_feed.inc b/squad-mortar-helper_amd/csrc/smh_feed.inc
--- a/squad-mortar-helper_amd/csrc/smh_feed.inc
+++ b/squad-mortar-helper_amd/csrc/smh_feed.inc
@@ -183,6 +183,10 @@
 	rc = feed_batch_source(b, first, map_source, true, &v);
 	if (rc) return rc;
 	HIPCHK(hipSetDevice(b->ctx->device));
+	if (map_source == (uint32_t)SMHV_VIEW_LSD_INPUT) {
+		rc = batch_materialize_mask(b, (hipStream_t)stream);
+		if (rc) return rc;
+	}
 	return feed_enqueue(f, v, b->d_results + first, first, n, flags, (hipStream_t)stream);
 }
 
diff --git a/squad-mortar-helper_amd/csrc/smh_kernels.h b/squad-mortar-helper_amd/csrc/smh_kernels.h
--- a/squad-mortar-helper_amd/csrc/smh_kernels.h
+++ b/squad-mortar-helper_amd/csrc/smh_kernels.h
@@ -312,7 +312,7 @@
 hipError_t launch_svc_publish(SvcCtl *ctl, unsigned long long *ring, SvcSlot *slots, uint32_t slot, const Buffers &b, uint32_t n, uint32_t seq, uint32_t ring_log2, hipStream_t s);
 hipError_t launch_lsd_service(const Geom &g, const SvcParams &p, uint32_t workgroups, uint32_t waves, uint32_t lds_bytes, hipStream_t s);
 
-enum : uint32_t { MAP_UI = 1u, MAP_MASK = 2u, MAP_PRIO = 0x100u, MAP_BAND_MAJOR = 0x200u };
+enum : uint32_t { MAP_UI = 1u, MAP_MASK = 2u, MAP_BYTES = 4u, MAP_PRIO = 0x100u, MAP_BAND_MAJOR = 0x200u };
 enum : uint32_t { BRQ_OCR = 1u, BRQ_SCALES = 2u };
 
 hipError_t launch_button(const Geom &g, const Buffers &b, uint32_t n, int force_open, hipStream_t s);
@@ -358,6 +358,7 @@
 float render_switch_ratio();
 hipError_t launch_debug_view(const Geom &g, const Buffers &b, uint32_t frame, int which, int isolated, uint8_t *d_rgba, hipStream_t s);
 hipError_t launch_marker_table(uint32_t *d_bits, hipStream_t s);
+hipError_t launch_mask_expand(const Geom &g, const uint32_t *d_bits, uint8_t *d_mask, uint32_t n, hipStream_t s);
 hipError_t launch_pack_rows(const void *d_src, uint32_t src_pitch_bytes, void *d_dst, uint32_t row_bytes, uint32_t rows, hipStream_t s);
 hipError_t launch_side_probe(uint32_t *d_out, uint32_t workgroups, uint32_t spin, hipStream_t s);
 hipError_t launch_build_sector_table(unsigned long long *d_tab, uint32_t T, hipStream_t s);
diff --git a/squad-mortar-helper_amd/csrc/smh_misc.hip b/squad-mortar-helper_amd/csrc/smh_misc.hip
--- a/squad-mortar-helper_amd/csrc/smh_misc.hip
+++ b/squad-mortar-helper_amd/csrc/smh_misc.hip
@@ -360,6 +360,25 @@
 	return hipGetLastError();
 }
 
+__global__ void __launch_bounds__(256) k_mask_expand(const uint16_t *__restrict__ bits, uint4 *__restrict__ mask, uint64_t groups) {
+	const uint64_t i = (uint64_t)blockIdx.x * 256u + threadIdx.x;
+	if (i >= groups) return;
+	const uint32_t v = bits[i];
+	uint4 o;
+	o.x = (((v & 15u) * 0x00204081u) & 0x01010101u) * 0xFFu;
+	o.y = ((((v >> 4) & 15u) * 0x00204081u) & 0x01010101u) * 0xFFu;
+	o.z = ((((v >> 8) & 15u) * 0x00204081u) & 0x01010101u) * 0xFFu;
+	o.w = ((((v >> 12) & 15u) * 0x00204081u) & 0x01010101u) * 0xFFu;
+	mask[i] = o;
+}
+hipError_t launch_mask_expand(const Geom &g, const uint32_t *d_bits, uint8_t *d_mask, uint32_t n, hipStream_t s) {
+	if (g.mask_pitch != (uint64_t)g.bits_pitch_w * 32u || (g.mask_stride & 15u)) return hipErrorInvalidValue;
+	const uint64_t groups = g.mask_stride / 16u * n, blocks = (groups + 255u) / 256u;
+	if (blocks == 0 || blocks > 0x7FFFFFFFull) return hipErrorInvalidValue;
+	hipLaunchKernelGGL(k_mask_expand, dim3((uint32_t)blocks), dim3(256), 0, s, (const uint16_t *)d_bits, (uint4 *)d_mask, groups);
+	return hipGetLastError();
+}
+
 hipError_t launch_debug_view(const Geom &g, const Buffers &b, uint32_t frame, int which, int isolated, uint8_t *d_rgba, hipStream_t s) {
 	const bool brq = which == SMHV_VIEW_OCR_INPUT || which == SMHV_VIEW_FIND_SCALES_INPUT || which == SMHV_VIEW_CROPPED_BRQ;
 	const uint32_t npx = brq ? g.qw * g.qh : g.rw * g.rh;
diff --git a/squad-mortar-helper_amd/csrc/smh_runtime.cpp b/squad-mortar-helper_amd/csrc/smh_runtime.cpp
--- a/squad-mortar-helper_amd/csrc/smh_runtime.cpp
+++ b/squad-mortar-helper_amd/csrc/smh_runtime.cpp
@@ -196,6 +196,10 @@
 	hipEvent_t ev_render = nullptr;
 	bool ui_written = false;
 	bool ui_gray = false, mask_written = false, ocr_written = false, scales_written = false;
+	std::mutex mask_mu;
+	uint32_t mask_stale = 0;
+	bool mask_eager = false;
+	hipEvent_t ev_mask = nullptr;
 	smhv_render_prim *h_prims = nullptr, *d_prims = nullptr;
 	hipEvent_t ev_prims = nullptr;
 	smhv_label_result *d_labels = nullptr;
@@ -543,6 +547,7 @@
 		hipError_t e = hipHostMalloc((void **)&b->h_err, sizeof(BatchError), hipHostMallocMapped | hipHostMallocCoherent);
 		if (e == hipSuccess) { memset(b->h_err, 0, sizeof(BatchError)); e = hipHostGetDevicePointer((void **)&b->d_err, b->h_err, 0); }
 		if (e == hipSuccess) e = hipEventCreateWithFlags(&b->ev_map_done, hipEventDisableTiming);
+		if (e == hipSuccess) e = hipEventCreateWithFlags(&b->ev_mask, hipEventDisableTiming);
 		if (max_frames > 1 && !lsd_rows_only(b->g)) {
 			if (e == hipSuccess) e = create_stream(&b->lsd_fork.s1, nullptr);
 			if (e == hipSuccess) e = create_stream(&b->lsd_fork.s2, nullptr);
@@ -594,6 +599,7 @@
 	if (b->ev_fork) (void)hipEventDestroy(b->ev_fork);
 	if (b->ev_join) (void)hipEventDestroy(b->ev_join);
 	if (b->ev_map_done) (void)hipEventDestroy(b->ev_map_done);
+	if (b->ev_mask) (void)hipEventDestroy(b->ev_mask);
 	for (auto e : b->ev_probe) if (e) (void)hipEventDestroy(e);
 	if (b->lsd_fork.s1) (void)hipStreamDestroy(b->lsd_fork.s1);
 	if (b->lsd_fork.s2) (void)hipStreamDestroy(b->lsd_fork.s2);
@@ -782,6 +788,16 @@
 	return SMHV_OK;
 }
 
+static int batch_materialize_mask(smhv_batch *b, hipStream_t stream) {
+	std::lock_guard<std::mutex> lk(b->mask_mu);
+	if (b->mask_stale) {
+		HIPCHK(launch_mask_expand(b->g, b->d_bits, b->d_mask, std::min(b->mask_stale, b->max_frames), stream));
+		HIPCHK(hipEventRecord(b->ev_mask, stream));
+		b->mask_stale = 0;
+	} else HIPCHK(hipStreamWaitEvent(stream, b->ev_mask, 0));
+	return SMHV_OK;
+}
+
 struct SvcPublish { SvcCtl *ctl; unsigned long long *ring; SvcSlot *slots; uint32_t slot, seq, ring_log2; const uint32_t *cull_tab; bool have_cull; hipStream_t s_pro; hipEvent_t ev_pro;
                     bool *published; };
 static int batch_run_impl(smhv_batch *b, const void *d_frames, uint32_t n, uint32_t stages, int grayscale, uint32_t max_gap,
@@ -851,6 +867,11 @@
 	STAGE_BEGIN(1, s);
 	if (mflags && qflags) HIPCHK(launch_map_brq_pass(g, bf, n, mflags, qflags, grayscale, 0, 1, s, &b->tune));
 	else if (mflags) HIPCHK(launch_map_pass(g, bf, n, mflags, grayscale, s, true, b->tune.map_overlapped != 0u));
+	if (mflags & MAP_MASK) {
+		std::lock_guard<std::mutex> lk(b->mask_mu);
+		if (b->mask_eager) HIPCHK(launch_mask_expand(g, b->d_bits, b->d_mask, n, s));
+		else b->mask_stale = std::max(b->mask_stale, n);
+	}
 	STAGE_END(1, s);
 	if (mflags & MAP_UI) { b->ui_written = true; b->ui_gray = grayscale != 0; }
 	if (mflags & MAP_MASK) b->mask_written = true;
@@ -964,7 +985,16 @@
 	if (!b) return fail(SMHV_E_INVALID, "null batch");
 	if (r) *r = b->d_results;
 	if (ui) *ui = b->d_ui;
-	if (mask) *mask = b->d_mask;
+	if (mask) {
+		CTX_OPEN(b->ctx);
+		HIPCHK(hipSetDevice(b->ctx->device));
+		{ std::lock_guard<std::mutex> lk(b->mask_mu); b->mask_eager = true; }
+		HIPCHK(hipDeviceSynchronize());
+		int rc = batch_materialize_mask(b, b->ctx->s_main);
+		if (rc) return rc;
+		HIPCHK(wait_stream(b->ctx->s_main));
+		*mask = b->d_mask;
+	}
 	if (ocr) *ocr = b->d_ocr;
 	if (scales) *scales = b->d_scales;
 	if (bits) *bits = b->d_bits;
@@ -1031,6 +1061,8 @@
 		break;
 	case SMHV_VIEW_LSD_INPUT: {
 		std::lock_guard<std::mutex> lk(b->ctx->mu);
+		int rc = batch_materialize_mask(b, b->ctx->s_main);
+		if (rc) return rc;
 		return copy_image_d2h(b->ctx, 2, out, b->d_mask + frame * g.mask_stride, g.mask_pitch, g.m_xoff, g.rw, g.rh, b->ctx->s_main);
 	}
 	case SMHV_VIEW_OCR_INPUT: {
@@ -1772,7 +1804,7 @@
 	Buffers bf = make_buffers(b, c->frame_ptr, 0);
 	hipStream_t s = c->s_main;
 	HIPCHK(launch_button(g, bf, 1, 0, s));
-	HIPCHK(launch_map_pass(g, bf, 1, MAP_UI | MAP_MASK, grayscale, s));
+	HIPCHK(launch_map_pass(g, bf, 1, MAP_UI | MAP_MASK | MAP_BYTES, grayscale, s));
 	b->ui_written = true; b->ui_gray = grayscale != 0;
 	HIPCHK(hipEventRecord(c->ev_map, s));
 	Buffers bm = make_buffers(b, c->frame_ptr, 3);
@@ -1907,7 +1939,7 @@
 	HIPCHK(hipSetDevice(c->device));
 	smhv_batch *b = c->fb;
 	Buffers bf = make_buffers(b, c->frame_ptr, 0);
-	HIPCHK(launch_map_pass(b->g, bf, 1, MAP_MASK, 1, c->s_markers));
+	HIPCHK(launch_map_pass(b->g, bf, 1, MAP_MASK | MAP_BYTES, 1, c->s_markers));
 	HIPCHK(wait_stream(c->s_markers));
 	c->mask_valid = true;
 	return SMHV_OK;
@@ -2497,6 +2529,22 @@
 	return SMHV_OK;
 }
 
+extern "C" SMHV_API int smhv_debug_batch_mask_state(smhv_batch *b, uint32_t *stale_frames, int *eager) {
+	if (!b) return fail(SMHV_E_INVALID, "null batch");
+	std::lock_guard<std::mutex> lk(b->mask_mu);
+	if (stale_frames) *stale_frames = b->mask_stale;
+	if (eager) *eager = b->mask_eager ? 1 : 0;
+	return SMHV_OK;
+}
+
+extern "C" SMHV_API int smhv_debug_mask_expand(smhv_batch *b, uint32_t n, void *stream) {
+	if (!b || n == 0 || n > b->max_frames) return fail(SMHV_E_INVALID, "debug_mask_expand: bad arguments");
+	CTX_OPEN(b->ctx);
+	HIPCHK(hipSetDevice(b->ctx->device));
+	HIPCHK(launch_mask_expand(b->g, b->d_bits, b->d_mask, n, (hipStream_t)stream));
+	return SMHV_OK;
+}
+
 extern "C" SMHV_API int smhv_debug_ingest_feed(smhv_ingest *q, uint32_t n, uint32_t *counter) {
 	if (!q || !counter) return fail(SMHV_E_INVALID, "ingest_feed: null argument");
 	for (uint32_t i = 0; i < n; ++i) {
@@ -2980,6 +3028,10 @@
 	rc = render_prepare(b, first, n, b->d_results + first, use_hm ? hm : nullptr, opt, &r);
 	if (rc) return rc;
 	hipStream_t s = (hipStream_t)stream;
+	if (layers->map_source == (uint32_t)SMHV_VIEW_LSD_INPUT) {
+		rc = batch_materialize_mask(b, s);
+		if (rc) return rc;
+	}
 	rc = render_upload_prims(b, layers, &y, s);
 	if (rc) return rc;
 	render_bind(b, use_hm ? hm : nullptr);
diff --git a/squad-mortar-helper_amd/csrc/smh_stream.hip b/squad-mortar-helper_amd/csrc/smh_stream.hip
--- a/squad-mortar-helper_amd/csrc/smh_stream.hip
+++ b/squad-mortar-helper_amd/csrc/smh_stream.hip
@@ -195,6 +195,7 @@
 #pragma unroll
 	for (int c = 0; c < 4; ++c) D[c] = ((vmask >> c) & 1u) ? (D[c] & rowmask) : 0ull;
 
+	const bool do_bytes = (flags & MAP_BYTES) != 0;
 	const uint32_t quads_padded = (g.m_quads + 15u) & ~15u;
 	const uint64_t any = D[0] | D[1] | D[2] | D[3];
 	const uint64_t lanes_set = __ballot(any != 0ull);
@@ -215,7 +216,7 @@
 			const int bit = row - r0 + 1;
 			const uint32_t nib = (uint32_t)((D[0] >> bit) & 1ull) | ((uint32_t)((D[1] >> bit) & 1ull) << 1) |
 			                     ((uint32_t)((D[2] >> bit) & 1ull) << 2) | ((uint32_t)((D[3] >> bit) & 1ull) << 3);
-			*(uint32_t *)(mp + (size_t)row * g.mask_pitch) = ((nib * 0x00204081u) & 0x01010101u) * 0xFFu;
+			if (do_bytes) *(uint32_t *)(mp + (size_t)row * g.mask_pitch) = ((nib * 0x00204081u) & 0x01010101u) * 0xFFu;
 			uint32_t v = nib;
 			v |= __shfl_down(v, 1) << 4;
 			v |= __shfl_down(v, 2) << 8;
@@ -695,18 +696,14 @@
 			if (band == 0u && q == 0u) b.aux[f].tiles = 1u;
 		}
 		if (q < quads_padded && !lanes_set) {
-			uint8_t *mbase = b.mask + (size_t)f * g.mask_stride;
 			uint32_t *bbase = b.bits + (size_t)f * g.bits_stride_w;
-			const uint32_t moff = q * 4u, boff = (q >> 3) * 4u;
+			const uint32_t boff = (q >> 3) * 4u;
 			const bool bit_lane = (lane & 7u) == 0;
-			for (int row = r0; row < r1; ++row) {
-				*(uint32_t *)(mbase + (size_t)row * g.mask_pitch + moff) = 0u;
-				if (bit_lane) *(uint32_t *)((uint8_t *)bbase + (size_t)row * g.bits_pitch_w * 4u + boff) = 0u;
-			}
+			if (bit_lane)
+				for (int row = r0; row < r1; ++row) *(uint32_t *)((uint8_t *)bbase + (size_t)row * g.bits_pitch_w * 4u + boff) = 0u;
 		} else if (q < quads_padded) {
-			uint8_t *mbase = b.mask + (size_t)f * g.mask_stride;
 			uint32_t *bbase = b.bits + (size_t)f * g.bits_stride_w;
-			const uint32_t moff = q * 4u, boff = (q >> 3) * 4u;
+			const uint32_t boff = (q >> 3) * 4u;
 			const bool bit_lane = (lane & 7u) == 0;
 			uint32_t *tp = nullptr;
 			uint32_t tpitch = 0;
@@ -718,7 +715,6 @@
 				for (int row = row_lo; row < row_hi; ++row) {
 					const uint32_t bit = (uint32_t)(row - base) & 31u;
 					const uint32_t nib = ((d0 >> bit) & 1u) | (((d1 >> bit) & 1u) << 1) | (((d2 >> bit) & 1u) << 2) | (((d3 >> bit) & 1u) << 3);
-					*(uint32_t *)(mbase + (size_t)row * g.mask_pitch + moff) = nib_to_bytes(nib);
 					uint32_t v = nib;
 					v |= SMH_DPP(v, 0x101) << 4;
 					v |= SMH_DPP(v, 0x102) << 8;
@@ -830,9 +826,10 @@
                                const LaunchTuning *tune) {
 	const uint32_t cap0 = tune ? tune->map_grid_cap : 0u;
 	const uint32_t RB0 = band_rows_for(g.rh, n, MAPQ_RB_MAX, false);
-	const bool no_tiles = b.tiled == nullptr || (tune && tune->map_deep) || (cap0 && cap0 < ((g.rh + RB0 - 1) / RB0) * n);
-	const uint32_t RB = no_tiles ? RB0 : band_rows_for(g.rh, n, MAPQ_RB_MAX, true, tune && tune->map_overlapped);
-	const uint32_t nbands = (g.rh + RB - 1) / RB, items = nbands * n;
+	bool no_tiles = b.tiled == nullptr || (tune && tune->map_deep) || (cap0 && cap0 < ((g.rh + RB0 - 1) / RB0) * n);
+	uint32_t RB = no_tiles ? RB0 : band_rows_for(g.rh, n, MAPQ_RB_MAX, true, tune && tune->map_overlapped);
+	uint32_t nbands = (g.rh + RB - 1) / RB, items = nbands * n;
+	if (!no_tiles && cap0 && cap0 < items) { no_tiles = true; RB = RB0; nbands = (g.rh + RB - 1) / RB; items = nbands * n; }
 	unsigned lds = (g.m_block / 64u) * 640u;
 	if (tune && tune->map_lds_total > map_brq_lds_bytes(g)) lds = tune->map_lds_total - map_brq_static_lds();
 	if (lds > 65536u) {
@@ -881,7 +878,6 @@
 	if (q >= g.m_quads) return;
 	const uint8_t *fp = b.frames + (size_t)f * g.frame_bytes + ((size_t)g.ry * g.W + g.m_ax) * 4 + (size_t)q * 16;
 	uint8_t *up = b.ui + (size_t)f * g.ui_stride + (size_t)q * 16;
-	uint8_t *mp = b.mask + (size_t)f * g.mask_stride + (size_t)q * 4;
 	const int qy0 = (int)(g.qy - g.ry);
 	const int qq = (int)q - (int)((g.q_ax - g.m_ax) >> 2);
 	const bool in_q = qq >= 0 && (uint32_t)qq < g.q_quads;
@@ -898,7 +894,6 @@
 			if (row >= r1) break;
 			*(uint4 *)(up + (size_t)row * g.ui_pitch) = v[k];
 			const uint32_t m = v[k].x ^ v[k].y ^ v[k].z ^ v[k].w;
-			*(uint32_t *)(mp + (size_t)row * g.mask_pitch) = m;
 			const int qrow = row - qy0;
 			if (in_q && qrow >= 0 && qrow < (int)g.qh) {
 				*(uint32_t *)(op + (size_t)qrow * g.ocr_pitch) = ~m;
```

After: 581,900, median of 6. 4.6% higher.
